# HKU-BAL/MegaGTA

Measured on AMD Instinct MI355X. Metric: HMM-scored node expansions/sec + SdBG-build Gk-mer/s, k=45, 100Mx150bp, higher is better.
Workload: dtype u32

## Files before the change

include/megagta_hip.h:

```cpp
#ifndef MEGAGTA_HIP_H_
#define MEGAGTA_HIP_H_
#include <stdint.h>
#ifdef __cplusplus
extern "C" {
#endif

#define MGTA_OK 0
#define MGTA_EINVAL (-1)
#define MGTA_EHIP (-2)
#define MGTA_ENOMEM (-3)
#define MGTA_EUNSUPPORTED (-4)
#define MGTA_ESINK (-5)
#define MGTA_EOVERFLOW (-6)
#define MGTA_EINTERNAL (-7)

#define MGTA_NUM_BUCKETS 65536

typedef struct mgta_ctx mgta_ctx;
typedef struct mgta_reads mgta_reads;
typedef struct mgta_sdbg mgta_sdbg;
typedef struct mgta_hmm mgta_hmm;

const char *mgta_last_error(void);
const char *mgta_version(void);

mgta_ctx *mgta_ctx_create(int device_id);
void mgta_ctx_destroy(mgta_ctx *);
int mgta_ctx_set_mem_limit(mgta_ctx *, uint64_t bytes);
int mgta_ctx_device_memory(mgta_ctx *, uint64_t *free_bytes, uint64_t *total_bytes);
int mgta_ctx_keep_stream(mgta_ctx *, int on);
typedef struct mgta_stream mgta_stream;
int mgta_sdbg_stream_detach(mgta_ctx *, mgta_stream **out);
int mgta_stream_sizes(const mgta_stream *, uint64_t *n_recs, uint64_t *n_tip_words);
int mgta_stream_download(mgta_stream *, uint16_t *recs, uint32_t *tips);
void mgta_stream_free(mgta_stream *);
int mgta_ctx_release_scratch(mgta_ctx *);
int mgta_ctx_set_full_lsd(mgta_ctx *, int on);
int mgta_sort_plan(uint64_t n_items, int words_per_key, uint32_t bucket_begin, uint32_t bucket_end, int *n_passes, int *skip_bits);
int mgta_ctx_set_search_cost_rate(mgta_ctx *, int expansions_per_seed);
int mgta_ctx_set_search_cost_curve(mgta_ctx *, int expansions_per_seed, uint64_t knee_expansions, int expansions_per_seed_beyond);
int mgta_ctx_set_search_arena(mgta_ctx *, int log2_base_nodes, uint64_t pool_bytes);
int mgta_ctx_set_search_page_limit(mgta_ctx *, int pages);
int mgta_ctx_keep_multiplicity(mgta_ctx *, int on);

int mgta_reads_pack_text(mgta_ctx *, const char *text, uint64_t n_bytes, const uint64_t *offsets , uint64_t n_reads,
                         uint32_t *bin_words, uint64_t capacity_words, uint64_t *n_words_out);


typedef int (*mgta_edge_sink)(void *user, int32_t bucket_begin, int32_t bucket_end,
                              const int64_t *bucket_counts ,
                              const uint16_t *recs, int64_t n_recs, const uint16_t *large, int64_t n_large,
                              const uint32_t *tips, int64_t n_tip_words);

typedef struct mgta_build_stats {
    int32_t k, words_per_key, words_per_tip, n_passes;
    int64_t n_reads, n_kmers;
    int64_t n_items;
    int64_t n_edges, n_tips, n_large;
    int64_t n_sort_launches;
    double ms_total;
    double ms_count, ms_gen, ms_sort, ms_emit, ms_d2h;
    double ms_sort_scatter;
    double ms_local_sort;
    int64_t n_big_segments;
    int64_t n_lsd_tiles;
    uint64_t bytes_peak;
    double ms_stage1;
    int64_t n_fused_passes;
} mgta_build_stats;

int mgta_reads_upload(mgta_ctx *, const uint32_t *packed_seq, uint64_t n_words, const uint64_t *start_idx,
                      uint64_t n_reads, mgta_reads **out);
int mgta_reads_adopt_device(mgta_ctx *, const uint32_t *d_packed_seq, uint64_t n_words,
                            const uint64_t *d_start_idx, uint64_t n_reads, mgta_reads **out);
void mgta_reads_free(mgta_reads *);

int mgta_sdbg_build_resident(mgta_ctx *, const mgta_reads *, uint64_t n_short_reads, int k, int min_count,
                             int need_mercy, int32_t bucket_begin, int32_t bucket_end ,
                             mgta_edge_sink sink, void *user, mgta_build_stats *stats);
int mgta_sdbg_last_counting(mgta_ctx *, int64_t *hist );
int mgta_sdbg_export_records_device(mgta_ctx *, void *d_dst, uint64_t capacity_bytes, uint64_t *n_records);
int mgta_sdbg_build(mgta_ctx *, const uint32_t *packed_seq, uint64_t n_words, const uint64_t *start_idx,
                    uint64_t n_reads, uint64_t n_short_reads, int k, int min_count, int need_mercy,
                    mgta_edge_sink sink, void *user, mgta_build_stats *stats);

int mgta_sdbg_load(mgta_ctx *, int k, const uint16_t *recs, int64_t size, const int64_t *bucket_items,
                   const uint32_t *tips, int64_t n_tip_words, int words_per_tip, mgta_sdbg **out);
int mgta_sdbg_load_resident(mgta_ctx *, mgta_sdbg **out);
int mgta_sdbg_load_large(mgta_ctx *, int k, const uint16_t *recs, int64_t size, const int64_t *bucket_items, const uint32_t *tips,
                         int64_t n_tip_words, int words_per_tip, const uint16_t *large, int64_t n_large, mgta_sdbg **out);
int mgta_sdbg_load_files(mgta_ctx *, const char *prefix, mgta_sdbg **out);
void mgta_sdbg_free(mgta_sdbg *);
int64_t mgta_sdbg_size(const mgta_sdbg *);
int mgta_sdbg_k(const mgta_sdbg *);
int mgta_sdbg_outgoing(mgta_sdbg *, const int64_t *edges, int64_t n, int64_t *out4, int8_t *outdeg);
int mgta_sdbg_invalid_bits(mgta_sdbg *, uint64_t *words);
int mgta_sdbg_index_edges(mgta_sdbg *, const uint8_t *seqs , int64_t n, int64_t *edge_ids);

int mgta_sdbg_edge_multiplicity(mgta_sdbg *, const int64_t *edge_ids, int64_t n, uint16_t *mult);

typedef struct mgta_contig_cov {
    uint64_t sum;
    uint32_t len, n_windows;
    uint32_t n_covered;
    uint32_t min, max, median;
} mgta_contig_cov;
typedef struct mgta_coverage_stats {
    int64_t n_contigs, n_windows;
    int64_t n_walked;
    int64_t n_index_searches;
    int64_t n_batches;
    int64_t groups_per_cu;
    double ms_kernel;
    double ms_walk;
} mgta_coverage_stats;
int mgta_ctx_set_coverage_batch(mgta_ctx *, uint64_t windows);
int mgta_contig_coverage(mgta_sdbg *, const char *seqs, const uint64_t *offsets , int64_t n, mgta_contig_cov *per_contig,
                         uint16_t *per_window , int64_t *abundance , mgta_coverage_stats *stats );

typedef struct mgta_contig_share {
    uint64_t mass;
    uint32_t len, n_windows;
    uint32_t n_covered;
    uint32_t n_unique;
    uint32_t max_share;
    uint32_t reserved_;
} mgta_contig_share;
typedef struct mgta_share_stats {
    int64_t n_contigs, n_windows;
    int64_t n_walked, n_index_searches;
    int64_t n_batches;
    int64_t n_covered;
    int64_t n_distinct_edges;
    uint64_t total_mult;
    uint64_t total_mass;
    uint64_t table_slots;
    uint64_t table_bytes;
    uint64_t window_bytes;
    double ms_walk;
    double ms_count;
    double ms_share;
    double ms_total;
} mgta_share_stats;
int mgta_ctx_set_share_hash_bits(mgta_ctx *, int bits);
int mgta_contig_share_coverage(mgta_sdbg *, const char *seqs, const uint64_t *offsets , int64_t n, mgta_contig_share *per_contig,
                               uint32_t *per_window_share , uint16_t *per_window , mgta_share_stats *stats );

typedef struct mgta_match_stats {
    int64_t n_contigs, n_contig_windows;
    int64_t n_marked_edges;
    int64_t n_reads, n_read_windows;
    int64_t n_walked, n_index_searches;
    int64_t n_matched_reads;
    int64_t groups_per_cu;
    double ms_mark, ms_walk;
} mgta_match_stats;
int mgta_reads_match_contigs(mgta_sdbg *, const mgta_reads *reads, int reads_reversed, uint64_t n_short_reads,
                             const char *seqs, const uint64_t *offsets , int64_t n,
                             uint64_t *match_bits ,
                             uint32_t *hit_windows , mgta_match_stats *stats );

typedef struct mgta_derep_stats {
    int64_t n_seqs, n_letters;
    int64_t n_first;
    int64_t n_duplicates, n_contained, n_kept;
    int64_t n_windows;
    int64_t anchor_len;
    int64_t n_compares;
    double ms_dups, ms_table, ms_verify;
} mgta_derep_stats;
int mgta_seqs_derep(mgta_ctx *, const char *seqs, const uint64_t *offsets , int64_t n,
                    uint8_t *status, int64_t *rep, uint32_t *copies, mgta_derep_stats *stats );
int mgta_ctx_set_derep_hash_bits(mgta_ctx *, int bits);

typedef struct mgta_align_rec {
    double score;
    int32_t status;
    int32_t model_from, model_to;
    int32_t n_match, n_insert, n_delete;
} mgta_align_rec;
typedef struct mgta_align_stats {
    int64_t n_seqs, n_aligned, n_unaligned;
    int64_t n_cells;
    int64_t n_batches;
    int64_t blocks_per_cu;
    int64_t waves_per_block;
    int64_t grid_blocks;
    int64_t lds_bytes;
    int64_t msc_in_lds;
    double ms_fill, ms_trace;
} mgta_align_stats;
int mgta_seqs_align(mgta_ctx *, const mgta_hmm *, const char *seqs, const uint64_t *offsets , int64_t n,
                    mgta_align_rec *recs , uint8_t *cols , char *path ,
                    int32_t *path_len , mgta_align_stats *stats );
int mgta_ctx_set_align_batch(mgta_ctx *, int64_t cells);

typedef struct mgta_row_pair { int32_t i, j; uint16_t n_diff, n_overlap; } mgta_row_pair;
typedef struct mgta_cluster_stats {
    int64_t n_rows, n_unaligned;
    int64_t n_pairs_kept;
    int64_t n_clusters, n_singletons, largest_cluster;
    int64_t n_components;
    int64_t n_tiles;
    int64_t n_link_pops;
    int64_t blocks_per_cu;
    int64_t grid_blocks;
    int64_t lds_bytes;
    int64_t peak_bytes;
    double ms_pairs, ms_link;
} mgta_cluster_stats;
int mgta_rows_pairs(mgta_ctx *, const uint8_t *rows , int64_t n, int64_t M, int64_t min_overlap, double cutoff,
                    mgta_row_pair *pairs , int64_t cap, int64_t *n_pairs, mgta_cluster_stats *stats );
int mgta_rows_cluster(mgta_ctx *, const uint8_t *rows , const int64_t *lens , int64_t n, int64_t M, int64_t min_overlap,
                      double cutoff, int32_t *cluster , int64_t *rep , uint16_t *rep_diff ,
                      uint16_t *rep_overlap , mgta_cluster_stats *stats );
int mgta_pairs_link(const mgta_row_pair *pairs , int64_t n_pairs, const int32_t *n_residues ,
                    const int64_t *lens , int64_t n, int32_t *cluster, int64_t *rep, uint16_t *rep_diff, uint16_t *rep_overlap,
                    mgta_cluster_stats *stats );
int mgta_ctx_set_cluster_tile(mgta_ctx *, int64_t rows_per_tile);

typedef struct mgta_nearest_rec { int32_t status, ref, score, ref_from, ref_to, n_match, n_ident, n_insert, n_delete; } mgta_nearest_rec;
// ... 117 lines not shown
```

megagta_amd/_lib.py:

```python
from __future__ import annotations

import ctypes as C
import os

_HERE = os.path.dirname(os.path.abspath(__file__))
LIB_PATH = os.environ.get("MEGAGTA_HIP_LIB") or os.path.join(_HERE, "libmegagta_hip.so")


class MegaGtaError(RuntimeError):
    pass


class DenovoStats(C.Structure):
    _fields_ = [("n_tips", C.c_int64), ("n_bubbles", C.c_int64), ("n_bubble_candidates", C.c_int64), ("n_bubble_rounds", C.c_int64),
                ("n_paths", C.c_int64), ("n_unitig_sweeps", C.c_int64), ("n_contigs", C.c_int64), ("total_len", C.c_int64),
                ("ms_tips", C.c_float), ("ms_bubbles", C.c_float), ("ms_unitigs", C.c_float)]

    def as_dict(self):
        return {n: getattr(self, n) for n, _ in self._fields_}


class BuildStats(C.Structure):
    _fields_ = [("k", C.c_int32), ("words_per_key", C.c_int32), ("words_per_tip", C.c_int32), ("n_passes", C.c_int32),
                ("n_reads", C.c_int64), ("n_kmers", C.c_int64), ("n_items", C.c_int64), ("n_edges", C.c_int64),
                ("n_tips", C.c_int64), ("n_large", C.c_int64), ("n_sort_launches", C.c_int64), ("ms_total", C.c_double),
                ("ms_count", C.c_double), ("ms_gen", C.c_double), ("ms_sort", C.c_double), ("ms_emit", C.c_double),
                ("ms_d2h", C.c_double), ("ms_sort_scatter", C.c_double), ("ms_local_sort", C.c_double), ("n_big_segments", C.c_int64), ("n_lsd_tiles", C.c_int64),
                ("bytes_peak", C.c_uint64), ("ms_stage1", C.c_double), ("n_fused_passes", C.c_int64)]

    def as_dict(self):
        return {n: getattr(self, n) for n, _ in self._fields_}


class AstarSide(C.Structure):
    _fields_ = [("ok", C.c_int32), ("fval", C.c_int32), ("length", C.c_int32), ("state_no", C.c_int32), ("state", C.c_int32),
                ("partial", C.c_int32), ("node_id", C.c_int64), ("n_closed", C.c_int64), ("n_expanded", C.c_int64),
                ("n_opened", C.c_int64), ("real_score", C.c_double), ("score", C.c_double)]


class AstarStats(C.Structure):
    _fields_ = [("n_seeds", C.c_int64), ("n_expansions", C.c_int64), ("n_opened", C.c_int64), ("n_retries", C.c_int64),
                ("ms_total", C.c_double), ("ms_kernel", C.c_double), ("n_grown", C.c_int64), ("n_rehash", C.c_int64),
                ("n_recycled", C.c_int64), ("pool_bytes", C.c_uint64), ("pool_used", C.c_uint64), ("n_resumes", C.c_int64),
                ("reserve_bytes", C.c_uint64), ("reserve_used", C.c_uint64), ("max_search_nodes", C.c_int64),
                ("max_search_expansions", C.c_int64), ("order_abandoned", C.c_int64), ("n_cache_drops", C.c_int64), ("hmm_in_lds", C.c_int64), ("n_over_limit", C.c_int64), ("ms_queue_drained", C.c_double)]

    def as_dict(self):
        return {n: getattr(self, n) for n, _ in self._fields_}


class LineProbe(C.Structure):
    _fields_ = [("waves_per_cu", C.c_int32), ("groups", C.c_int32), ("unroll", C.c_int32), ("dependent", C.c_int32), ("steps", C.c_uint64),
                ("lines_in_flight_per_cu", C.c_int32), ("pad_", C.c_int32), ("lines", C.c_uint64), ("ms", C.c_double), ("gb_per_s", C.c_double),
                ("ns_per_step", C.c_double)]

    def as_dict(self):
        return {n: getattr(self, n) for n, _ in self._fields_ if n != "pad_"}


class ContigCov(C.Structure):
    _fields_ = [("sum", C.c_uint64), ("len", C.c_uint32), ("n_windows", C.c_uint32), ("n_covered", C.c_uint32), ("min", C.c_uint32),
                ("max", C.c_uint32), ("median", C.c_uint32)]


class CoverageStats(C.Structure):
    _fields_ = [("n_contigs", C.c_int64), ("n_windows", C.c_int64), ("n_walked", C.c_int64), ("n_index_searches", C.c_int64),
                ("n_batches", C.c_int64), ("groups_per_cu", C.c_int64), ("ms_kernel", C.c_double), ("ms_walk", C.c_double)]

    def as_dict(self):
        return {n: getattr(self, n) for n, _ in self._fields_}


class ContigShare(C.Structure):
    _fields_ = [("mass", C.c_uint64), ("len", C.c_uint32), ("n_windows", C.c_uint32), ("n_covered", C.c_uint32), ("n_unique", C.c_uint32),
                ("max_share", C.c_uint32), ("reserved_", C.c_uint32)]


class ShareStats(C.Structure):
    _fields_ = [("n_contigs", C.c_int64), ("n_windows", C.c_int64), ("n_walked", C.c_int64), ("n_index_searches", C.c_int64), ("n_batches", C.c_int64),
                ("n_covered", C.c_int64), ("n_distinct_edges", C.c_int64), ("total_mult", C.c_uint64), ("total_mass", C.c_uint64),
                ("table_slots", C.c_uint64), ("table_bytes", C.c_uint64), ("window_bytes", C.c_uint64), ("ms_walk", C.c_double), ("ms_count", C.c_double),
                ("ms_share", C.c_double), ("ms_total", C.c_double)]

    def as_dict(self):
        return {n: getattr(self, n) for n, _ in self._fields_}


class MatchStats(C.Structure):
    _fields_ = [("n_contigs", C.c_int64), ("n_contig_windows", C.c_int64), ("n_marked_edges", C.c_int64), ("n_reads", C.c_int64),
                ("n_read_windows", C.c_int64), ("n_walked", C.c_int64), ("n_index_searches", C.c_int64), ("n_matched_reads", C.c_int64),
                ("groups_per_cu", C.c_int64), ("ms_mark", C.c_double), ("ms_walk", C.c_double)]

    def as_dict(self):
        return {n: getattr(self, n) for n, _ in self._fields_}


class DerepStats(C.Structure):
    _fields_ = [("n_seqs", C.c_int64), ("n_letters", C.c_int64), ("n_first", C.c_int64), ("n_duplicates", C.c_int64), ("n_contained", C.c_int64),
                ("n_kept", C.c_int64), ("n_windows", C.c_int64), ("anchor_len", C.c_int64), ("n_compares", C.c_int64), ("ms_dups", C.c_double),
                ("ms_table", C.c_double), ("ms_verify", C.c_double)]

    def as_dict(self):
        return {n: getattr(self, n) for n, _ in self._fields_}


class AlignRec(C.Structure):
    _fields_ = [("score", C.c_double), ("status", C.c_int32), ("model_from", C.c_int32), ("model_to", C.c_int32), ("n_match", C.c_int32),
                ("n_insert", C.c_int32), ("n_delete", C.c_int32)]


class AlignStats(C.Structure):
    _fields_ = [("n_seqs", C.c_int64), ("n_aligned", C.c_int64), ("n_unaligned", C.c_int64), ("n_cells", C.c_int64), ("n_batches", C.c_int64),
                ("blocks_per_cu", C.c_int64), ("waves_per_block", C.c_int64), ("grid_blocks", C.c_int64), ("lds_bytes", C.c_int64),
                ("msc_in_lds", C.c_int64), ("ms_fill", C.c_double), ("ms_trace", C.c_double)]

    def as_dict(self):
        return {n: getattr(self, n) for n, _ in self._fields_}


class RowPair(C.Structure):
    _fields_ = [("i", C.c_int32), ("j", C.c_int32), ("n_diff", C.c_uint16), ("n_overlap", C.c_uint16)]


class ClusterStats(C.Structure):
    _fields_ = [("n_rows", C.c_int64), ("n_unaligned", C.c_int64), ("n_pairs_kept", C.c_int64), ("n_clusters", C.c_int64), ("n_singletons", C.c_int64),
                ("largest_cluster", C.c_int64), ("n_components", C.c_int64), ("n_tiles", C.c_int64), ("n_link_pops", C.c_int64),
                ("blocks_per_cu", C.c_int64), ("grid_blocks", C.c_int64), ("lds_bytes", C.c_int64), ("peak_bytes", C.c_int64),
                ("ms_pairs", C.c_double), ("ms_link", C.c_double)]

    def as_dict(self):
        return {n: getattr(self, n) for n, _ in self._fields_}


class NearestRec(C.Structure):
    _fields_ = [("status", C.c_int32), ("ref", C.c_int32), ("score", C.c_int32), ("ref_from", C.c_int32), ("ref_to", C.c_int32), ("n_match", C.c_int32),
                ("n_ident", C.c_int32), ("n_insert", C.c_int32), ("n_delete", C.c_int32)]


class NearestStats(C.Structure):
    _fields_ = [("n_seqs", C.c_int64), ("n_refs", C.c_int64), ("n_pairs", C.c_int64), ("n_unaligned", C.c_int64), ("n_cells", C.c_int64),
                ("n_trace_cells", C.c_int64), ("n_batches", C.c_int64), ("n_segments", C.c_int64), ("blocks_per_cu", C.c_int64),
                ("waves_per_block", C.c_int64), ("grid_blocks", C.c_int64), ("lds_bytes", C.c_int64), ("peak_bytes", C.c_int64),
                ("ms_score", C.c_double), ("ms_trace", C.c_double)]

    def as_dict(self):
        return {n: getattr(self, n) for n, _ in self._fields_}


class ChimeraRec(C.Structure):
    _fields_ = [("status", C.c_int32), ("ref", C.c_int32), ("score", C.c_int32), ("brk", C.c_int32), ("left_ref", C.c_int32), ("left_score", C.c_int32),
                ("right_ref", C.c_int32), ("right_score", C.c_int32), ("two", C.c_int32), ("one", C.c_int32), ("gain", C.c_int32)]


class ChimeraStats(C.Structure):
    _fields_ = [("n_seqs", C.c_int64), ("n_refs", C.c_int64), ("n_clean", C.c_int64), ("n_chimeric", C.c_int64), ("n_unchecked", C.c_int64),
                ("n_cells", C.c_int64), ("n_parent_cells", C.c_int64), ("n_items", C.c_int64), ("n_parent_items", C.c_int64), ("n_segments", C.c_int64),
                ("n_groups", C.c_int64), ("grid_blocks", C.c_int64), ("waves_per_block", C.c_int64), ("blocks_per_cu", C.c_int64), ("lds_bytes", C.c_int64),
                ("bound_bytes", C.c_int64), ("peak_bytes", C.c_int64), ("ms_top", C.c_double), ("ms_parents", C.c_double)]

    def as_dict(self):
        return {n: getattr(self, n) for n, _ in self._fields_}


EDGE_SINK = C.CFUNCTYPE(C.c_int, C.c_void_p, C.c_int32, C.c_int32, C.POINTER(C.c_int64), C.POINTER(C.c_uint16), C.c_int64,
                        C.POINTER(C.c_uint16), C.c_int64, C.POINTER(C.c_uint32), C.c_int64)
CONTIG_SINK = C.CFUNCTYPE(C.c_int, C.c_void_p, C.c_int64, C.c_void_p, C.c_int64, C.c_void_p, C.c_int64,
                          C.POINTER(AstarSide), C.POINTER(AstarSide))

SYMBOLS = {
    "mgta_last_error": (C.c_char_p, []),
    "mgta_version": (C.c_char_p, []),
    "mgta_ctx_create": (C.c_void_p, [C.c_int]),
    "mgta_ctx_destroy": (None, [C.c_void_p]),
    "mgta_ctx_set_mem_limit": (C.c_int, [C.c_void_p, C.c_uint64]),
    "mgta_ctx_set_full_lsd": (C.c_int, [C.c_void_p, C.c_int]),
    "mgta_sort_plan": (C.c_int, [C.c_uint64, C.c_int, C.c_uint32, C.c_uint32, C.POINTER(C.c_int), C.POINTER(C.c_int)]),
    "mgta_reads_upload": (C.c_int, [C.c_void_p, C.c_void_p, C.c_uint64, C.c_void_p, C.c_uint64, C.POINTER(C.c_void_p)]),
    "mgta_reads_adopt_device": (C.c_int, [C.c_void_p, C.c_void_p, C.c_uint64, C.c_void_p, C.c_uint64, C.POINTER(C.c_void_p)]),
    "mgta_reads_free": (None, [C.c_void_p]),
    "mgta_sdbg_build_resident": (C.c_int, [C.c_void_p, C.c_void_p, C.c_uint64, C.c_int, C.c_int, C.c_int, C.c_int32, C.c_int32,
                                          EDGE_SINK, C.c_void_p, C.POINTER(BuildStats)]),
    "mgta_sdbg_last_counting": (C.c_int, [C.c_void_p, C.c_void_p]),
    "mgta_sdbg_export_records_device": (C.c_int, [C.c_void_p, C.c_void_p, C.c_uint64, C.POINTER(C.c_uint64)]),
    "mgta_sdbg_build": (C.c_int, [C.c_void_p, C.c_void_p, C.c_uint64, C.c_void_p, C.c_uint64, C.c_uint64, C.c_int, C.c_int,
                                 C.c_int, EDGE_SINK, C.c_void_p, C.POINTER(BuildStats)]),
    "mgta_findstart": (C.c_int, [C.c_void_p, C.c_void_p, C.c_int, C.c_int, C.c_void_p, C.c_int64, C.c_void_p, C.c_int64, C.c_void_p, C.c_void_p]),
    "mgta_sdbg_load_resident": (C.c_int, [C.c_void_p, C.c_void_p]),
    "mgta_sdbg_load_files": (C.c_int, [C.c_void_p, C.c_char_p, C.c_void_p]),
    "mgta_sdbg_invalid_bits": (C.c_int, [C.c_void_p, C.c_void_p]),
    "mgta_ctx_set_search_cost_rate": (C.c_int, [C.c_void_p, C.c_int]),
    "mgta_ctx_set_search_cost_curve": (C.c_int, [C.c_void_p, C.c_int, C.c_uint64, C.c_int]),
    "mgta_ctx_set_search_arena": (C.c_int, [C.c_void_p, C.c_int, C.c_uint64]),
    "mgta_ctx_set_search_page_limit": (C.c_int, [C.c_void_p, C.c_int]),
    "mgta_ctx_device_memory": (C.c_int, [C.c_void_p, C.POINTER(C.c_uint64), C.POINTER(C.c_uint64)]),
    "mgta_ctx_keep_stream": (C.c_int, [C.c_void_p, C.c_int]),
    "mgta_sdbg_stream_detach": (C.c_int, [C.c_void_p, C.POINTER(C.c_void_p)]),
    "mgta_stream_sizes": (C.c_int, [C.c_void_p, C.POINTER(C.c_uint64), C.POINTER(C.c_uint64)]),
    "mgta_stream_download": (C.c_int, [C.c_void_p, C.c_void_p, C.c_void_p]),
    "mgta_stream_free": (None, [C.c_void_p]),
    "mgta_sdbg_k": (C.c_int, [C.c_void_p]),
    "mgta_ctx_set_search_share": (C.c_int, [C.c_void_p, C.c_int, C.c_int]),
    "mgta_astar_batch_on": (C.c_int, [C.c_void_p, C.c_void_p, C.c_void_p, C.c_void_p, C.c_char_p, C.c_void_p, C.c_int64, C.c_int, C.c_double,
                                     C.c_int, CONTIG_SINK, C.c_void_p, C.POINTER(AstarStats)]),
    "mgta_astar_batch_packed": (C.c_int, [C.c_void_p, C.c_void_p, C.c_void_p, C.c_char_p, C.c_void_p, C.c_int64, C.c_int, C.c_double, C.c_int,
                                         C.POINTER(C.c_void_p), C.c_void_p, C.c_void_p, C.POINTER(AstarStats)]),
    "mgta_reads_pack_text": (C.c_int, [C.c_void_p, C.c_char_p, C.c_uint64, C.c_void_p, C.c_uint64, C.c_void_p, C.c_uint64, C.POINTER(C.c_uint64)]),
    "mgta_ctx_release_scratch": (C.c_int, [C.c_void_p]),
    "mgta_denovo": (C.c_int, [C.c_void_p, C.c_int, C.c_int, C.c_int, C.c_void_p, C.c_void_p, C.c_void_p]),
    "mgta_host_free": (None, [C.c_void_p]),
    "mgta_sdbg_load": (C.c_int, [C.c_void_p, C.c_int, C.c_void_p, C.c_int64, C.c_void_p, C.c_void_p, C.c_int64, C.c_int,
                                C.POINTER(C.c_void_p)]),
    "mgta_ctx_keep_multiplicity": (C.c_int, [C.c_void_p, C.c_int]),
    "mgta_ctx_set_coverage_batch": (C.c_int, [C.c_void_p, C.c_uint64]),
    "mgta_sdbg_load_large": (C.c_int, [C.c_void_p, C.c_int, C.c_void_p, C.c_int64, C.c_void_p, C.c_void_p, C.c_int64, C.c_int, C.c_void_p, C.c_int64,
                                      C.POINTER(C.c_void_p)]),
    "mgta_sdbg_edge_multiplicity": (C.c_int, [C.c_void_p, C.c_void_p, C.c_int64, C.c_void_p]),
    "mgta_contig_coverage": (C.c_int, [C.c_void_p, C.c_char_p, C.c_void_p, C.c_int64, C.c_void_p, C.c_void_p, C.c_void_p, C.c_void_p]),
    "mgta_contig_share_coverage": (C.c_int, [C.c_void_p, C.c_char_p, C.c_void_p, C.c_int64, C.c_void_p, C.c_void_p, C.c_void_p, C.c_void_p]),
    "mgta_ctx_set_share_hash_bits": (C.c_int, [C.c_void_p, C.c_int]),
    "mgta_reads_match_contigs": (C.c_int, [C.c_void_p, C.c_void_p, C.c_int, C.c_uint64, C.c_char_p, C.c_void_p, C.c_int64, C.c_void_p, C.c_void_p,
                                          C.c_void_p]),
    "mgta_seqs_derep": (C.c_int, [C.c_void_p, C.c_char_p, C.c_void_p, C.c_int64, C.c_void_p, C.c_void_p, C.c_void_p, C.c_void_p]),
    "mgta_ctx_set_derep_hash_bits": (C.c_int, [C.c_void_p, C.c_int]),
    "mgta_seqs_align": (C.c_int, [C.c_void_p, C.c_void_p, C.c_char_p, C.c_void_p, C.c_int64, C.c_void_p, C.c_void_p, C.c_void_p, C.c_void_p, C.c_void_p]),
    "mgta_ctx_set_align_batch": (C.c_int, [C.c_void_p, C.c_int64]),
    "mgta_rows_pairs": (C.c_int, [C.c_void_p, C.c_void_p, C.c_int64, C.c_int64, C.c_int64, C.c_double, C.c_void_p, C.c_int64, C.c_void_p, C.c_void_p]),
    "mgta_rows_cluster": (C.c_int, [C.c_void_p, C.c_void_p, C.c_void_p, C.c_int64, C.c_int64, C.c_int64, C.c_double, C.c_void_p, C.c_void_p, C.c_void_p,
                                    C.c_void_p, C.c_void_p]),
    "mgta_pairs_link": (C.c_int, [C.c_void_p, C.c_int64, C.c_void_p, C.c_void_p, C.c_int64, C.c_void_p, C.c_void_p, C.c_void_p, C.c_void_p, C.c_void_p]),
    "mgta_ctx_set_cluster_tile": (C.c_int, [C.c_void_p, C.c_int64]),
    "mgta_seqs_nearest": (C.c_int, [C.c_void_p, C.c_char_p, C.c_void_p, C.c_int64, C.c_char_p, C.c_void_p, C.c_int64, C.c_void_p, C.c_int32, C.c_int32,
                                    C.c_void_p, C.c_void_p, C.c_void_p, C.c_void_p, C.c_void_p]),
    "mgta_ctx_set_nearest_batch": (C.c_int, [C.c_void_p, C.c_int64]),
    "mgta_seqs_chimera": (C.c_int, [C.c_void_p, C.c_char_p, C.c_void_p, C.c_int64, C.c_char_p, C.c_void_p, C.c_int64, C.c_void_p, C.c_int32, C.c_int32,
                                    C.c_int32, C.c_int32, C.c_void_p, C.c_void_p, C.c_void_p]),
    "mgta_ctx_set_chimera_segment": (C.c_int, [C.c_void_p, C.c_int64]),
    "mgta_ctx_set_chimera_groups": (C.c_int, [C.c_void_p, C.c_int64]),
    "mgta_sdbg_free": (None, [C.c_void_p]),
    "mgta_sdbg_size": (C.c_int64, [C.c_void_p]),
    "mgta_sdbg_outgoing": (C.c_int, [C.c_void_p, C.c_void_p, C.c_int64, C.c_void_p, C.c_void_p]),
    "mgta_sdbg_index_edges": (C.c_int, [C.c_void_p, C.c_void_p, C.c_int64, C.c_void_p]),
    "mgta_hmm_load": (C.c_int, [C.c_void_p, C.c_int, C.c_int, C.c_void_p, C.c_void_p, C.c_void_p, C.c_void_p, C.c_void_p,
                               C.POINTER(C.c_void_p)]),
    "mgta_hmm_free": (None, [C.c_void_p]),
    "mgta_probe_random_lines": (C.c_int, [C.c_void_p, C.c_uint64, C.POINTER(LineProbe), C.c_int]),
    "mgta_astar_batch": (C.c_int, [C.c_void_p, C.c_void_p, C.c_void_p, C.c_char_p, C.c_void_p, C.c_int64, C.c_int, C.c_double,
                                  C.c_int, CONTIG_SINK, C.c_void_p, C.POINTER(AstarStats)]),
}

_LIB = None


def load():
    global _LIB
    if _LIB is not None:
        return _LIB
    if not os.path.exists(LIB_PATH):
        raise MegaGtaError(f"{LIB_PATH} is missing: build it with `python -c 'import __graft_entry__ as g; g.build()'` "
                           "(make -C megagta_amd/csrc). There is no CPU fallback.")
    L = C.CDLL(LIB_PATH)
    for name, (res, args) in SYMBOLS.items():
        fn = getattr(L, name)
        fn.restype, fn.argtypes = res, args
    _LIB = L
    return L


def check(rc: int, what: str):
    if rc != 0:
        raise MegaGtaError(f"{what} failed ({rc}): {load().mgta_last_error().decode()}")
```

megagta_amd/csrc/common.hpp:

```cpp
#pragma once
#include <hip/hip_runtime.h>

#include <cstdarg>
#include <cstdint>
#include <cstdio>
#include <cstring>
#include <exception>
#include <new>
#include <string>
#include <vector>

#include "../../include/megagta_hip.h"

namespace mgta {

void set_error(const char *fmt, ...);

struct HipError {
    int code;
};

#define MGTA_HIP_CHECK(expr)                                                                        \
    do {                                                                                            \
        hipError_t e_ = (expr);                                                                     \
        if (e_ != hipSuccess) {                                                                     \
            ::mgta::set_error("%s failed: %s (%s:%d)", #expr, hipGetErrorString(e_), __FILE__, __LINE__); \
            throw ::mgta::HipError{e_ == hipErrorOutOfMemory ? MGTA_ENOMEM : MGTA_EHIP};           \
        }                                                                                           \
    } while (0)

struct DevBuf {
    void *p = nullptr;
    size_t bytes = 0;
    uint64_t *live = nullptr, *peak = nullptr;
    DevBuf() = default;
    DevBuf(const DevBuf &) = delete;
    DevBuf &operator=(const DevBuf &) = delete;
    DevBuf(DevBuf &&o) noexcept { *this = std::move(o); }
    DevBuf &operator=(DevBuf &&o) noexcept {
        if (this != &o) { release(); p = o.p; bytes = o.bytes; live = o.live; peak = o.peak; o.p = nullptr; o.bytes = 0; }
        return *this;
    }
    ~DevBuf() { release(); }
    void alloc(size_t n, uint64_t *live_ = nullptr, uint64_t *peak_ = nullptr) {
        release();
        if (n == 0) n = 16;
        MGTA_HIP_CHECK(hipMalloc(&p, n));
        bytes = n; live = live_; peak = peak_;
        if (live) { *live += n; if (peak && *live > *peak) *peak = *live; }
    }
    void release() {
        if (p) { (void)hipFree(p); if (live) *live -= bytes; }
        p = nullptr; bytes = 0;
    }
    template <class T> T *as() const { return reinterpret_cast<T *>(p); }
};

template <class F> int guarded(const char *who, F &&f) {
    try { return f(); }
    catch (const HipError &e) { return e.code; }
    catch (const std::bad_alloc &) { set_error("%s: out of host memory", who); return MGTA_ENOMEM; }
    catch (const std::exception &e) { set_error("%s: %s", who, e.what()); return MGTA_EHIP; }
}

struct Timer {
    hipEvent_t a = nullptr, b = nullptr;
    hipStream_t st;
    explicit Timer(hipStream_t s) : st(s) { MGTA_HIP_CHECK(hipEventCreate(&a)); MGTA_HIP_CHECK(hipEventCreate(&b)); }
    Timer(Timer &&o) noexcept : a(o.a), b(o.b), st(o.st) { o.a = o.b = nullptr; }
    ~Timer() { if (a) (void)hipEventDestroy(a); if (b) (void)hipEventDestroy(b); }
    void start() { MGTA_HIP_CHECK(hipEventRecord(a, st)); }
    void end() { MGTA_HIP_CHECK(hipEventRecord(b, st)); }
    float ms() const { float t = 0; MGTA_HIP_CHECK(hipEventElapsedTime(&t, a, b)); return t; }
    double stop() {
        MGTA_HIP_CHECK(hipGetLastError());
        end();
        MGTA_HIP_CHECK(hipEventSynchronize(b));
        MGTA_HIP_CHECK(hipGetLastError());
        return ms();
    }
};

enum Slot { S_BLOCK_COUNT, S_BLOCK_BASE, S_SCAN_TMP, S_SMALL, S_KEYS_A, S_KEYS_B, S_HIST, S_TILE_HEADS, S_TILE_BASE, S_CNT, S_BASE,
            S_FIRST, S_OUT_REC, S_OUT_LARGE, S_OUT_TIPS, S_PLAN, S_BIG, S_LSD, S_MULTI_COUNT, S_POS2ID, S_SOLID, S_MERCY, S_EDGE_COUNT, S_SIDE, S_FUSED_HIST, S_NUM };

}

namespace mgta {
struct AstarArenas {
    DevBuf pool, meta;
};
}

struct mgta_ctx {
    int refs = 1;
    int device = 0;
    hipStream_t stream = nullptr;
    uint64_t mem_limit = 0;
    int force_full_lsd = 0;
    int lsd_skip_left = 0;
    int astar_log_b0 = 0;
    uint64_t astar_pool_bytes = 0;
    int search_page_limit = 0;
    int search_share_num = 1, search_share_den = 1;
    int search_cost_rate = 0;
    uint64_t search_cost_knee = 0;
    int search_cost_rate2 = 0;
    int force_lsd_tiles = 0;
    uint64_t live_bytes = 0, peak_bytes = 0;
    int num_cus = 256;
    hipDeviceProp_t prop;
    std::vector<mgta::DevBuf> pool;
    mgta::AstarArenas astar;
    std::vector<int64_t> edge_counting;
    const void *last_rec = nullptr;
    uint64_t last_n_rec = 0;
    uint32_t last_bucket_lo = 0, last_bucket_hi = 0;
    const void *last_tips = nullptr;
    const void *last_first = nullptr;
    uint64_t last_n_tips = 0;
    int last_k = 0, last_words_per_tip = 0;
    int keep_stream = 0;
    bool acc_valid = false;
    mgta::DevBuf acc_rec, acc_tips;
    uint64_t acc_n_rec = 0, acc_n_tips = 0;
    std::vector<int64_t> acc_items;
    int keep_multiplicity = 0;
    uint64_t coverage_batch_windows = 0;
    uint64_t align_batch_cells = 0;
    uint64_t nearest_batch_cells = 0;
    uint64_t chimera_segment_cols = 0;
    uint64_t chimera_groups = 0;
    uint64_t cluster_tile_rows = 0;
    int derep_hash_bits = 64;
    int share_hash_bits = 64;
    const void *last_large = nullptr;
    uint64_t last_n_large = 0;
    mgta::DevBuf acc_large;
    uint64_t acc_n_large = 0;
    bool acc_has_large = false;
};

namespace mgta {
inline void ctx_retain(mgta_ctx *c) { __atomic_add_fetch(&c->refs, 1, __ATOMIC_RELAXED); }
void ctx_release(mgta_ctx *c);
inline void forget_last_build(mgta_ctx *c) {
    c->last_rec = nullptr; c->last_tips = nullptr; c->last_first = nullptr; c->last_n_rec = 0; c->last_n_tips = 0; c->last_k = 0;
    c->last_large = nullptr; c->last_n_large = 0;
}
}

struct mgta_hmm {
    mgta_ctx *ctx = nullptr;
    int M = 0, A = 0;
    mgta::DevBuf tab;
    int8_t col[2][64];
    mgta::DevBuf d_col;
    int8_t alpha[128];
    mgta::DevBuf d_alpha;
    size_t n_doubles = 0;
};

struct mgta_reads {
    mgta_ctx *ctx = nullptr;
    const uint32_t *d_packed = nullptr;
    const uint64_t *d_start = nullptr;
    uint64_t n_words = 0, n_reads = 0;
    mgta::DevBuf own_packed, own_start;
};
```

megagta_amd/csrc/sdbg_build.hip:

```cpp
#include <algorithm>
#include <cmath>
#include <cstdlib>
#include <memory>
#include <type_traits>

#include "common.hpp"
#include "device_utils.hpp"
#include "scan.hpp"

namespace mgta {

constexpr int kDollar = 4;

template <int W>
struct Key {
    uint32_t w[W];
};

template <int W>
__device__ __forceinline__ void shl_bits(uint32_t (&x)[W], int s) {
    if (s == 0) return;
    if (s == 32) {
#pragma unroll
        for (int j = 0; j < W - 1; ++j) x[j] = x[j + 1];
        x[W - 1] = 0;
        return;
    }
#pragma unroll
    for (int j = 0; j < W; ++j) x[j] = (x[j] << s) | (j + 1 < W ? (x[j + 1] >> (32 - s)) : 0u);
}

template <int W>
__device__ __forceinline__ void keep_chars(uint32_t (&x)[W], int n) {
#pragma unroll
    for (int j = 0; j < W; ++j) {
        int lo = j * 16;
        if (n <= lo) x[j] = 0;
        else if (n < lo + 16) x[j] &= ~0u << (32 - 2 * (n - lo));
    }
}

template <int W>
__device__ __forceinline__ Key<W> make_key(const uint32_t (&e)[W], int from, int n, int k, int prev) {
    uint32_t t[W];
#pragma unroll
    for (int j = 0; j < W; ++j) t[j] = e[j];
    shl_bits<W>(t, 2 * from);
    keep_chars<W>(t, n);
    t[W - 1] |= (uint32_t)(n == k) << 3;
    t[W - 1] |= (uint32_t)prev;
    Key<W> key;
#pragma unroll
    for (int j = 0; j < W; ++j) key.w[j] = t[j];
    return key;
}

__device__ __forceinline__ uint32_t rev_chars(uint32_t x) {
    x = __brev(x);
    return ((x >> 1) & 0x55555555u) | ((x & 0x55555555u) << 1);
}

constexpr int kScanBlock = 256;
constexpr int kReadsPerBlock = 64;

struct ScanArgs {
    const uint32_t *packed;
    uint64_t n_words;
    const uint64_t *start;
    uint64_t n_reads;
    int k;
    uint32_t b_lo, b_hi;
    uint32_t *block_count;
    const uint64_t *block_base;
    void *out;
    unsigned long long *n_kmers;
    const unsigned long long *is_solid;
    int num_k1_per_read;
    uint64_t n_short;
    unsigned long long *n_sentinel;
    uint32_t multi_width, multi_n;
    uint64_t multi_magic;
    uint8_t *side;
    int side_shift;
    uint32_t side_bias;
    uint64_t *fz_hist;
    const uint64_t *fz_totals;
    uint64_t fz_n;
    uint32_t fz_bias[8];
    uint32_t fz_shift[8];
};
constexpr int kMaxCountRanges = 64;
constexpr int kMaxFusedRanges = 8;

__device__ __forceinline__ uint32_t xcd_tile(uint32_t b, uint32_t n) {
    if (n < 64) return b;
    const uint32_t x = b & 7u, idx = b >> 3, q = n >> 3, r = n & 7u;
    return x * q + (x < r ? x : r) + idx;
}

constexpr int kFusedLdsKB = 26;
template <int W> struct FusedCfg {
    static constexpr int kWaveRound = 6 * 64;
    static constexpr int kFit = (kFusedLdsKB * 1024 - 5 * 1024) / (4 * W + 2) / 128 * 128;
    static constexpr int kCap = kFit < kWaveRound ? kWaveRound : (kFit > 8192 ? 8192 : kFit);
};
template <int W> struct FusedShared {
    Key<W> stage[FusedCfg<W>::kCap];
    uint16_t perm[FusedCfg<W>::kCap];
    uint32_t cnt[256];
    uint32_t pos[256];
    uint64_t next[256];
    uint32_t wave_tot[2][kScanBlock / 64];
    uint32_t scr[kScanBlock / 64];
    uint64_t s64[kScanBlock / 64 + 1];
};

template <int W>
__device__ __forceinline__ void keep_masks(int n, uint32_t (&m)[W]) {
#pragma unroll
    for (int j = 0; j < W; ++j) {
        const int lo = j * 16;
        m[j] = n <= lo ? 0u : (n < lo + 16 ? ~0u << (32 - 2 * (n - lo)) : ~0u);
    }
}

template <int W, bool WRITE, bool CENSUS, bool FUSED>
__device__ __forceinline__ void item_scan_body(const ScanArgs &a) {
    static_assert(!(CENSUS && WRITE) && !(FUSED && !WRITE), "the census belongs to the count scan, the placing to the writer");
    static_assert(kScanBlock == 256, "fused writer: one thread per digit value");
    __shared__ uint32_t s_cursor;
    __shared__ uint32_t s_wave_cnt[kScanBlock / 64];
    __shared__ uint32_t s_range_cnt[kMaxCountRanges];
    __shared__ uint32_t s_fz_hist[CENSUS ? kMaxFusedRanges * 256 : 1];
    __shared__ uint32_t s_fz_bias[kMaxFusedRanges], s_fz_shift[kMaxFusedRanges];
    __shared__ std::conditional_t<FUSED, FusedShared<W>, uint32_t> fs;
    const int k = a.k;
    const int lane = lane_id(), wv = wave_id();
    __shared__ uint64_t s_start[kReadsPerBlock + 1];
    const bool multi = !WRITE && a.multi_n > 0;
    const uint64_t multi_magic = a.multi_magic;
    const bool magic24 = multi_magic < (1u << 24);
    const uint32_t blk = (CENSUS || FUSED) ? xcd_tile(blockIdx.x, gridDim.x) : blockIdx.x;
    uint64_t r0 = (uint64_t)blk * kReadsPerBlock;
    uint64_t r1 = r0 + kReadsPerBlock < a.n_reads ? r0 + kReadsPerBlock : a.n_reads;
    if (threadIdx.x == 0) s_cursor = 0;
    if (!WRITE && threadIdx.x < kMaxCountRanges) s_range_cnt[threadIdx.x] = 0;
    if (threadIdx.x <= r1 - r0) s_start[threadIdx.x] = a.start[r0 + threadIdx.x];
    if constexpr (CENSUS) {
        for (int i = threadIdx.x; i < kMaxFusedRanges * 256; i += kScanBlock) s_fz_hist[i] = 0;
        if (threadIdx.x < kMaxFusedRanges) { s_fz_bias[threadIdx.x] = a.fz_bias[threadIdx.x]; s_fz_shift[threadIdx.x] = a.fz_shift[threadIdx.x]; }
    }
    const uint32_t fz_bias = a.fz_bias[0], fz_shift = a.fz_shift[0];
    uint32_t fz_fill = 0, fz_round = 0;
    if constexpr (FUSED) {
        const uint64_t t = a.fz_totals[threadIdx.x];
        const uint64_t ex = block_excl_scan64<kScanBlock>(t, fs.s64, nullptr);
        fs.next[threadIdx.x] = ex + a.fz_hist[(uint64_t)threadIdx.x * gridDim.x + blk];
        fs.cnt[threadIdx.x] = 0;
    }
    __syncthreads();
    Key<W> *out = reinterpret_cast<Key<W> *>(a.out);
    uint64_t base = WRITE && !FUSED ? a.block_base[blockIdx.x] : 0;
    uint32_t my_count = 0;
    unsigned long long kmers = 0;
    const int pad_bits = 2 * (16 * W - (k + 1));
    const bool even = !((k + 1) & 1);
    const bool few = multi && a.multi_n <= 8;
    uint32_t acc[8] = {0, 0, 0, 0, 0, 0, 0, 0};
    uint32_t m_edge[W], m_k[W], m_k1[W];
    keep_masks<W>(k + 1, m_edge);
    keep_masks<W>(k, m_k);
    keep_masks<W>(k - 1, m_k1);
    const bool in_bounds = wave_uniform((s_start[r1 - r0] >> 4) + (uint64_t)(W + 1)) < a.n_words;

    auto fz_digit = [&](uint32_t w0) { return ((w0 - fz_bias) >> fz_shift) & 255u; };
    auto flush = [&](uint32_t n) {
        if constexpr (FUSED) {
            const uint32_t tid = threadIdx.x;
            __syncthreads();
            const uint32_t c = fs.cnt[tid], inc = wave_incl_scan(c);
            if (lane == 63) fs.scr[wv] = inc;
            __syncthreads();
            uint32_t ex = inc - c;
            for (int w = 0; w < wv; ++w) ex += fs.scr[w];
            fs.pos[tid] = ex;
            fs.cnt[tid] = 0;
            __syncthreads();
            for (uint32_t j = tid; j < n; j += kScanBlock) {
                const uint32_t d = fz_digit(fs.stage[j].w[0]);
                fs.perm[fs.pos[d] + atomicAdd(&fs.cnt[d], 1u)] = (uint16_t)j;
            }
            __syncthreads();
            for (uint32_t i = tid; i < n; i += kScanBlock) {
                const Key<W> key = fs.stage[fs.perm[i]];
                const uint32_t d = fz_digit(key.w[0]);
                const uint64_t to = fs.next[d] + (i - fs.pos[d]);
                if (to < a.fz_n) {
                    out[to] = key;
                    if (a.side) a.side[to] = (uint8_t)((key.w[0] - a.side_bias) >> a.side_shift);
                }
            }
            __syncthreads();
            fs.next[tid] += c;
            fs.cnt[tid] = 0;
            __syncthreads();
        }
    };
    auto positions = [&](bool active, uint64_t r, uint64_t s0, int p, int npos, bool more = false) {
        bool run_first = p == 0, run_last = p == npos - 1;
        if (active && a.is_solid && r < a.n_short) {
            auto sol = [&](int pp) {
                uint64_t bit = (uint64_t)a.num_k1_per_read * r + (uint64_t)pp;
                return (bool)((a.is_solid[bit >> 6] >> (bit & 63)) & 1);
            };
            active = sol(p);
            if (active) {
                run_first = p == 0 || !sol(p - 1);
                run_last = p == npos - 1 || !sol(p + 1);
            }
        }
        int cnt = 0;
        uint32_t fields = 0;
        uint32_t mask = 0;
        uint32_t e[W], rc[W];
        if (active) {
            uint64_t q = s0 + (uint64_t)p;
            uint64_t wi = q >> 4;
            int sh = (int)(q & 15) * 2;
            uint32_t raw[W + 1];
            if (in_bounds) {
#pragma unroll
                for (int j = 0; j <= W; ++j) raw[j] = a.packed[wi + j];
            } else {
#pragma unroll
                for (int j = 0; j <= W; ++j) raw[j] = (wi + j < a.n_words) ? a.packed[wi + j] : 0u;
            }
#pragma unroll
            for (int j = 0; j < W; ++j) e[j] = (uint32_t)(((((uint64_t)raw[j]) << 32) | (uint64_t)raw[j + 1]) >> (32 - sh)) & m_edge[j];
#pragma unroll
            for (int j = 0; j < W; ++j) rc[j] = rev_chars(~e[W - 1 - j]);
            shl_bits<W>(rc, pad_bits);
            bool pal = even;
            if (even) {
#pragma unroll
                for (int j = 0; j < W; ++j) pal = pal && (e[j] == rc[j]);
            }
            auto push = [&](int t, const uint32_t (&src)[W], int from, uint32_t keep0) {
                const uint32_t b = ((src[0] << (2 * from)) >> 16);
                if (b < a.b_lo || b >= a.b_hi) return;
                if (WRITE) mask |= 1u << t;
                else if (multi) {
                    const uint32_t x = b - a.b_lo;
                    uint32_t range;
                    if (magic24) asm("v_mul_hi_u32_u24 %0, %1, %2" : "=v"(range) : "v"(x), "v"((uint32_t)multi_magic));
                    else range = (uint32_t)(((uint64_t)x * multi_magic) >> 32);
                    if (few) fields += 1u << (4 * range);
                    else atomicAdd(&s_range_cnt[range], 1u);
                    if constexpr (CENSUS) {
                        const uint32_t w0 = (from ? ((src[0] << (2 * from)) | (src[W > 1 ? 1 : 0] >> (32 - 2 * from))) : src[0]) & keep0;
                        if (range < (uint32_t)kMaxFusedRanges)
                            atomicAdd(&s_fz_hist[range * 256u + (((w0 - s_fz_bias[range]) >> s_fz_shift[range]) & 255u)], 1u);
                    }
                }
                ++cnt;
            };
            if (run_first) {
                push(0, e, 0, m_k[0]);
                if (!pal) push(1, rc, 2, m_k1[0]);
            }
            push(2, e, 1, m_k[0]);
            if (!pal) push(3, rc, 1, m_k[0]);
            if (run_last) {
                push(4, e, 2, m_k1[0]);
                if (!pal) push(5, rc, 0, m_k[0]);
            }
        }
        if (!WRITE) {
            my_count += (uint32_t)cnt;
            if (few) {
#pragma unroll
                for (int g = 0; g < 8; ++g)
                    if (g < (int)a.multi_n) acc[g] += (fields >> (4 * g)) & 15u;
            }
        } else {
            const uint32_t inc = wave_incl_scan((uint32_t)cnt);
            const uint32_t tot = __shfl(inc, 63, 64);
            uint32_t fz_before = 0, fz_tot[kScanBlock / 64] = {};
            bool any_more = false;
            if constexpr (FUSED) {
                const uint32_t par = fz_round & 1u;
                ++fz_round;
                if (lane == 0) fs.wave_tot[par][wv] = tot | (more ? 0x80000000u : 0u);
                __syncthreads();
                for (int w = 0; w < kScanBlock / 64; ++w) fz_tot[w] = wave_uniform(fs.wave_tot[par][w]);
            }
            auto take_turns = [&](int from, int to) {
                if constexpr (FUSED) {
#pragma unroll
                    for (int turn = 0; turn < kScanBlock / 64; ++turn) {
                        if (turn < from || turn >= to) continue;
                        const uint32_t tw = fz_tot[turn] & 0x7FFFFFFFu;
                        any_more = any_more || (fz_tot[turn] >> 31);
                        if (fz_fill + tw > (uint32_t)FusedCfg<W>::kCap) { flush(fz_fill); fz_fill = 0; }
                        fz_before = fz_fill;
                        fz_fill += tw;
                    }
                }
            };
            take_turns(0, wv + 1);
            if (tot) {
                uint32_t wbase = 0;
                if (!FUSED && lane == 0) wbase = atomicAdd(&s_cursor, tot);
                const uint64_t first = base + (uint64_t)wave_uniform(wbase);
                char *const wave_out = reinterpret_cast<char *>(out + first);
                uint8_t *const wave_side = !FUSED && a.side ? a.side + first : nullptr;
                uint32_t slot = inc - (uint32_t)cnt + fz_before;
                auto put = [&](int t, const uint32_t (&src)[W], int from, const uint32_t (&keep)[W], uint32_t flags) {
                    if (!((mask >> t) & 1u)) return;
                    Key<W> key;
#pragma unroll
                    for (int j = 0; j < W; ++j) {
                        const uint32_t nx = j + 1 < W ? src[j + 1 < W ? j + 1 : j] : 0u;
                        key.w[j] = (from ? ((src[j] << (2 * from)) | (nx >> (32 - 2 * from))) : src[j]) & keep[j];
                    }
                    key.w[W - 1] |= flags;
                    if constexpr (FUSED) {
                        if (slot < (uint32_t)FusedCfg<W>::kCap) {
                            fs.stage[slot] = key;
                            atomicAdd(&fs.cnt[fz_digit(key.w[0])], 1u);
                        }
                    } else {
                        *reinterpret_cast<Key<W> *>(wave_out + slot * (uint32_t)sizeof(Key<W>)) = key;
                        if (wave_side) wave_side[slot] = (uint8_t)((key.w[0] - a.side_bias) >> a.side_shift);
                    }
                    ++slot;
                };
                const uint32_t e0 = e[0] >> 30, e1 = (e[0] >> 28) & 3u, r0c = rc[0] >> 30, r1c = (rc[0] >> 28) & 3u;
                put(0, e, 0, m_k, 8u | (uint32_t)kDollar);
                put(1, rc, 2, m_k1, r1c);
                put(2, e, 1, m_k, 8u | e0);
                put(3, rc, 1, m_k, 8u | r0c);
                put(4, e, 2, m_k1, e1);
                put(5, rc, 0, m_k, 8u | (uint32_t)kDollar);
            }
            take_turns(wv + 1, kScanBlock / 64);
            if constexpr (FUSED) {
                if (!any_more) flush(fz_fill);
                return any_more;
            }
        }
        return false;
    };
// ... 116 lines not shown
    if (threadIdx.x == kScanBlock - 1) s_first[256] = ex + t;
    __syncthreads();
    if (blockIdx.x == 0 && threadIdx.x == 0 && s_first[256] != n) atomicAdd(&bad[1], 1u);
    for (uint64_t i = (uint64_t)blockIdx.x * kScanBlock + threadIdx.x; i < n; i += (uint64_t)gridDim.x * kScanBlock) {
        const uint32_t d = ((keys[i].w[0] - bias) >> shift) & 255u;
        if (i < s_first[d] || i >= s_first[d + 1]) atomicAdd(&bad[0], 1u);
    }
}

template <int W>
__global__ __launch_bounds__(kScanBlock) void item_write_closed_kernel(ScanArgs a) {
    __shared__ uint32_t s_read_base[kReadsPerBlock];
    __shared__ uint64_t s_start[kReadsPerBlock + 1];
    const int k = a.k;
    const int lane = lane_id(), wv = wave_id();
    const uint64_t r0 = (uint64_t)blockIdx.x * kReadsPerBlock;
    const uint64_t r1 = r0 + kReadsPerBlock < a.n_reads ? r0 + kReadsPerBlock : a.n_reads;
    if (wv == 0) {
        const uint64_t st = r0 + lane <= r1 ? a.start[r0 + lane] : 0, st_next = r0 + lane < r1 ? a.start[r0 + lane + 1] : st;
        s_start[lane] = st;
        if (r0 + lane + 1 == r1) s_start[lane + 1] = st_next;
        uint32_t items = 0;
        if (r0 + lane < r1) {
            const int len = (int)(st_next - st);
            if (len >= k + 1) items = 2u * (uint32_t)(len - k) + 4u;
        }
        s_read_base[lane] = wave_incl_scan(items) - items;
    }
    __syncthreads();
    Key<W> *out = reinterpret_cast<Key<W> *>(a.out) + a.block_base[blockIdx.x];
    const int pad_bits = 2 * (16 * W - (k + 1));
    for (uint64_t r = r0 + wv; r < r1; r += kScanBlock / 64) {
        const uint64_t s0 = s_start[r - r0];
        const int len = (int)(s_start[r - r0 + 1] - s0);
        if (len < k + 1) continue;
        const int npos = len - k;
        Key<W> *ro = out + s_read_base[r - r0];
        for (int c0 = 0; c0 < npos; c0 += 64) {
            const int p = c0 + lane;
            if (p >= npos) continue;
            const uint64_t q = s0 + (uint64_t)p, wi = q >> 4;
            const int sh = (int)(q & 15) * 2;
            uint32_t raw[W + 1], e[W], rc[W];
#pragma unroll
            for (int j = 0; j <= W; ++j) raw[j] = (wi + j < a.n_words) ? a.packed[wi + j] : 0u;
#pragma unroll
            for (int j = 0; j < W; ++j) e[j] = sh ? ((raw[j] << sh) | (raw[j + 1] >> (32 - sh))) : raw[j];
            keep_chars<W>(e, k + 1);
#pragma unroll
            for (int j = 0; j < W; ++j) rc[j] = rev_chars(~e[W - 1 - j]);
            shl_bits<W>(rc, pad_bits);
            const int e0 = e[0] >> 30, e1 = (e[0] >> 28) & 3, r0c = rc[0] >> 30, r1c = (rc[0] >> 28) & 3;
            bool pal = false;
            if (!((k + 1) & 1)) {
                pal = true;
#pragma unroll
                for (int j = 0; j < W; ++j) pal = pal && e[j] == rc[j];
            }
            Key<W> sentinel;
#pragma unroll
            for (int j = 0; j < W; ++j) sentinel.w[j] = ~0u;
            ro[2 + 2 * p] = make_key<W>(e, 1, k, k, e0);
            ro[3 + 2 * p] = pal ? sentinel : make_key<W>(rc, 1, k, k, r0c);
            if (p == 0) {
                ro[0] = make_key<W>(e, 0, k, k, kDollar);
                ro[1] = pal ? sentinel : make_key<W>(rc, 2, k - 1, k, r1c);
            }
            if (p == npos - 1) {
                ro[2 + 2 * npos] = make_key<W>(e, 2, k - 1, k, e1);
                ro[3 + 2 * npos] = pal ? sentinel : make_key<W>(rc, 0, k, k, kDollar);
            }
            const unsigned long long pm = __ballot(pal);
            if (pm && lane == __ffsll((long long)pm) - 1) {
                unsigned long long c = 0;
                for (unsigned long long m = pm; m; m &= m - 1) {
                    const int l = __ffsll((long long)m) - 1, pp = c0 + l;
                    c += 1ull + (pp == 0) + (pp == npos - 1);
                }
                atomicAdd(a.n_sentinel, c);
            }
        }
    }
}

__global__ __launch_bounds__(256) void item_count_closed_kernel(const uint64_t *start, uint64_t n_reads, uint64_t n_blocks, int k,
                                                                uint32_t *block_count, unsigned long long *n_kmers) {
    unsigned long long kmers = 0;
    for (int q = 0; q < 16; ++q) {
        const uint64_t blk = ((uint64_t)blockIdx.x * 4 + wave_id()) * 16 + q;
        if (blk >= n_blocks) break;
        const uint64_t r = blk * kReadsPerBlock + lane_id();
        uint32_t items = 0, npos = 0;
        if (r < n_reads) {
            const int len = (int)(start[r + 1] - start[r]);
            if (len >= k + 1) { npos = (uint32_t)(len - k); items = 2 * npos + 4; }
        }
        items = wave_sum(items);
        kmers += wave_sum(npos);
        if (lane_id() == 0 && block_count) block_count[blk] = items;
    }
    if (lane_id() == 0 && n_kmers && kmers) atomicAdd(n_kmers, kmers);
}

constexpr int kSortThreads = 1024;
constexpr int kSortWaves = kSortThreads / 64;
constexpr int kItemsPerThread = 4;
constexpr int kSubTile = kSortThreads * kItemsPerThread;
constexpr int kSubTilesPerBlock = 8;
constexpr int kBlockTile = kSubTile * kSubTilesPerBlock;

struct Digit {
    int pos;
    int bits;
    uint32_t bias;
};

template <int W, bool BIASED = false>
__device__ __forceinline__ uint32_t get_digit(const Key<W> &key, Digit d) {
    const int wi = W - 1 - (d.pos >> 5), off = d.pos & 31;
    uint32_t lo = 0, hi = 0;
#pragma unroll
    for (int j = 0; j < W; ++j) {
        if (j == wi) {
            lo = key.w[j] - (BIASED && j == 0 ? d.bias : 0u);
            hi = j > 0 ? key.w[j - 1] - (BIASED && j == 1 ? d.bias : 0u) : 0u;
            asm volatile("" : "+v"(lo), "+v"(hi));
        }
    }
    return __builtin_amdgcn_alignbit(hi, lo, (uint32_t)off) & ((1u << d.bits) - 1u);
}

template <int W, int N, bool BIASED = false>
__device__ __forceinline__ void get_digits(const Key<W> (&key)[N], Digit d, uint32_t (&dg)[N]) {
    const int wi = W - 1 - (d.pos >> 5), off = d.pos & 31;
    uint32_t lo[N], hi[N];
#pragma unroll
    for (int i = 0; i < N; ++i) { lo[i] = 0; hi[i] = 0; }
#pragma unroll
    for (int j = 0; j < W; ++j) {
        if (j == wi) {
#pragma unroll
            for (int i = 0; i < N; ++i) {
                lo[i] = key[i].w[j] - (BIASED && j == 0 ? d.bias : 0u);
                hi[i] = j > 0 ? key[i].w[j - 1] - (BIASED && j == 1 ? d.bias : 0u) : 0u;
                asm volatile("" : "+v"(lo[i]), "+v"(hi[i]));
            }
        }
    }
    const uint32_t mask = (1u << d.bits) - 1u;
#pragma unroll
    for (int i = 0; i < N; ++i) dg[i] = __builtin_amdgcn_alignbit(hi[i], lo[i], (uint32_t)off) & mask;
}

template <int W>
__global__ __launch_bounds__(kSortThreads) void radix_census_kernel(const Key<W> *keys, uint64_t n, Digit d, uint64_t n_tiles,
                                                                     uint64_t *hist) {
    __shared__ uint32_t h[256];
    for (int i = threadIdx.x; i < 256; i += kSortThreads) h[i] = 0;
    __syncthreads();
    const uint32_t tile = xcd_tile(blockIdx.x, (uint32_t)n_tiles);
    uint64_t base = (uint64_t)tile * kBlockTile;
    int wi = W - 1 - (d.pos >> 5), off = d.pos & 31;
    bool straddle = off + d.bits > 32 && wi > 0;
    uint32_t mask = (1u << d.bits) - 1u;
    for (int i = 0; i < kBlockTile / kSortThreads; ++i) {
        uint64_t idx = base + (uint64_t)i * kSortThreads + threadIdx.x;
        if (idx < n) {
            uint32_t v = (keys[idx].w[wi] - (wi == 0 ? d.bias : 0u)) >> off;
            if (straddle) v |= (keys[idx].w[wi - 1] - (wi == 1 ? d.bias : 0u)) << (32 - off);
            atomicAdd(&h[v & mask], 1u);
        }
    }
    __syncthreads();
    for (int i = threadIdx.x; i < 256; i += kSortThreads) hist[(uint64_t)i * n_tiles + tile] = h[i];
}

__global__ __launch_bounds__(kSortThreads) void radix_census_side_kernel(const uint8_t *side, uint64_t n, uint64_t n_tiles, uint64_t *hist) {
    __shared__ uint32_t h[256];
    for (int i = threadIdx.x; i < 256; i += kSortThreads) h[i] = 0;
    __syncthreads();
    const uint32_t tile = xcd_tile(blockIdx.x, (uint32_t)n_tiles);
    const uint64_t base = (uint64_t)tile * kBlockTile;
    constexpr int kPerThread = kBlockTile / kSortThreads;
#pragma unroll
    for (int half = 0; half < kPerThread / 16; ++half) {
        const uint64_t idx = base + (uint64_t)half * (kSortThreads * 16) + (uint64_t)threadIdx.x * 16;
        if (idx + 16 <= n) {
            const uint4 v = *reinterpret_cast<const uint4 *>(side + idx);
            const uint32_t w[4] = {v.x, v.y, v.z, v.w};
#pragma unroll
            for (int j = 0; j < 4; ++j) {
                atomicAdd(&h[w[j] & 255u], 1u);
                atomicAdd(&h[(w[j] >> 8) & 255u], 1u);
                atomicAdd(&h[(w[j] >> 16) & 255u], 1u);
                atomicAdd(&h[w[j] >> 24], 1u);
            }
        } else {
            for (uint64_t i = idx; i < n && i < idx + 16; ++i) atomicAdd(&h[side[i]], 1u);
        }
    }
    __syncthreads();
    for (int i = threadIdx.x; i < 256; i += kSortThreads) hist[(uint64_t)i * n_tiles + tile] = h[i];
}

template <int W>
__global__ __launch_bounds__(kScanBlock) void item_write_tiled_kernel(ScanArgs a, uint64_t n_blocks, uint64_t n_items, int digit_shift,
                                                                      uint64_t n_tiles, uint64_t *hist) {
    __shared__ uint32_t s_hist[256];
    __shared__ uint32_t s_read_base[kReadsPerBlock];
    __shared__ uint64_t s_start[kReadsPerBlock + 1];
    const int k = a.k;
    const int lane = lane_id(), wv = wave_id();
    for (int i = threadIdx.x; i < 256; i += kScanBlock) s_hist[i] = 0;
    const uint64_t lo = (uint64_t)blockIdx.x * kBlockTile;
    const uint64_t hi = lo + kBlockTile < n_items ? lo + kBlockTile : n_items;
    uint64_t left = 0, right = n_blocks;
    while (right - left > 1) {
        const uint64_t step = (right - left + 63) / 64, idx = left + (uint64_t)lane * step;
        const bool ok = idx < right && a.block_base[idx] <= lo;
        const unsigned long long m = __ballot(ok);
        const uint64_t nl = left + (uint64_t)(__popcll(m) - 1) * step;
        right = nl + step < right ? nl + step : right;
        left = nl;
    }
    Key<W> *out = reinterpret_cast<Key<W> *>(a.out);
    const int pad_bits = 2 * (16 * W - (k + 1));
    for (uint64_t b = left; b < n_blocks; ++b) {
        const uint64_t bb = a.block_base[b];
        if (bb >= hi) break;
        const uint64_t r0 = b * kReadsPerBlock;
        const uint64_t r1 = r0 + kReadsPerBlock < a.n_reads ? r0 + kReadsPerBlock : a.n_reads;
        __syncthreads();
        if (wv == 0) {
            const uint64_t st = r0 + lane <= r1 ? a.start[r0 + lane] : 0, st_next = r0 + lane < r1 ? a.start[r0 + lane + 1] : st;
            s_start[lane] = st;
            if (r0 + lane + 1 == r1) s_start[lane + 1] = st_next;
            uint32_t items = 0;
            if (r0 + lane < r1) {
                const int len = (int)(st_next - st);
                if (len >= k + 1) items = 2u * (uint32_t)(len - k) + 4u;
            }
            s_read_base[lane] = wave_incl_scan(items) - items;
        }
        __syncthreads();
        for (uint64_t r = r0 + wv; r < r1; r += kScanBlock / 64) {
            const uint64_t s0 = s_start[r - r0];
            const int len = (int)(s_start[r - r0 + 1] - s0);
            if (len < k + 1) continue;
            const int npos = len - k;
            const uint64_t rb = bb + s_read_base[r - r0], re = rb + 2ull * (uint64_t)npos + 4ull;
            if (re <= lo || rb >= hi) continue;
            const int j_lo = rb >= lo ? 0 : (int)((lo - rb) >> 1), j_hi = re <= hi ? npos + 2 : (int)((hi - rb) >> 1);
            Key<W> *ro = out + rb;
            for (int c0 = j_lo; c0 < j_hi; c0 += 64) {
                const int j = c0 + lane;
                if (j >= j_hi) continue;
                const int p = j == 0 ? 0 : (j == npos + 1 ? npos - 1 : j - 1);
                const uint64_t q = s0 + (uint64_t)p, wi = q >> 4;
                const int sh = (int)(q & 15) * 2;
                uint32_t raw[W + 1], e[W], rc[W];
#pragma unroll
                for (int i = 0; i <= W; ++i) raw[i] = (wi + i < a.n_words) ? a.packed[wi + i] : 0u;
#pragma unroll
                for (int i = 0; i < W; ++i) e[i] = sh ? ((raw[i] << sh) | (raw[i + 1] >> (32 - sh))) : raw[i];
                keep_chars<W>(e, k + 1);
#pragma unroll
                for (int i = 0; i < W; ++i) rc[i] = rev_chars(~e[W - 1 - i]);
                shl_bits<W>(rc, pad_bits);
                const int e0 = e[0] >> 30, e1 = (e[0] >> 28) & 3, r0c = rc[0] >> 30, r1c = (rc[0] >> 28) & 3;
                bool pal = false;
                if (!((k + 1) & 1)) {
                    pal = true;
#pragma unroll
                    for (int i = 0; i < W; ++i) pal = pal && e[i] == rc[i];
                }
                Key<W> ka, kb;
                if (j == 0) {
                    ka = make_key<W>(e, 0, k, k, kDollar);
                    kb = make_key<W>(rc, 2, k - 1, k, r1c);
                } else if (j == npos + 1) {
                    ka = make_key<W>(e, 2, k - 1, k, e1);
                    kb = make_key<W>(rc, 0, k, k, kDollar);
                } else {
                    ka = make_key<W>(e, 1, k, k, e0);
                    kb = make_key<W>(rc, 1, k, k, r0c);
                }
                if (pal) {
#pragma unroll
                    for (int i = 0; i < W; ++i) kb.w[i] = ~0u;
                }
                const unsigned long long pm = __ballot(pal);
                if (pm && lane == __ffsll((long long)pm) - 1) atomicAdd(a.n_sentinel, (unsigned long long)__popcll(pm));
                ro[2 * j] = ka;
                ro[2 * j + 1] = kb;
                atomicAdd(&s_hist[(ka.w[0] >> digit_shift) & 255u], 1u);
                atomicAdd(&s_hist[(kb.w[0] >> digit_shift) & 255u], 1u);
            }
        }
    }
    __syncthreads();
    for (int i = threadIdx.x; i < 256; i += kScanBlock) hist[(uint64_t)i * n_tiles + blockIdx.x] = s_hist[i];
}

__global__ __launch_bounds__(1024) void radix_rowscan_kernel(uint64_t *hist, uint64_t n_tiles, uint64_t *totals) {
    __shared__ uint64_t scratch[1024 / 64 + 1];
    __shared__ uint64_t carry_s;
    uint64_t *row = hist + (uint64_t)blockIdx.x * n_tiles;
    if (threadIdx.x == 0) carry_s = 0;
    __syncthreads();
    for (uint64_t b = 0; b < n_tiles; b += 1024) {
        uint64_t idx = b + threadIdx.x;
        uint64_t x = idx < n_tiles ? row[idx] : 0, tot;
        uint64_t ex = block_excl_scan64<1024>(x, scratch, &tot);
        uint64_t carry = carry_s;
        if (idx < n_tiles) row[idx] = carry + ex;
        __syncthreads();
        if (threadIdx.x == 0) carry_s = carry + tot;
        __syncthreads();
    }
    if (threadIdx.x == 0) totals[blockIdx.x] = carry_s;
}

template <int W> struct ScatterCfg {
    static constexpr int kIpt = W >= 10 ? 2 : kItemsPerThread;
    static constexpr int kSub = kSortThreads * kIpt;
    static constexpr int kChunk = kSub / kSortWaves;
};

template <int W>
struct ScatterShared {
    Key<W> keys[ScatterCfg<W>::kSub];
    uint16_t whist[kSortWaves][256];
    uint64_t gbase[256];
    uint64_t gdelta[256];
    uint32_t scratch[kSortThreads / 64 + 1];
};

struct SideShared {
    uint8_t bytes[kBlockTile];
    uint64_t gtile[256];
    uint32_t toff[257];
};

template <int W, bool BIASED = false, bool SIDE = false, bool STABLE = true>
__device__ __forceinline__ void scatter_subtiles(ScatterShared<W> &sh, const Key<W> *in, Key<W> *out, uint64_t n, Digit d, SideShared *ss = nullptr,
                                                 Digit d_next = Digit{0, 0, 0}) {
    constexpr int kItemsPerThread = ScatterCfg<W>::kIpt, kSubTile = ScatterCfg<W>::kSub, kWaveChunk = ScatterCfg<W>::kChunk;
    const int tid = threadIdx.x, lane = lane_id(), wv = wave_id();
    uint16_t *whist = sh.whist[wv];
    for (int i = lane; i < 256; i += 64) whist[i] = 0;
    constexpr bool kPrefetch = W * kItemsPerThread <= 16;
    Key<W> key[kItemsPerThread], nxt[kItemsPerThread];
    auto load = [&](Key<W> (&dst)[kItemsPerThread], uint64_t sub_base) {
#pragma unroll
        for (int it = 0; it < kItemsPerThread; ++it) {
            uint64_t idx = sub_base + (uint32_t)wv * kWaveChunk + (uint32_t)it * 64 + (uint32_t)lane;
            if (idx < n) dst[it] = in[idx];
        }
    };
    load(key, 0);
    for (uint64_t sub_base = 0; sub_base < n; sub_base += kSubTile) {
        uint32_t n_valid = (uint32_t)((n - sub_base) < (uint64_t)kSubTile ? (n - sub_base) : (uint64_t)kSubTile);
        uint32_t dr[kItemsPerThread], cnt[kItemsPerThread];
        get_digits<W, kItemsPerThread, BIASED>(key, d, dr);
        if constexpr (STABLE) {
#pragma unroll
            for (int it = 0; it < kItemsPerThread; ++it) {
                uint32_t j = (uint32_t)wv * kWaveChunk + (uint32_t)it * 64 + (uint32_t)lane;
                bool valid = j < n_valid;
                uint32_t dg = valid ? dr[it] : 0u, rank;
                wave_match(dg, d.bits, valid, rank, cnt[it]);
                dr[it] = dg | (rank << 8) | ((uint32_t)valid << 31);
            }
#pragma unroll
            for (int it = 0; it < kItemsPerThread; ++it) {
                if (dr[it] >> 31) {
                    const uint32_t dg = dr[it] & 255u, rank = (dr[it] >> 8) & 0xFFu, prev = whist[dg];
                    if (rank == cnt[it] - 1) whist[dg] = (uint16_t)(prev + cnt[it]);
                    dr[it] += prev << 8;
                }
                wave_lds_fence();
            }
        } else {
            uint32_t *const wh32 = reinterpret_cast<uint32_t *>(whist);
#pragma unroll
            for (int it = 0; it < kItemsPerThread; ++it) {
                const uint32_t j = (uint32_t)wv * kWaveChunk + (uint32_t)it * 64 + (uint32_t)lane;
                const bool valid = j < n_valid;
                const uint32_t dg = valid ? dr[it] : 0u;
                uint32_t taken = 0;
                if (valid) taken = (atomicAdd(&wh32[dg >> 1], 1u << (16u * (dg & 1u))) >> (16u * (dg & 1u))) & 0xFFFFu;
                dr[it] = dg | (taken << 8) | ((uint32_t)valid << 31);
            }
            wave_lds_fence();
        }
        if (kPrefetch && sub_base + kSubTile < n) load(nxt, sub_base + kSubTile);
        __syncthreads();
        uint32_t tot = 0, inc = 0;
        if (wv < 4) {
#pragma unroll
            for (int w = 0; w < kSortWaves; ++w) tot += sh.whist[w][tid];
            inc = wave_incl_scan(tot);
            if (lane == 63) sh.scratch[wv] = inc;
        }
        __syncthreads();
        if (wv < 4) {
            uint32_t running = inc - tot;
            for (int w = 0; w < wv; ++w) running += sh.scratch[w];
            const uint64_t g = sh.gbase[tid];
            sh.gdelta[tid] = g - running;
            sh.gbase[tid] = g + tot;
#pragma unroll
            for (int w = 0; w < kSortWaves; ++w) { uint32_t c = sh.whist[w][tid]; sh.whist[w][tid] = (uint16_t)running; running += c; }
        }
        __syncthreads();
#pragma unroll
        for (int it = 0; it < kItemsPerThread; ++it) {
            if (dr[it] >> 31) {
                const uint32_t pos = whist[dr[it] & 255u] + ((dr[it] >> 8) & 0x7FFFFFu);
#pragma unroll
                for (int w = 0; w < W; ++w) sh.keys[pos].w[w] = key[it].w[w];
            }
        }
        __syncthreads();
        for (int i = lane; i < 256; i += 64) whist[i] = 0;
        if (kPrefetch) {
            Key<W> kk[kItemsPerThread];
            uint32_t dg[kItemsPerThread];
#pragma unroll
            for (int it = 0; it < kItemsPerThread; ++it) {
                uint32_t j = (uint32_t)it * kSortThreads + (uint32_t)tid;
                if (j < n_valid) kk[it] = sh.keys[j];
            }
            get_digits<W, kItemsPerThread, BIASED>(kk, d, dg);
            if constexpr (SIDE) {
                uint32_t dn[kItemsPerThread];
                get_digits<W, kItemsPerThread, BIASED>(kk, d_next, dn);
#pragma unroll
                for (int it = 0; it < kItemsPerThread; ++it) {
                    uint32_t j = (uint32_t)it * kSortThreads + (uint32_t)tid;
                    if (j < n_valid) {
                        const uint64_t to = sh.gdelta[dg[it]] + j;
                        out[to] = kk[it];
                        ss->bytes[(uint32_t)(to - ss->gtile[dg[it]])] = (uint8_t)dn[it];
                    }
                }
            } else {
#pragma unroll
                for (int it = 0; it < kItemsPerThread; ++it) {
                    uint32_t j = (uint32_t)it * kSortThreads + (uint32_t)tid;
                    if (j < n_valid) out[sh.gdelta[dg[it]] + j] = kk[it];
                }
            }
#pragma unroll
            for (int it = 0; it < kItemsPerThread; ++it) key[it] = nxt[it];
        } else {
#pragma unroll
            for (int it = 0; it < kItemsPerThread; ++it) {
                uint32_t j = (uint32_t)it * kSortThreads + (uint32_t)tid;
                if (j < n_valid) {
                    Key<W> kk = sh.keys[j];
                    const uint32_t dg = get_digit<W, BIASED>(kk, d);
                    const uint64_t to = sh.gdelta[dg] + j;
                    out[to] = kk;
                    if constexpr (SIDE) ss->bytes[(uint32_t)(to - ss->gtile[dg])] = (uint8_t)get_digit<W, BIASED>(kk, d_next);
                }
            }
            if (sub_base + kSubTile < n) load(key, sub_base + kSubTile);
        }
    }
}

template <int W> constexpr bool kSideFits = sizeof(ScatterShared<W>) + sizeof(SideShared) + 1024 <= 160 * 1024;

template <int W, bool BIASED, bool SIDE = false, bool STABLE = true>
__global__ __launch_bounds__(kSortThreads, 4) void radix_scatter_kernel(const Key<W> *in, Key<W> *out, uint64_t n, Digit d,
                                                                      uint64_t n_tiles, const uint64_t *rowoff,
                                                                      const uint64_t *totals, uint8_t *side = nullptr,
                                                                      Digit d_next = Digit{0, 0, 0}) {
    __shared__ ScatterShared<W> sh;
    __shared__ uint64_t s64[kSortThreads / 64 + 1];
    const int tid = threadIdx.x;
    const uint32_t tile = xcd_tile(blockIdx.x, (uint32_t)n_tiles);
    uint64_t t = tid < 256 ? totals[tid] : 0;
    uint64_t ex = block_excl_scan64<kSortThreads>(t, s64, nullptr);
    const uint64_t my_off = tid < 256 ? rowoff[(uint64_t)tid * n_tiles + tile] : 0;
    if (tid < 256) sh.gbase[tid] = ex + my_off;
    const uint64_t tile_base = (uint64_t)tile * kBlockTile;
    if constexpr (SIDE) {
        __shared__ SideShared ss;
        uint64_t c = 0;
        if (tid < 256) c = (tile + 1 < n_tiles ? rowoff[(uint64_t)tid * n_tiles + tile + 1] : t) - my_off;
        __syncthreads();
        const uint64_t place = block_excl_scan64<kSortThreads>(c, s64, nullptr);
        if (tid < 256) {
            ss.toff[tid] = (uint32_t)place;
            ss.gtile[tid] = ex + my_off - place;
            if (tid == 255) ss.toff[256] = (uint32_t)(place + c);
        }
        __syncthreads();
        if (tile_base >= n) return;
        const uint64_t cnt = (n - tile_base) < (uint64_t)kBlockTile ? (n - tile_base) : (uint64_t)kBlockTile;
        scatter_subtiles<W, BIASED, true, STABLE>(sh, in + tile_base, out, cnt, d, &ss, d_next);
        __syncthreads();
        const int lane = lane_id(), wv = wave_id();
        for (int v = wv * (256 / kSortWaves); v < (wv + 1) * (256 / kSortWaves); ++v) {
            const uint32_t from = ss.toff[v], len = ss.toff[v + 1] - from;
            uint8_t *to = side + ss.gtile[v] + from;
            for (uint32_t i = lane; i < len; i += 64) to[i] = ss.bytes[from + i];
        }
    } else {
        __syncthreads();
        if (tile_base >= n) return;
        const uint64_t cnt = (n - tile_base) < (uint64_t)kBlockTile ? (n - tile_base) : (uint64_t)kBlockTile;
        scatter_subtiles<W, BIASED, false, STABLE>(sh, in + tile_base, out, cnt, d);
    }
}

template <int W>
__global__ __launch_bounds__(kSortThreads) void segment_sort_kernel(Key<W> *buf_a, Key<W> *buf_b, const uint64_t *big, const uint64_t *big_end,
                                                                     const Digit *low_plan, int n_low, uint32_t lds_cap) {
    __shared__ ScatterShared<W> sh;
    __shared__ uint64_t s64[kSortThreads / 64 + 1];
    __shared__ uint32_t s_cnt[256];
    const int tid = threadIdx.x;
    const uint64_t s0 = big[blockIdx.x], cnt = big_end[blockIdx.x] - s0;
    if (cnt <= (uint64_t)lds_cap) return;
    Key<W> *x = buf_a + s0, *y = buf_b + s0;
    for (int pass = 0; pass < n_low; ++pass) {
        const Digit d = low_plan[pass];
        if (tid < 256) s_cnt[tid] = 0;
        __syncthreads();
        for (uint64_t i = tid; i < cnt; i += kSortThreads) atomicAdd(&s_cnt[get_digit<W>(x[i], d)], 1u);
        __syncthreads();
        uint64_t c = tid < 256 ? s_cnt[tid] : 0;
        uint64_t ex = block_excl_scan64<kSortThreads>(c, s64, nullptr);
        if (tid < 256) sh.gbase[tid] = ex;
        __syncthreads();
        scatter_subtiles<W>(sh, x, y, cnt, d);
        __threadfence();
        __syncthreads();
        Key<W> *t = x; x = y; y = t;
    }
    if (x != buf_a + s0)
        for (uint64_t i = tid; i < cnt; i += kSortThreads) y[i] = x[i];
}

template <int W> struct LocalCfg {
    static constexpr int kTile = W <= 4 ? 4096 : 2048;
    static constexpr int kIpt = kTile / kSortThreads;
    static constexpr int kChunk = kTile / kSortWaves;
};

template <int W> struct BigCfg {
    static constexpr int kTile = W <= 4 ? 8192 : (W <= 8 ? 4096 : 0);
};

template <int W, int TILE = LocalCfg<W>::kTile>
struct LocalShared {
    Key<W> keys[TILE];
    uint16_t seg[TILE];
    uint16_t whist[kSortWaves][256];
    uint32_t start[256];
    uint32_t scratch[kSortThreads / 64 + 1];
    uint32_t wheads[kSortWaves + 1];
};

template <int W>
struct CompareShared {
    static constexpr int kRoom = (80 * 1024 - 1024 - LocalCfg<W>::kTile * 4 * W) / 2;
    static constexpr int kBins = kRoom >= 2048 ? (kRoom / 2048 * 2048 < 16384 ? kRoom / 2048 * 2048 : 16384) : 16384;
    static_assert(kBins >= LocalCfg<W>::kTile || kBins == 16384, "a bin per segment at least");
    Key<W> keys[LocalCfg<W>::kTile];
    uint32_t hist[kBins / 2];
    uint32_t scratch[kSortThreads / 64 + 1];
    uint32_t flags[2];
    uint64_t masks[LocalCfg<W>::kTile / 64];
};

template <int W>
__device__ __forceinline__ uint32_t key_prefix(const Key<W> &key, int T) { return T == 0 ? 0u : (key.w[0] >> (32 - T)); }

struct LocalPlan {
    const Digit *low_plan;
    int n_low;
    int T;
    Digit upper;
    uint32_t mask_last2;
    uint32_t mask_last;
    uint32_t stride;
    uint64_t *lsd_list;
    uint32_t *lsd_count;
    uint32_t lsd_cap;
    int debug;
};

constexpr uint32_t kMaxAvgRun = 40;
constexpr uint32_t kMaxRun = 256;

template <int W, int FIRST, bool MASKED>
__device__ __forceinline__ bool key_less(const Key<W> &a, const Key<W> &b, uint32_t m2, uint32_t m1) {
    bool lt = false;
    auto word = [&](const Key<W> &k, int j) {
        uint32_t x = k.w[j];
        if (MASKED && j == W - 1) x &= m1;
        if (MASKED && j == W - 2) x &= m2;
        return x;
    };
#pragma unroll
    for (int j = W - 1; j >= FIRST; j -= 2) {
        if (j - 1 >= FIRST) {
            const uint64_t x = ((uint64_t)word(a, j - 1) << 32) | word(a, j), y = ((uint64_t)word(b, j - 1) << 32) | word(b, j);
            lt = x < y || (x == y && lt);
        } else {
            const uint32_t x = word(a, j), y = word(b, j);
            lt = x < y || (x == y && lt);
        }
    }
    return lt;
}

template <int W>
__device__ __forceinline__ int tile_load(LocalShared<W> &sh, const Key<W> *keys, uint64_t first, uint32_t nt, int T, Key<W> (&key)[LocalCfg<W>::kIpt],
                                         uint32_t (&seg)[LocalCfg<W>::kIpt]) {
    constexpr int kIpt = LocalCfg<W>::kIpt, kChunk = LocalCfg<W>::kChunk;
    const int lane = lane_id(), wv = wave_id();
    const uint64_t le_mask = lanemask_lt() | (1ull << lane);
    uint32_t running = 0;
#pragma unroll
    for (int it = 0; it < kIpt; ++it) {
        uint32_t j = (uint32_t)wv * kChunk + (uint32_t)it * 64 + (uint32_t)lane;
        bool valid = j < nt, head = false;
        if (valid) {
            key[it] = keys[first + j];
            head = j == 0 || key_prefix<W>(key[it], T) != key_prefix<W>(keys[first + j - 1], T);
        }
        uint64_t bal = __ballot(head);
        seg[it] = running + (uint32_t)__popcll(bal & le_mask);
        running += (uint32_t)__popcll(bal);
    }
    if (lane == 0) sh.wheads[wv] = running;
    __syncthreads();
    uint32_t before = 0, nseg = 0;
    for (int w = 0; w < kSortWaves; ++w) { uint32_t c = sh.wheads[w]; if (w < wv) before += c; nseg += c; }
    before = wave_uniform(before);
    nseg = wave_uniform(nseg);
#pragma unroll
    for (int it = 0; it < kIpt; ++it) seg[it] = seg[it] + before - 1;
    return nseg <= 1 ? 0 : (nseg <= 256 ? 1 : 2);
}

template <int W, int TILE = LocalCfg<W>::kTile>
__device__ __forceinline__ void tile_zero_counts(LocalShared<W, TILE> &sh) {
    uint16_t *whist = sh.whist[wave_id()];
    for (int i = lane_id(); i < 256; i += 64) whist[i] = 0;
}

template <int W, int TILE = LocalCfg<W>::kTile>
__device__ __forceinline__ void lds_pass(LocalShared<W, TILE> &sh, Key<W> (&key)[TILE / kSortThreads], uint32_t (&seg)[TILE / kSortThreads], uint32_t nt,
                                         Digit d, bool by_seg, int seg_shift, bool reload, uint32_t off = 0) {
    constexpr int kIpt = TILE / kSortThreads, kChunk = TILE / kSortWaves;
    const int tid = threadIdx.x, lane = lane_id(), wv = wave_id();
    uint16_t *whist = sh.whist[wv];
    uint32_t dr[kIpt], cnt[kIpt];
    if (by_seg) {
#pragma unroll
        for (int it = 0; it < kIpt; ++it) dr[it] = (seg[it] >> seg_shift) & 255u;
    } else {
// ... 457 lines not shown
constexpr int kDecideTile = kDecideThreads * kDecidePerThread;
constexpr int kDecideHalo = 32;

__device__ __forceinline__ bool run_suppressed(int a, int b, int has_a, int has_b) {
    return (a == kDollar && ((has_b >> b) & 1)) || (b == kDollar && ((has_a >> a) & 1));
}

__global__ __launch_bounds__(kDecideThreads) void emit_decide_kernel(RunStarts sub_start, const uint8_t *sub_info, uint64_t m,
                                                                      uint64_t n_items, uint16_t *rec, uint32_t *cnt_e,
                                                                      uint32_t *cnt_l, uint32_t *cnt_t) {
    __shared__ uint32_t s_e[kDecideThreads / 64], s_l[kDecideThreads / 64], s_t[kDecideThreads / 64];
    __shared__ uint8_t s_info[kDecideTile + 2 * kDecideHalo];
    const uint64_t t0 = (uint64_t)blockIdx.x * kDecideTile;
    const uint64_t w_lo = t0 >= (uint64_t)kDecideHalo ? t0 - kDecideHalo : 0;
    const uint64_t w_hi = t0 + kDecideTile + kDecideHalo < m ? t0 + kDecideTile + kDecideHalo : m;
    for (uint64_t x = w_lo + threadIdx.x; x < w_hi; x += kDecideThreads) s_info[x - w_lo] = sub_info[x];
    __syncthreads();
    auto info_at = [&](uint64_t x) -> int { return (x >= w_lo && x < w_hi) ? (int)s_info[x - w_lo] : (int)sub_info[x]; };
    uint32_t ne = 0, nl = 0, nt = 0;
    for (int q = 0; q < kDecidePerThread; ++q) {
        uint64_t s = t0 + (uint64_t)q * kDecideThreads + threadIdx.x;
        if (s >= m) break;
        int inf = info_at(s);
        int a = inf & 7, b = (inf >> 3) & 7;
        int has_a = 0, has_b = 0;
        auto collect = [&](int xi) {
            const int xa = xi & 7, xb = (xi >> 3) & 7;
            if (xa != kDollar && xb != kDollar) { has_a |= 1 << xa; has_b |= 1 << xb; }
        };
        collect(inf);
        bool front_b_solid = false, front_b_dollar = false;
        uint64_t gs = s;
        for (int gi = inf; !(gi & 64);) {
            --gs; gi = info_at(gs); collect(gi);
            if (((gi >> 3) & 7) == b) { if ((gi & 7) != kDollar) front_b_solid = true; else front_b_dollar = true; }
        }
        uint64_t ge = s + 1;
        while (ge < m) {
            const int xi = info_at(ge);
            if (xi & 64) break;
            collect(xi);
            ++ge;
        }
        uint16_t r = 0xFFFF;
        if (!run_suppressed(a, b, has_a, has_b)) {
            const bool seen_b = front_b_solid || (front_b_dollar && !((has_b >> b) & 1));
            int w = (b == kDollar) ? 0 : (seen_b ? b + 5 : b + 1);
            int last = 0;
            if (a != kDollar) {
                bool later = false;
                for (uint64_t x = s + 1; x < ge; ++x) {
                    int xi = info_at(x), xa = xi & 7, xb = (xi >> 3) & 7;
                    if (xa == a && (xb != kDollar || !((has_a >> a) & 1))) later = true;
                }
                last = later ? 0 : 1;
            }
            uint64_t run = run_length(sub_start, s, m, n_items);
            uint32_t count = run > 65535 ? 65535u : (uint32_t)run;
            int tip = a == kDollar;
            r = (uint16_t)(w | (last << 4) | (tip << 5) | ((count > 255 ? 255u : count) << 8));
            ne++;
            nl += count > 254;
            nt += tip;
        }
        rec[s] = r;
    }
    ne = wave_sum(ne); nl = wave_sum(nl); nt = wave_sum(nt);
    if (lane_id() == 0) { s_e[wave_id()] = ne; s_l[wave_id()] = nl; s_t[wave_id()] = nt; }
    __syncthreads();
    if (threadIdx.x == 0) {
        uint32_t e = 0, l = 0, t = 0;
        for (int w = 0; w < kDecideThreads / 64; ++w) { e += s_e[w]; l += s_l[w]; t += s_t[w]; }
        cnt_e[blockIdx.x] = e; cnt_l[blockIdx.x] = l; cnt_t[blockIdx.x] = t;
    }
}

template <int W>
__global__ __launch_bounds__(kDecideThreads) void emit_write_kernel(const Key<W> *keys, RunStarts sub_start, const uint8_t *sub_info, const uint16_t *rec,
                                                                     uint64_t m, uint64_t n_items, const uint64_t *base_e,
                                                                     const uint64_t *base_l, const uint64_t *base_t, int words_per_tip,
                                                                     uint32_t b_lo, uint16_t *out_rec, uint16_t *out_large,
                                                                     uint32_t *out_tips, int64_t *bucket_first ) {
    __shared__ uint64_t s_scr[kDecideThreads / 64 + 1];
    uint64_t s0 = (uint64_t)blockIdx.x * kDecideTile + (uint64_t)threadIdx.x * kDecidePerThread;
    uint16_t r[kDecidePerThread];
    uint64_t packed = 0;
    uint32_t cnts[kDecidePerThread];
    for (int q = 0; q < kDecidePerThread; ++q) {
        uint64_t s = s0 + q;
        r[q] = 0xFFFF; cnts[q] = 0;
        if (s < m) {
            r[q] = rec[s];
            if (r[q] != 0xFFFF) {
                uint64_t run = run_length(sub_start, s, m, n_items);
                cnts[q] = run > 65535 ? 65535u : (uint32_t)run;
                packed += 1ull + ((uint64_t)(cnts[q] > 254) << 20) + ((uint64_t)((r[q] >> 5) & 1) << 40);
            }
        }
    }
    uint64_t ex = block_excl_scan64<kDecideThreads>(packed, s_scr, nullptr);
    uint64_t ie = base_e[blockIdx.x] + (ex & 0xFFFFF), il = base_l[blockIdx.x] + ((ex >> 20) & 0xFFFFF),
             it = base_t[blockIdx.x] + (ex >> 40);
    for (int q = 0; q < kDecidePerThread; ++q) {
        uint64_t s = s0 + q;
        if (s >= m) break;
        const bool is_tip = r[q] != 0xFFFF && ((r[q] >> 5) & 1);
        const bool bucket_head = (sub_info[s] & 128) != 0;
        const uint64_t first_item = (is_tip || bucket_head) ? run_full_start(sub_start, s) : 0;
        if (bucket_head) {
            uint32_t bucket = keys[first_item].w[0] >> 16;
            int64_t *bf = bucket_first + (uint64_t)(bucket - b_lo) * 3;
            bf[0] = (int64_t)ie; bf[1] = (int64_t)il; bf[2] = (int64_t)it;
        }
        if (r[q] != 0xFFFF) {
            out_rec[ie++] = r[q];
            if (cnts[q] > 254) out_large[il++] = (uint16_t)cnts[q];
            if ((r[q] >> 5) & 1) {
                for (int j = 0; j < words_per_tip; ++j) out_tips[it * words_per_tip + j] = keys[first_item].w[j];
                it++;
            }
        }
    }
}

}
#include "sdbg_solid.hpp"
namespace mgta {

static std::vector<Digit> low_digit_plan(int k, int W, int T) {
    std::vector<Digit> plan;
    int pad = 32 * W - 2 * k - 4, top = 32 * W - T;
    if (top > 0) plan.push_back(Digit{0, std::min(4, top)});
    for (int pos = 4 + pad; pos < top; pos += 8) plan.push_back(Digit{pos, std::min(8, top - pos)});
    return plan;
}

template <class T>
static T *pool_get(mgta_ctx *ctx, int slot, uint64_t bytes) {
    if ((int)ctx->pool.size() < S_NUM) ctx->pool.resize(S_NUM);
    DevBuf &b = ctx->pool[slot];
    if (b.bytes < bytes || !b.p) {
        b.release();
        b.alloc(bytes + bytes / 8, &ctx->live_bytes, &ctx->peak_bytes);
    }
    return b.as<T>();
}
static uint64_t pool_bytes(const mgta_ctx *ctx) {
    uint64_t t = 0;
    for (const DevBuf &b : ctx->pool) t += b.bytes;
    return t;
}

struct SortModes {
    int bias = 1, side = 1, fused = 1;
    static SortModes from_env() {
        const char *bias = getenv("MGTA_SORT_BIAS"), *side = getenv("MGTA_SORT_SIDE"), *fused = getenv("MGTA_SORT_FUSED");
        return SortModes{bias ? atoi(bias) : 1, side ? atoi(side) : 1, fused ? atoi(fused) : 1};
    }
};

static double avg_segment_len(uint64_t n_items, int p, double prefix_frac) { return (double)n_items / std::max(1.0, std::pow(256.0, p) * prefix_frac); }
struct TopPlan {
    int P = 0, skip = 0;
    uint32_t bias = 0;
    double frac = 1.0;
    int T() const { return 8 * P + skip; }
    Digit pass_digit(int W, int i) const { return Digit{32 * W - 8 * (i + 1) - skip, 8, bias}; }
};
static TopPlan choose_top_plan(const mgta_ctx *ctx, uint64_t n_items, int max_top, double prefix_frac, uint32_t b_lo = 0, uint32_t b_hi = 0,
                               int mode = 0) {
    TopPlan plain;
    plain.frac = prefix_frac;
    if (ctx && ctx->force_full_lsd) return plain;
    while (plain.P < max_top && avg_segment_len(n_items, plain.P, prefix_frac) > (plain.P >= 3 ? 700.0 : 256.0)) ++plain.P;
    if (mode == 0 || b_hi <= b_lo || (b_lo == 0 && b_hi >= (uint32_t)MGTA_NUM_BUCKETS)) return plain;
    const uint32_t span = ((b_hi - b_lo) << 16) - 1u;
    const int skip_full = __builtin_clz(span | 1u);
    for (int P = 1; P <= max_top; ++P) {
        const int skip = std::min(skip_full, 32 - 8 * P);
        if (skip <= 0 || 8 * P + skip < 16) continue;
        const double frac = std::min(1.0, prefix_frac * std::pow(2.0, skip));
        const double limit = mode >= 2 ? (P >= 3 ? 700.0 : 256.0) : (P >= 3 ? 400.0 : 256.0);
        if (P < max_top && avg_segment_len(n_items, P, frac) > limit) continue;
        if (P < plain.P || (mode >= 2 && P <= plain.P)) return TopPlan{P, skip, b_lo << 16, frac};
        break;
    }
    return plain;
}

template <int WT>
struct SortJob {
    Key<WT> *a = nullptr, *b = nullptr;
    uint64_t n = 0;
    TopPlan top;
    std::vector<Digit> low;
    uint32_t mask_last2 = ~0u, mask_last = ~0u;
    int side_mode = 1;
    bool census_done = false;
    bool side_done = false;
    bool first_pass_done = false;
    bool uses_side() const { return side_mode > 0 && top.P >= 2 && kSideFits<WT>; }
};
struct SortLog {
    mgta_build_stats *S = nullptr;
    std::vector<Timer> scatter;
};

template <int WT>
static Key<WT> *global_passes(mgta_ctx *ctx, const SortJob<WT> &job, SortLog *log) {
    hipStream_t stream = ctx->stream;
    const uint64_t n = job.n, tiles = (n + kBlockTile - 1) / kBlockTile;
    uint64_t *d_hist = pool_get<uint64_t>(ctx, S_HIST, std::max<uint64_t>(1, tiles) * 256 * 8);
    uint64_t *d_totals = pool_get<uint64_t>(ctx, S_SMALL, 4096) + 8;
    uint8_t *d_side = job.uses_side() ? pool_get<uint8_t>(ctx, S_SIDE, n + 64) : nullptr;
    bool side_valid = job.side_done && d_side;
    const dim3 grid((unsigned)tiles), block(kSortThreads);
    Key<WT> *src = job.a, *dst = job.b;
    for (int i = job.top.P - 1 - (job.first_pass_done ? 1 : 0); i >= 0; --i) {
        const bool first = i == job.top.P - 1;
        const Digit dg = job.top.pass_digit(WT, i), dn = i > 0 ? job.top.pass_digit(WT, i - 1) : Digit{0, 0, 0};
        if (!(first && job.census_done)) {
            if (side_valid) {
                hipLaunchKernelGGL(radix_census_side_kernel, grid, block, 0, stream, d_side, n, tiles, d_hist);
                if (job.side_mode >= 2) {
                    std::vector<uint64_t> h_side(tiles * 256), h_keys(tiles * 256);
                    MGTA_HIP_CHECK(hipStreamSynchronize(stream));
                    MGTA_HIP_CHECK(hipMemcpy(h_side.data(), d_hist, tiles * 256 * 8, hipMemcpyDeviceToHost));
                    hipLaunchKernelGGL((radix_census_kernel<WT>), grid, block, 0, stream, src, n, dg, tiles, d_hist);
                    MGTA_HIP_CHECK(hipStreamSynchronize(stream));
                    MGTA_HIP_CHECK(hipMemcpy(h_keys.data(), d_hist, tiles * 256 * 8, hipMemcpyDeviceToHost));
                    if (h_side != h_keys) { set_error("internal: side-digit census differs from the census of the keys"); return nullptr; }
                }
            } else
                hipLaunchKernelGGL((radix_census_kernel<WT>), grid, block, 0, stream, src, n, dg, tiles, d_hist);
        }
        hipLaunchKernelGGL(radix_rowscan_kernel, dim3(256), dim3(1024), 0, stream, d_hist, tiles, d_totals);
        if (log) log->scatter.emplace_back(stream).start();
        const bool write_side = d_side && i > 0;
        auto launch = [&](auto biased, auto side, auto stable) {
            hipLaunchKernelGGL((radix_scatter_kernel<WT, decltype(biased)::value, decltype(side)::value, decltype(stable)::value>), grid, block, 0, stream, src, dst, n,
                               dg, tiles, d_hist, d_totals, decltype(side)::value ? d_side : nullptr, dn);
        };
        auto pick_stable = [&](auto biased, auto side) { first ? launch(biased, side, std::false_type{}) : launch(biased, side, std::true_type{}); };
        auto pick_side = [&](auto biased) {
            if constexpr (kSideFits<WT>) {
                if (write_side) { pick_stable(biased, std::true_type{}); return; }
            }
            pick_stable(biased, std::false_type{});
        };
        dg.bias ? pick_side(std::true_type{}) : pick_side(std::false_type{});
        side_valid = write_side;
        if (log) { log->scatter.back().end(); log->S->n_sort_launches++; }
        std::swap(src, dst);
    }
    return src;
}

template <int WT>
static Key<WT> *lds_finish(mgta_ctx *ctx, const SortJob<WT> &job, Key<WT> *src, Key<WT> *dst, SortLog *log) {
    hipStream_t stream = ctx->stream;
    const uint64_t n_items = job.n;
    const int T = job.top.T();
    const std::vector<Digit> &low = job.low;
    if (low.size() > 64) { set_error("too many sort digits"); return nullptr; }
    Digit *d_plan = pool_get<Digit>(ctx, S_PLAN, 64 * sizeof(Digit));
    MGTA_HIP_CHECK(hipMemcpyAsync(d_plan, low.data(), low.size() * sizeof(Digit), hipMemcpyHostToDevice, stream));
    const double avg_seg = avg_segment_len(n_items, job.top.P, job.top.frac);
    uint32_t margin = (uint32_t)std::min<double>(LocalCfg<WT>::kTile / 2, std::max<double>(LocalCfg<WT>::kTile / 8, 2.5 * avg_seg));
    margin = (margin + 63u) & ~63u;
    const uint32_t stride = (uint32_t)LocalCfg<WT>::kTile - margin;
    const uint64_t l_blocks = (n_items + stride - 1) / stride;
    if (l_blocks > 0x7FFFFFFFull) { set_error("too many sort tiles"); return nullptr; }
    const uint32_t big_cap = (uint32_t)l_blocks + 1;
    uint64_t *d_big = pool_get<uint64_t>(ctx, S_BIG, (2 * (uint64_t)big_cap + 2) * 8);
    uint32_t *d_big_count = reinterpret_cast<uint32_t *>(d_big + 2 * (uint64_t)big_cap);
    MGTA_HIP_CHECK(hipMemsetAsync(d_big_count, 0, 8, stream));
    uint64_t *d_lsd = pool_get<uint64_t>(ctx, S_LSD, 2 * l_blocks * 8);
    Timer t(stream);
    t.start();
    const bool skip_a = ctx->lsd_skip_left > 0;
    if (skip_a) --ctx->lsd_skip_left;
    const int ub = ((ctx->force_lsd_tiles & 1) || skip_a) ? 0 : std::max(0, std::min(8, (WT > 1 ? 40 : 32) - T));
    LocalPlan lp;
    lp.low_plan = d_plan; lp.n_low = (int)low.size(); lp.T = T;
    lp.upper = Digit{32 * WT - T - ub, ub};
    lp.mask_last2 = job.mask_last2; lp.mask_last = job.mask_last; lp.stride = stride;
    lp.lsd_list = d_lsd; lp.lsd_count = d_big_count + 1; lp.lsd_cap = (uint32_t)l_blocks;
    lp.debug = ctx->force_lsd_tiles >> 1;
    if (ub > 0)
        hipLaunchKernelGGL((local_sort_kernel<WT, true>), dim3((unsigned)l_blocks), dim3(kSortThreads), 0, stream, src, n_items, lp, d_big, d_big_count,
                           big_cap);
    else
        hipLaunchKernelGGL((local_sort_kernel<WT, false>), dim3((unsigned)l_blocks), dim3(kSortThreads), 0, stream, src, n_items, lp, d_big, d_big_count,
                           big_cap);
    t.end();
    uint32_t n_big = 0, n_lsd_tiles = 0;
    MGTA_HIP_CHECK(hipMemcpyAsync(&n_lsd_tiles, d_big_count + 1, 4, hipMemcpyDeviceToHost, stream));
    MGTA_HIP_CHECK(hipMemcpyAsync(&n_big, d_big_count, 4, hipMemcpyDeviceToHost, stream));
    MGTA_HIP_CHECK(hipStreamSynchronize(stream));
    const float ms_local = t.ms();
    if (n_big > big_cap) { set_error("more than %u oversized key segments in one pass", big_cap); return nullptr; }
    if (n_lsd_tiles > lp.lsd_cap) { set_error("internal: tile list overflow"); return nullptr; }
    if (ub > 0 && l_blocks >= 64 && 2 * (uint64_t)n_lsd_tiles > l_blocks) ctx->lsd_skip_left = 7;
    t.start();
    if (n_lsd_tiles > 0 && !(lp.debug & 2))
        hipLaunchKernelGGL((local_lsd_kernel<WT>), dim3(n_lsd_tiles), dim3(kSortThreads), 0, stream, src, d_lsd, d_lsd + 1, 2, lp);
    if (n_big > 0) {
        hipLaunchKernelGGL((segment_end_kernel<WT>), dim3(n_big), dim3(256), 0, stream, src, n_items, T, d_big, d_big + big_cap);
        hipLaunchKernelGGL((local_lsd_kernel<WT>), dim3(n_big), dim3(kSortThreads), 0, stream, src, d_big, d_big + big_cap, 1, lp);
        const bool use_big = BigCfg<WT>::kTile > 0 && !low.empty();
        if (use_big) hipLaunchKernelGGL((segment_lds_kernel<WT>), dim3(n_big), dim3(kSortThreads), 0, stream, src, d_big, d_big + big_cap, lp);
        hipLaunchKernelGGL((segment_sort_kernel<WT>), dim3(n_big), dim3(kSortThreads), 0, stream, src, dst, d_big, d_big + big_cap, d_plan,
                           (int)low.size(), (uint32_t)(use_big ? BigCfg<WT>::kTile : LocalCfg<WT>::kTile));
    }
    t.end();
    MGTA_HIP_CHECK(hipEventSynchronize(t.b));
    const float ms = t.ms();
    if (log) { log->S->ms_local_sort += ms_local + ms; log->S->n_lsd_tiles += n_lsd_tiles; log->S->n_big_segments += n_big; }
    return src;
}

template <int WT>
static Key<WT> *device_sort(mgta_ctx *ctx, const SortJob<WT> &job, SortLog *log = nullptr) {
    Key<WT> *src = global_passes(ctx, job, log);
    return src ? lds_finish(ctx, job, src, src == job.a ? job.b : job.a, log) : nullptr;
}

template <int W>
static int run_stage1(mgta_ctx *ctx, const mgta_reads *rd, uint64_t n_short, int k, int min_count, int need_mercy, uint64_t budget,
                      int side_mode, unsigned long long **is_solid_out, int *num_k1_out) {
    constexpr int WT = W + 2;
    hipStream_t stream = ctx->stream;
    const uint64_t n_reads = rd->n_reads;
    const uint64_t n_blocks = (n_reads + kReadsPerBlock - 1) / kReadsPerBlock;
    uint64_t *d_small = pool_get<uint64_t>(ctx, S_SMALL, 4096);
    uint64_t *d_total = d_small;
    unsigned int *d_maxlen = reinterpret_cast<unsigned int *>(d_small + 300);
    unsigned long long *d_mercy_count = reinterpret_cast<unsigned long long *>(d_small + 302), *d_num_mercy = d_mercy_count + 1;
    MGTA_HIP_CHECK(hipMemsetAsync(d_small + 300, 0, 64, stream));
    if (n_short > n_reads) n_short = n_reads;
    if (n_short) hipLaunchKernelGGL(max_len_kernel, dim3((unsigned)((n_short + 255) / 256)), dim3(256), 0, stream, rd->d_start, n_short, d_maxlen);
    unsigned int max_len = 0;
    MGTA_HIP_CHECK(hipMemcpyAsync(&max_len, d_maxlen, 4, hipMemcpyDeviceToHost, stream));
    MGTA_HIP_CHECK(hipStreamSynchronize(stream));
    if (n_reads >= 0xFFFFFFFFull) { set_error("stage 1: more than 2^32 reads"); return MGTA_EUNSUPPORTED; }
    const uint64_t bases_bound = rd->n_words * 16 + 16;
    const uint64_t n_pos_entries = (bases_bound >> kPosStepLog) + 2;
    uint32_t *d_pos2id = pool_get<uint32_t>(ctx, S_POS2ID, n_pos_entries * 4);
    hipLaunchKernelGGL(pos_to_id_kernel, dim3((unsigned)((n_pos_entries + 255) / 256)), dim3(256), 0, stream, rd->d_start, n_reads, n_pos_entries, d_pos2id);
    int cand_shift = 0;
    while (cand_shift < 40 && (((bases_bound << 2) | 3ull) << (cand_shift + 1)) >> (cand_shift + 1) == ((bases_bound << 2) | 3ull)) ++cand_shift;
    const int num_k1 = std::max<int>(0, (int)max_len - k);
    const uint64_t n_bits = (uint64_t)num_k1 * n_short;
    unsigned long long *d_solid = pool_get<unsigned long long>(ctx, S_SOLID, (n_bits / 64 + 2) * 8);
    MGTA_HIP_CHECK(hipMemsetAsync(d_solid, 0, (n_bits / 64 + 2) * 8, stream));
    unsigned long long *d_edge_count = pool_get<unsigned long long>(ctx, S_EDGE_COUNT, 65536 * 8);
    MGTA_HIP_CHECK(hipMemsetAsync(d_edge_count, 0, 65536 * 8, stream));
    uint32_t *d_block_count = pool_get<uint32_t>(ctx, S_BLOCK_COUNT, std::max<uint64_t>(1, n_blocks) * 4);
    uint64_t *d_block_base = pool_get<uint64_t>(ctx, S_BLOCK_BASE, std::max<uint64_t>(1, n_blocks) * 8);

    S1Args sa;
    sa.packed = rd->d_packed; sa.n_words = rd->n_words; sa.start = rd->d_start; sa.n_reads = n_reads; sa.k = k;
    sa.block_count = d_block_count; sa.block_base = d_block_base; sa.out = nullptr;
    Key<2> *d_mercy = nullptr;
    uint64_t mercy_cap = 0;
    int n_pass = 1;
    uint32_t b_lo = 0;
    while (b_lo < MGTA_NUM_BUCKETS) {
        uint32_t width = (MGTA_NUM_BUCKETS + n_pass - 1) / n_pass;
        uint32_t b_hi = std::min<uint32_t>(MGTA_NUM_BUCKETS, b_lo + width);
        sa.b_lo = b_lo; sa.b_hi = b_hi;
        uint64_t *d_scan_tmp = pool_get<uint64_t>(ctx, S_SCAN_TMP, scan_tmp_elems(std::max<uint64_t>(n_blocks, 1024)) * 8);
        if (n_blocks) hipLaunchKernelGGL((s1_scan_kernel<W, false>), dim3((unsigned)n_blocks), dim3(kScanBlock), 0, stream, sa);
        exclusive_scan_u32(stream, d_block_count, n_blocks, d_block_base, d_scan_tmp, d_total);
        uint64_t n_items = 0;
        MGTA_HIP_CHECK(hipMemcpyAsync(&n_items, d_total, 8, hipMemcpyDeviceToHost, stream));
        MGTA_HIP_CHECK(hipStreamSynchronize(stream));
        uint64_t n_tiles = (n_items + kBlockTile - 1) / kBlockTile;
        uint64_t need = 2 * n_items * sizeof(Key<WT>) + n_tiles * 256 * 8 + (need_mercy ? n_items * 8 : 0) + (8u << 20);
        uint64_t other = ctx->live_bytes - pool_bytes(ctx);
        if (need + need / 8 > budget - std::min<uint64_t>(budget, other) && width > 1) { n_pass *= 2; continue; }
        if (n_items > 0) {
            Key<WT> *d_a = pool_get<Key<WT>>(ctx, S_KEYS_A, n_items * sizeof(Key<WT>));
            Key<WT> *d_b = pool_get<Key<WT>>(ctx, S_KEYS_B, n_items * sizeof(Key<WT>));
            if (need_mercy && (!d_mercy || mercy_cap < 2 * n_items)) {
                uint64_t have = 0;
                MGTA_HIP_CHECK(hipMemcpy(&have, d_mercy_count, 8, hipMemcpyDeviceToHost));
                uint64_t new_cap = have + 2 * n_items;
                DevBuf keep;
                if (have) { keep.alloc(have * 8); MGTA_HIP_CHECK(hipMemcpy(keep.p, d_mercy, have * 8, hipMemcpyDeviceToDevice)); }
                d_mercy = pool_get<Key<2>>(ctx, S_MERCY, new_cap * 8);
                if (have) MGTA_HIP_CHECK(hipMemcpy(d_mercy, keep.p, have * 8, hipMemcpyDeviceToDevice));
                mercy_cap = new_cap;
            }
            sa.out = d_a;
            hipLaunchKernelGGL((s1_scan_kernel<W, true>), dim3((unsigned)n_blocks), dim3(kScanBlock), 0, stream, sa);
            const int pad1 = 32 * W - 2 * (k - 1) - 6;
            auto low_plan = [&](int T) {
                std::vector<Digit> plan;
                int top = 32 * WT - T;
                plan.push_back(Digit{0, 6});
                if (top > 64) plan.push_back(Digit{64, std::min(6, top - 64)});
                for (int pos = 64 + 6 + pad1; pos < top; pos += 8) plan.push_back(Digit{pos, std::min(8, top - pos)});
                return plan;
            };
            const int max_top = std::min(4, std::max(0, (2 * (k - 1)) / 8));
            SortJob<WT> job{d_a, d_b, n_items, choose_top_plan(ctx, n_items, max_top, (double)(b_hi - b_lo) / MGTA_NUM_BUCKETS)};
            job.low = low_plan(job.top.T()); job.mask_last2 = 0u; job.mask_last = 0x3Fu; job.side_mode = side_mode;
            Key<WT> *sorted = device_sort(ctx, job);
            if (!sorted) return MGTA_EUNSUPPORTED;
            char *scratch = reinterpret_cast<char *>(sorted == d_a ? d_b : d_a);
            uint64_t e_tiles = (n_items + kEmitTile - 1) / kEmitTile;
            uint32_t *d_tile_heads = pool_get<uint32_t>(ctx, S_TILE_HEADS, e_tiles * 4);
            uint64_t *d_tile_base = pool_get<uint64_t>(ctx, S_TILE_BASE, e_tiles * 8);
            d_scan_tmp = pool_get<uint64_t>(ctx, S_SCAN_TMP, scan_tmp_elems(std::max<uint64_t>(n_blocks, e_tiles)) * 8);
            hipLaunchKernelGGL((s1_mark_kernel<W>), dim3((unsigned)e_tiles), dim3(kEmitThreads), 0, stream, sorted, n_items, d_tile_heads);
            exclusive_scan_u32(stream, d_tile_heads, e_tiles, d_tile_base, d_scan_tmp, d_total);
            uint64_t m = 0;
            MGTA_HIP_CHECK(hipMemcpyAsync(&m, d_total, 8, hipMemcpyDeviceToHost, stream));
            MGTA_HIP_CHECK(hipStreamSynchronize(stream));
            uint64_t *run_start = reinterpret_cast<uint64_t *>(scratch);
            uint16_t *run_info = reinterpret_cast<uint16_t *>(scratch + m * 8);
            uint16_t *group_mask = reinterpret_cast<uint16_t *>(scratch + m * 10);
            hipLaunchKernelGGL((s1_compact_kernel<W>), dim3((unsigned)e_tiles), dim3(kEmitThreads), 0, stream, sorted, n_items, k, d_tile_base,
                               run_start, run_info);
            unsigned rb = (unsigned)((m + 255) / 256);
            hipLaunchKernelGGL(s1_group_kernel, dim3(rb), dim3(256), 0, stream, run_start, run_info, m, n_items, min_count, group_mask);
            hipLaunchKernelGGL((s1_apply_kernel<W>), dim3(std::min(rb, 8192u)), dim3(256), 0, stream, sorted, run_start, run_info, group_mask, m, n_items, min_count,
                               k, rd->d_start, n_reads, n_short, num_k1, d_solid, d_edge_count, d_mercy, d_mercy_count, mercy_cap, need_mercy,
                               d_pos2id, cand_shift);
        }
        b_lo = b_hi;
    }
    ctx->edge_counting.assign(65536, 0);
    MGTA_HIP_CHECK(hipMemcpyAsync(ctx->edge_counting.data(), d_edge_count, 65536 * 8, hipMemcpyDeviceToHost, stream));
    MGTA_HIP_CHECK(hipStreamSynchronize(stream));
    if (need_mercy) {
        uint64_t n_cand = 0;
        MGTA_HIP_CHECK(hipMemcpy(&n_cand, d_mercy_count, 8, hipMemcpyDeviceToHost));
        if (n_cand > mercy_cap) { set_error("mercy candidate list overflow"); return MGTA_ENOMEM; }
        if (n_cand > 0) {
            Key<2> *d_tmp = pool_get<Key<2>>(ctx, S_KEYS_A, n_cand * 8);
            auto low64 = [&](int T) {
                std::vector<Digit> plan;
                for (int pos = 0; pos < 64 - T; pos += 8) plan.push_back(Digit{pos, std::min(8, 64 - T - pos)});
                return plan;
            };
            SortJob<2> job{d_mercy, d_tmp, n_cand, choose_top_plan(ctx, n_cand, 4, 1.0)};
            job.low = low64(job.top.T()); job.side_mode = side_mode;
            Key<2> *cs = device_sort(ctx, job);
            if (!cs) return MGTA_EUNSUPPORTED;
            if ((int)max_len <= kMercyMaxLen) {
                hipLaunchKernelGGL(mercy_kernel<false>, dim3((unsigned)((n_cand + 255) / 256)), dim3(256), 0, stream, cs, n_cand, rd->d_start, n_reads, k,
                                   num_k1, d_solid, d_num_mercy, d_pos2id, cand_shift, (uint8_t *)nullptr, (uint64_t)0);
                MGTA_HIP_CHECK(hipGetLastError());
                MGTA_HIP_CHECK(hipStreamSynchronize(stream));
            } else {
                const uint64_t stride = ((uint64_t)max_len + 64 + 63) & ~63ull;
                const unsigned grid = (unsigned)std::min<uint64_t>((n_cand + 255) / 256, (uint64_t)ctx->num_cus * 8);
                DevBuf d_flags;
                d_flags.alloc((uint64_t)grid * 4 * 3 * stride, &ctx->live_bytes, &ctx->peak_bytes);
                hipLaunchKernelGGL(mercy_kernel<true>, dim3(grid), dim3(256), 0, stream, cs, n_cand, rd->d_start, n_reads, k, num_k1, d_solid,
                                   d_num_mercy, d_pos2id, cand_shift, d_flags.as<uint8_t>(), stride);
                MGTA_HIP_CHECK(hipGetLastError());
                MGTA_HIP_CHECK(hipStreamSynchronize(stream));
            }
        }
    }
    *is_solid_out = d_solid;
    *num_k1_out = num_k1;
    return MGTA_OK;
}

struct Pass {
    uint32_t b_lo = 0, b_hi = 0, width = 0;
    bool closed_form = false;
    uint64_t n_items = 0, n_tiles = 0, key_b = 0;
    uint64_t n_edges = 0, n_large = 0, n_tips = 0;
    uint16_t *rec = nullptr, *large = nullptr;
    uint32_t *tips = nullptr;
    int64_t *first = nullptr;
    uint32_t nb() const { return b_hi - b_lo; }
};

template <int W>
struct Build {
    mgta_ctx *ctx;
    hipStream_t stream = ctx->stream;
    const mgta_reads *rd = nullptr;
    uint64_t n_short = 0, n_blocks = 0;
    int k = 0, words_per_tip = 0, min_count = 1, need_mercy = 0;
    uint32_t bucket_begin = 0, bucket_end = 0;
    mgta_edge_sink sink = nullptr; void *user = nullptr;
    SortModes modes;
    uint64_t budget = 0;
    bool acc = false;
    ScanArgs sa{};
    uint64_t *d_block_base = nullptr, *d_total = nullptr, *d_kmers = nullptr, *d_tot3 = nullptr, *d_sentinel = nullptr;
    uint32_t multi_n = 0, multi_width = 0, multi_lo = 0;
    uint32_t *d_multi_count = nullptr;
    struct FusedAhead { bool on = false; int P = 0, skip = 0; uint32_t bias = 0; };
    FusedAhead fz_plan[kMaxFusedRanges];
    uint64_t *fz_table = nullptr;
    uint64_t wide_items = 0;
    uint32_t wide_nb = 0;
    bool fz_check_failed = false;
    mgta_build_stats S{};
    Timer t_all{stream}, t_ph{stream};
    SortLog log{&S, {}};
    std::vector<int64_t> h_first, h_items;
    std::vector<uint16_t> h_rec, h_large;
    std::vector<uint32_t> h_tips;
    explicit Build(mgta_ctx *c) : ctx(c) {}

    int run() {
        int rc = start();
        if (rc == MGTA_OK) rc = solid_from_stage1();
        if (rc != MGTA_OK) return rc;
        t_all.start();
        int n_pass = 1;
        for (uint32_t b_lo = bucket_begin; b_lo < bucket_end;) {
            Pass p;
            p.width = (bucket_end - bucket_begin + n_pass - 1) / n_pass;
            p.b_lo = b_lo; p.b_hi = std::min<uint32_t>(bucket_end, b_lo + p.width);
            count_pass(p);
            if (const int more = admit_pass(p, n_pass)) { n_pass = more; wide_items = p.n_items; wide_nb = p.nb(); continue; }
            S.n_items += (int64_t)p.n_items;
            S.n_passes++;
            if (p.n_items > 0) {
                Key<W> *a = pool_get<Key<W>>(ctx, S_KEYS_A, p.key_b), *b = pool_get<Key<W>>(ctx, S_KEYS_B, p.key_b);
                const SortJob<W> job = plan_sort(p, a, b);
                write_keys(p, job);
                if (fz_check_failed) { set_error("internal: the fused key writer left keys outside the slice of their first sort digit"); return MGTA_EINTERNAL; }
                Key<W> *sorted = sort_keys(job);
                if (!sorted) return MGTA_EUNSUPPORTED;
                if ((rc = drop_sentinels(p)) != MGTA_OK || (rc = emit(p, sorted, sorted == a ? b : a)) != MGTA_OK) return rc;
            }
            publish_last(p.b_lo, p.b_hi, p.rec, p.n_edges, p.tips, p.n_tips, p.first, p.large, p.n_large);
            if (acc && p.n_items > 0) append_to_stream(p);
            S.n_edges += (int64_t)p.n_edges; S.n_large += (int64_t)p.n_large; S.n_tips += (int64_t)p.n_tips;
            if ((rc = deliver_pass(p)) != MGTA_OK) return rc;
            b_lo = p.b_hi;
        }
        if (acc) publish_last(bucket_begin, bucket_end, ctx->acc_rec.p, ctx->acc_n_rec, ctx->acc_tips.p, ctx->acc_n_tips, nullptr,
                              ctx->acc_has_large ? ctx->acc_large.p : nullptr, ctx->acc_n_large);
        ctx->acc_valid = acc;
        S.ms_total = t_all.stop();
        for (const Timer &t : log.scatter) S.ms_sort_scatter += t.ms();
        S.bytes_peak = ctx->peak_bytes;
        return MGTA_OK;
    }

    int start() {
        words_per_tip = (2 * k + 31) / 32;
        n_blocks = (rd->n_reads + kReadsPerBlock - 1) / kReadsPerBlock;
        if (n_blocks * (uint64_t)kScanBlock >= (1ull << 32)) { set_error("too many reads for one launch (%llu)", (unsigned long long)rd->n_reads); return MGTA_EUNSUPPORTED; }
        S.k = k; S.words_per_key = W; S.words_per_tip = words_per_tip; S.n_reads = (int64_t)rd->n_reads;
        ctx->peak_bytes = ctx->live_bytes;
        size_t free_b = 0, total_b = 0;
        MGTA_HIP_CHECK(hipMemGetInfo(&free_b, &total_b));
        const uint64_t avail = (uint64_t)free_b + pool_bytes(ctx);
        budget = ctx->mem_limit ? std::min<uint64_t>(ctx->mem_limit, avail) : (uint64_t)(avail * 0.9);
        acc = ctx->keep_stream != 0;
        ctx->acc_valid = false; ctx->acc_n_rec = 0; ctx->acc_n_tips = 0;
        ctx->acc_n_large = 0; ctx->acc_has_large = acc && ctx->keep_multiplicity;
        if (acc) ctx->acc_items.assign(MGTA_NUM_BUCKETS, 0);
        point_scans_at_pool();
        uint64_t *d_small = pool_get<uint64_t>(ctx, S_SMALL, 4096);
        d_total = d_small; d_kmers = d_small + 1; d_tot3 = d_small + 2; d_sentinel = d_small + 5;
        sa.packed = rd->d_packed; sa.n_words = rd->n_words; sa.start = rd->d_start; sa.n_reads = rd->n_reads; sa.k = k; sa.n_short = n_short;
        sa.n_kmers = (unsigned long long *)d_kmers; sa.n_sentinel = (unsigned long long *)d_sentinel;
        return MGTA_OK;
    }
    void point_scans_at_pool() {
        sa.block_count = pool_get<uint32_t>(ctx, S_BLOCK_COUNT, std::max<uint64_t>(1, n_blocks) * 4);
        sa.block_base = d_block_base = pool_get<uint64_t>(ctx, S_BLOCK_BASE, std::max<uint64_t>(1, n_blocks) * 8);
    }

    int solid_from_stage1() {
        if (min_count <= 1) return MGTA_OK;
        unsigned long long *sol = nullptr;
        int nk1 = 0;
        t_ph.start();
        const int rc = run_stage1<W>(ctx, rd, n_short, k, min_count, need_mercy, budget, modes.side, &sol, &nk1);
        if (rc != MGTA_OK) return rc;
        S.ms_stage1 = t_ph.stop();
        sa.is_solid = sol; sa.num_k1_per_read = nk1;
        point_scans_at_pool();
        return MGTA_OK;
    }

    void count_pass(Pass &p) {
        const bool first_pass = S.n_passes == 0;
        t_ph.start();
        sa.b_lo = p.b_lo; sa.b_hi = p.b_hi;
        sa.n_kmers = first_pass ? (unsigned long long *)d_kmers : nullptr;
        if (first_pass) MGTA_HIP_CHECK(hipMemsetAsync(d_kmers, 0, 8, stream));
        uint64_t *d_scan_tmp = pool_get<uint64_t>(ctx, S_SCAN_TMP, scan_tmp_elems(std::max<uint64_t>(n_blocks, 1024)) * 8);
        static_assert(kReadsPerBlock == 64, "item_count_closed_kernel: one lane per read of a workgroup");
        p.closed_form = !sa.is_solid && p.b_lo == 0 && p.b_hi == (uint32_t)MGTA_NUM_BUCKETS && !ctx->force_full_lsd;
        const uint32_t *counts = sa.block_count;
        sa.multi_n = 0; sa.multi_width = 0; sa.multi_magic = 0;
        if (n_blocks && (p.closed_form || sa.n_kmers))
            hipLaunchKernelGGL(item_count_closed_kernel, dim3((unsigned)((n_blocks + 63) / 64)), dim3(256), 0, stream, sa.start, sa.n_reads, n_blocks, k,
                               p.closed_form ? sa.block_count : nullptr, sa.n_kmers);
        if (n_blocks && !p.closed_form) {
            sa.n_kmers = nullptr;
            const uint32_t width = p.width, b_lo = p.b_lo, ranges_left = (bucket_end - b_lo + width - 1) / width;
            if (multi_n && (width != multi_width || b_lo < multi_lo || (b_lo - multi_lo) % width != 0 || (b_lo - multi_lo) / width >= multi_n)) multi_n = 0;
            if (!multi_n && ranges_left > 1 && ranges_left <= (uint32_t)kMaxCountRanges) {
                d_multi_count = pool_get<uint32_t>(ctx, S_MULTI_COUNT, (uint64_t)ranges_left * n_blocks * 4);
                ScanArgs sm = sa;
                sm.block_count = d_multi_count; sm.b_hi = bucket_end; sm.multi_width = width; sm.multi_n = ranges_left; sm.multi_magic = ((1ull << 32) + width - 1) / width;
                fz_table = nullptr;
                if (plan_ahead(sm, b_lo, width, ranges_left)) {
                    fz_table = sm.fz_hist = pool_get<uint64_t>(ctx, S_FUSED_HIST, fused_table_bytes(ranges_left));
                    if constexpr (W >= 2)
                        hipLaunchKernelGGL((item_scan_kernel<W, false, true>), dim3((unsigned)n_blocks), dim3(kScanBlock), 0, stream, sm);
                } else
                    hipLaunchKernelGGL((item_scan_kernel<W, false>), dim3((unsigned)n_blocks), dim3(kScanBlock), 0, stream, sm);
                multi_n = ranges_left; multi_width = width; multi_lo = b_lo;
            }
            if (multi_n) counts = d_multi_count + (uint64_t)((b_lo - multi_lo) / width) * n_blocks;
            else hipLaunchKernelGGL((item_scan_kernel<W, false>), dim3((unsigned)n_blocks), dim3(kScanBlock), 0, stream, sa);
        }
        exclusive_scan_u32(stream, counts, n_blocks, d_block_base, d_scan_tmp, d_total);
        MGTA_HIP_CHECK(hipMemcpyAsync(&p.n_items, d_total, 8, hipMemcpyDeviceToHost, stream));
        S.ms_count += t_ph.stop();
        if (first_pass) {
            unsigned long long km = 0;
            MGTA_HIP_CHECK(hipMemcpy(&km, d_kmers, 8, hipMemcpyDeviceToHost));
            S.n_kmers = (int64_t)km;
        }
    }

    int max_top() const { return (2 * k + 4 + 7) / 8 > 1 ? std::min(4, (32 * W - 8) / 8) : 0; }
    uint64_t fused_table_bytes(uint32_t ranges) const { return (uint64_t)ranges * 256 * std::max<uint64_t>(1, n_blocks) * 8; }

    bool plan_ahead(ScanArgs &sm, uint32_t b_lo, uint32_t width, uint32_t ranges) {
        for (FusedAhead &f : fz_plan) f = FusedAhead{};
        if (modes.fused <= 0 || W < 2 || !wide_nb || ranges > (uint32_t)kMaxFusedRanges) return false;
        bool any = false;
        uint64_t est_max = 0;
        for (uint32_t g = 0; g < ranges; ++g) {
            const uint32_t lo = b_lo + g * width, hi = std::min<uint32_t>(bucket_end, lo + width);
            const uint64_t est = (uint64_t)((double)wide_items * (double)(hi - lo) / (double)wide_nb);
            const TopPlan tp = choose_top_plan(ctx, est, max_top(), (double)(hi - lo) / MGTA_NUM_BUCKETS, lo, hi, modes.bias);
            est_max = std::max(est_max, est);
            sm.fz_bias[g] = 0; sm.fz_shift[g] = 0;
            if (tp.P < 1 || tp.T() > 32) continue;
            fz_plan[g] = FusedAhead{true, tp.P, tp.skip, tp.bias};
            sm.fz_bias[g] = tp.bias; sm.fz_shift[g] = (uint32_t)(32 - tp.T());
            any = true;
        }
        if (!any) return false;
        uint64_t key_b = 0;
        const uint64_t need = pass_need(est_max, &key_b) + fused_table_bytes(ranges);
        return need + need / 8 <= avail_bytes();
    }

    uint64_t pass_need(uint64_t n_items, uint64_t *key_b) const {
        const uint64_t n_tiles = (n_items + kBlockTile - 1) / kBlockTile;
        *key_b = std::max<uint64_t>(n_items * sizeof(Key<W>), n_items * 12) + 4096;
        return 2 * *key_b + n_tiles * 256 * 8 + n_items * 2 + n_items  + (8u << 20);
    }
    uint64_t avail_bytes() const {
        uint64_t other = ctx->live_bytes - pool_bytes(ctx);
        if (acc) {
            const double range_frac = (double)(bucket_end - bucket_begin) / (double)MGTA_NUM_BUCKETS;
            const uint64_t est = (uint64_t)((double)S.n_kmers * 1.5 * range_frac) + (64ull << 20);
            const uint64_t have = ctx->acc_rec.bytes + ctx->acc_tips.bytes;
            other += est > have ? est - have : 0;
        }
        return budget - std::min<uint64_t>(budget, other);
    }

    int admit_pass(Pass &p, int n_pass) {
        p.n_tiles = (p.n_items + kBlockTile - 1) / kBlockTile;
        uint64_t need = pass_need(p.n_items, &p.key_b);
        const uint64_t avail = avail_bytes();
        if ((int)ctx->pool.size() > S_FUSED_HIST && ctx->pool[S_FUSED_HIST].bytes) {
            const uint64_t with = need + ctx->pool[S_FUSED_HIST].bytes;
            if (with + with / 8 <= avail) need = with;
            else if (need + need / 8 <= avail) { ctx->pool[S_FUSED_HIST].release(); fz_table = nullptr; }
        }
        if (need + need / 8 <= avail || p.width <= 1) return 0;
        const double ratio = (double)(need + need / 8) / (double)std::max<uint64_t>(avail, 1) * 1.03;
        return std::max(n_pass + 1, (int)std::ceil((double)n_pass * ratio));
    }

    SortJob<W> plan_sort(const Pass &p, Key<W> *a, Key<W> *b) const {
        SortJob<W> job{a, b, p.n_items, choose_top_plan(ctx, p.n_items, max_top(), (double)p.nb() / MGTA_NUM_BUCKETS, p.b_lo, p.b_hi, modes.bias)};
        job.low = low_digit_plan(k, W, job.top.T());
        job.side_mode = modes.side;
        job.census_done = p.closed_form && job.top.P >= 1 && p.n_tiles <= 0x7FFFFFFFull;
        job.side_done = !p.closed_form && job.uses_side();
        if (!p.closed_form && fz_table && multi_n && p.width == multi_width && p.b_lo >= multi_lo && (p.b_lo - multi_lo) % p.width == 0) {
            const uint32_t g = (p.b_lo - multi_lo) / p.width;
            if (g < multi_n && g < (uint32_t)kMaxFusedRanges) {
                const FusedAhead &f = fz_plan[g];
                job.first_pass_done = f.on && job.top.P >= 1 && f.P == job.top.P && f.skip == job.top.skip && f.bias == job.top.bias;
            }
        }
        return job;
    }

    void write_keys(const Pass &p, const SortJob<W> &job) {
        t_ph.start();
        sa.out = job.a;
        if (p.closed_form) MGTA_HIP_CHECK(hipMemsetAsync(d_sentinel, 0, 8, stream));
        const int shift = 32 - job.top.T();
        if (job.census_done) {
            uint64_t *d_hist = pool_get<uint64_t>(ctx, S_HIST, std::max<uint64_t>(1, p.n_tiles) * 256 * 8);
            hipLaunchKernelGGL((item_write_tiled_kernel<W>), dim3((unsigned)p.n_tiles), dim3(kScanBlock), 0, stream, sa, n_blocks, p.n_items,
                               shift, p.n_tiles, d_hist);
        } else if (p.closed_form)
            hipLaunchKernelGGL((item_write_closed_kernel<W>), dim3((unsigned)n_blocks), dim3(kScanBlock), 0, stream, sa);
        else if (job.first_pass_done) {
            uint64_t *tab = fz_table + (uint64_t)((p.b_lo - multi_lo) / p.width) * 256 * n_blocks;
            uint64_t *d_totals = pool_get<uint64_t>(ctx, S_SMALL, 4096) + 8;
            hipLaunchKernelGGL(radix_rowscan_kernel, dim3(256), dim3(1024), 0, stream, tab, n_blocks, d_totals);
            sa.fz_hist = tab; sa.fz_totals = d_totals; sa.fz_n = p.n_items;
            sa.fz_bias[0] = job.top.bias; sa.fz_shift[0] = (uint32_t)shift;
            if (job.side_done) {
                sa.side = pool_get<uint8_t>(ctx, S_SIDE, p.n_items + 64);
                sa.side_shift = shift + 8;
                sa.side_bias = job.top.bias;
            }
            if constexpr (W >= 2)
                hipLaunchKernelGGL((item_write_fused_kernel<W>), dim3((unsigned)n_blocks), dim3(kScanBlock), 0, stream, sa);
            sa.side = nullptr; sa.fz_hist = nullptr; sa.fz_totals = nullptr;
            S.n_fused_passes++;
            if (modes.fused >= 2) {
                uint32_t *d_bad = reinterpret_cast<uint32_t *>(pool_get<uint64_t>(ctx, S_SMALL, 4096) + 320);
                uint32_t bad[2] = {0, 0};
                MGTA_HIP_CHECK(hipMemsetAsync(d_bad, 0, 8, stream));
                const unsigned grid = (unsigned)std::min<uint64_t>((p.n_items + kScanBlock - 1) / kScanBlock, (uint64_t)ctx->num_cus * 16);
                hipLaunchKernelGGL((fused_check_kernel<W>), dim3(grid), dim3(kScanBlock), 0, stream, job.a, p.n_items, d_totals, job.top.bias, (uint32_t)shift, d_bad);
                MGTA_HIP_CHECK(hipMemcpyAsync(bad, d_bad, 8, hipMemcpyDeviceToHost, stream));
                MGTA_HIP_CHECK(hipStreamSynchronize(stream));
                if (bad[0] || bad[1]) fz_check_failed = true;
            }
        } else {
            if (job.side_done) {
                sa.side = pool_get<uint8_t>(ctx, S_SIDE, p.n_items + 64);
                sa.side_shift = shift;
                sa.side_bias = job.top.bias;
            }
            hipLaunchKernelGGL((item_scan_kernel<W, true>), dim3((unsigned)n_blocks), dim3(kScanBlock), 0, stream, sa);
            sa.side = nullptr;
        }
        S.ms_gen += t_ph.stop();
    }

    Key<W> *sort_keys(const SortJob<W> &job) {
        t_ph.start();
        Key<W> *sorted = device_sort(ctx, job, &log);
        if (sorted) S.ms_sort += t_ph.stop();
        return sorted;
    }

    int drop_sentinels(Pass &p) {
        if (!p.closed_form || ((k + 1) & 1)) return MGTA_OK;
        unsigned long long n_sent = 0;
        MGTA_HIP_CHECK(hipMemcpy(&n_sent, d_sentinel, 8, hipMemcpyDeviceToHost));
        if (n_sent >= p.n_items) { set_error("internal: %llu sentinel keys among %llu items", n_sent, (unsigned long long)p.n_items); return MGTA_EINTERNAL; }
        p.n_items -= n_sent;
        S.n_items -= (int64_t)n_sent;
        return MGTA_OK;
    }

    int emit(Pass &p, const Key<W> *sorted, Key<W> *scratch_keys) {
        const uint64_t n_items = p.n_items;
        t_ph.start();
        char *scratch = reinterpret_cast<char *>(scratch_keys);
        uint64_t e_tiles = (n_items + kEmitTile - 1) / kEmitTile;
        uint64_t *d_scan_tmp = pool_get<uint64_t>(ctx, S_SCAN_TMP, scan_tmp_elems(std::max<uint64_t>(std::max(n_blocks, e_tiles), n_items / kDecideTile + 1)) * 8);
        if (e_tiles > 0xFFFFFFFFull) { set_error("too many emit tiles"); return MGTA_EUNSUPPORTED; }
        unsigned long long *d_chain = pool_get<unsigned long long>(ctx, S_TILE_BASE, (e_tiles + 4) * 8);
        EmitChain chain;
        chain.state = d_chain; chain.total = d_chain + e_tiles;
        chain.ticket = reinterpret_cast<uint32_t *>(d_chain + e_tiles + 1); chain.error = reinterpret_cast<uint32_t *>(d_chain + e_tiles + 2);
        RunStarts sub_start;
        sub_start.lo = reinterpret_cast<uint32_t *>(scratch);
        uint16_t *rec = reinterpret_cast<uint16_t *>(scratch + n_items * 4);
        uint8_t *info = reinterpret_cast<uint8_t *>(scratch + n_items * 6);
        sub_start.base = reinterpret_cast<uint64_t *>(scratch + ((n_items * 7 + 7) & ~7ull));
        unsigned long long chain_out[3] = {0, 0, 0};
        for (int attempt = 0; attempt < 2; ++attempt) {
            MGTA_HIP_CHECK(hipMemsetAsync(d_chain, 0, (e_tiles + 4) * 8, stream));
            if (attempt == 0 && !ctx->force_full_lsd)
                hipLaunchKernelGGL((emit_compact_kernel<W, false>), dim3((unsigned)e_tiles), dim3(kEmitThreads), 0, stream, sorted, n_items, k, chain,
                                   (uint32_t)e_tiles, sub_start, info);
            else
                hipLaunchKernelGGL((emit_compact_kernel<W, true>), dim3((unsigned)e_tiles), dim3(kEmitThreads), 0, stream, sorted, n_items, k, chain,
                                   (uint32_t)e_tiles, sub_start, info);
            MGTA_HIP_CHECK(hipMemcpyAsync(chain_out, d_chain + e_tiles, 24, hipMemcpyDeviceToHost, stream));
            MGTA_HIP_CHECK(hipStreamSynchronize(stream));
            if ((uint32_t)chain_out[2] == 0) break;
        }
        if ((uint32_t)chain_out[2] != 0) { set_error("internal: chained scan of the emitter timed out"); return MGTA_EINTERNAL; }
        const uint64_t m = chain_out[0];
        uint64_t d_tiles = (m + kDecideTile - 1) / kDecideTile;
        uint32_t *ce = pool_get<uint32_t>(ctx, S_CNT, d_tiles * 4 * 3), *cl = ce + d_tiles, *ct = cl + d_tiles;
        uint64_t *be = pool_get<uint64_t>(ctx, S_BASE, d_tiles * 8 * 3), *bl = be + d_tiles, *bt = bl + d_tiles;
        p.first = pool_get<int64_t>(ctx, S_FIRST, (uint64_t)MGTA_NUM_BUCKETS * 3 * 8);
        MGTA_HIP_CHECK(hipMemsetAsync(p.first, 0xFF, (uint64_t)p.nb() * 3 * 8, stream));
        hipLaunchKernelGGL(emit_decide_kernel, dim3((unsigned)d_tiles), dim3(kDecideThreads), 0, stream, sub_start, info, m, n_items,
                           rec, ce, cl, ct);
        exclusive_scan_u32(stream, ce, d_tiles, be, d_scan_tmp, d_tot3);
        exclusive_scan_u32(stream, cl, d_tiles, bl, d_scan_tmp, d_tot3 + 1);
        exclusive_scan_u32(stream, ct, d_tiles, bt, d_scan_tmp, d_tot3 + 2);
        uint64_t tot3[3];
        MGTA_HIP_CHECK(hipMemcpyAsync(tot3, d_tot3, 24, hipMemcpyDeviceToHost, stream));
        MGTA_HIP_CHECK(hipStreamSynchronize(stream));
        p.n_edges = tot3[0]; p.n_large = tot3[1]; p.n_tips = tot3[2];
        p.rec = pool_get<uint16_t>(ctx, S_OUT_REC, p.n_edges * 2);
        p.large = pool_get<uint16_t>(ctx, S_OUT_LARGE, p.n_large * 2);
        p.tips = pool_get<uint32_t>(ctx, S_OUT_TIPS, p.n_tips * words_per_tip * 4);
        hipLaunchKernelGGL((emit_write_kernel<W>), dim3((unsigned)d_tiles), dim3(kDecideThreads), 0, stream, sorted, sub_start, info, rec, m,
                           n_items, be, bl, bt, words_per_tip, p.b_lo, p.rec, p.large, p.tips, p.first);
        S.ms_emit += t_ph.stop();
        return MGTA_OK;
    }

    void publish_last(uint32_t lo, uint32_t hi, const void *rec, uint64_t n_rec, const void *tips, uint64_t n_tips, const void *first,
                      const void *large, uint64_t n_large) {
        ctx->last_large = large; ctx->last_n_large = n_large;
        ctx->last_rec = rec; ctx->last_n_rec = n_rec; ctx->last_bucket_lo = lo; ctx->last_bucket_hi = hi;
        ctx->last_tips = tips; ctx->last_n_tips = n_tips; ctx->last_first = first; ctx->last_k = k; ctx->last_words_per_tip = words_per_tip;
    }

    void append_to_stream(const Pass &p) {
        const uint64_t tip_b = words_per_tip * 4;
        auto ensure = [&](DevBuf &buf, uint64_t used, uint64_t add) {
            if (used + add <= buf.bytes) return;
            const double done = (double)(p.b_hi - bucket_begin) / (double)(bucket_end - bucket_begin);
            uint64_t want = (uint64_t)((double)(used + add) / std::max(done, 1e-3) * 1.1) + (1u << 20);
            want = std::max<uint64_t>(want, used + add);
            DevBuf bigger;
            bigger.alloc(want, &ctx->live_bytes, &ctx->peak_bytes);
            if (used) MGTA_HIP_CHECK(hipMemcpyAsync(bigger.p, buf.p, used, hipMemcpyDeviceToDevice, stream));
            MGTA_HIP_CHECK(hipStreamSynchronize(stream));
            buf = std::move(bigger);
        };
        ensure(ctx->acc_rec, ctx->acc_n_rec * 2, p.n_edges * 2);
        ensure(ctx->acc_tips, ctx->acc_n_tips * tip_b, p.n_tips * tip_b);
        if (ctx->acc_has_large) {
            ensure(ctx->acc_large, ctx->acc_n_large * 2, p.n_large * 2);
            if (p.n_large) MGTA_HIP_CHECK(hipMemcpyAsync(ctx->acc_large.as<char>() + ctx->acc_n_large * 2, p.large, p.n_large * 2, hipMemcpyDeviceToDevice, stream));
        }
        if (p.n_edges) MGTA_HIP_CHECK(hipMemcpyAsync(ctx->acc_rec.as<char>() + ctx->acc_n_rec * 2, p.rec, p.n_edges * 2, hipMemcpyDeviceToDevice, stream));
        if (p.n_tips) MGTA_HIP_CHECK(hipMemcpyAsync(ctx->acc_tips.as<char>() + ctx->acc_n_tips * tip_b, p.tips, p.n_tips * tip_b, hipMemcpyDeviceToDevice, stream));
        h_first.resize((size_t)p.nb() * 3);
        MGTA_HIP_CHECK(hipMemcpyAsync(h_first.data(), p.first, (size_t)p.nb() * 3 * 8, hipMemcpyDeviceToHost, stream));
        MGTA_HIP_CHECK(hipStreamSynchronize(stream));
        int64_t nxt = (int64_t)p.n_edges;
        for (int64_t b = (int64_t)p.nb() - 1; b >= 0; --b) {
            int64_t f = h_first[(size_t)b * 3];
            if (f < 0) f = nxt;
            ctx->acc_items[(size_t)p.b_lo + (size_t)b] = nxt - f;
            nxt = f;
        }
        ctx->acc_n_rec += p.n_edges; ctx->acc_n_tips += p.n_tips; ctx->acc_n_large += p.n_large;
    }

    int deliver_pass(const Pass &p) {
        if (!sink) return MGTA_OK;
        const bool to_host = ctx->keep_stream != 2;
        const uint64_t n_tip_words = p.n_tips * words_per_tip;
        h_items.assign((size_t)p.nb() * 3, 0);
        if (p.n_items > 0) {
            t_ph.start();
            h_rec.resize(to_host ? p.n_edges : 0); h_large.resize(p.n_large); h_tips.resize(to_host ? n_tip_words : 0);
            h_first.resize((size_t)p.nb() * 3);
            if (p.n_edges && to_host) MGTA_HIP_CHECK(hipMemcpyAsync(h_rec.data(), p.rec, p.n_edges * 2, hipMemcpyDeviceToHost, stream));
            if (p.n_large) MGTA_HIP_CHECK(hipMemcpyAsync(h_large.data(), p.large, p.n_large * 2, hipMemcpyDeviceToHost, stream));
            if (p.n_tips && to_host) MGTA_HIP_CHECK(hipMemcpyAsync(h_tips.data(), p.tips, n_tip_words * 4, hipMemcpyDeviceToHost, stream));
            MGTA_HIP_CHECK(hipMemcpyAsync(h_first.data(), p.first, (size_t)p.nb() * 3 * 8, hipMemcpyDeviceToHost, stream));
            S.ms_d2h += t_ph.stop();
            int64_t nxt[3] = {(int64_t)p.n_edges, (int64_t)p.n_large, (int64_t)p.n_tips};
            for (int64_t b = (int64_t)p.nb() - 1; b >= 0; --b)
                for (int c = 0; c < 3; ++c) {
                    int64_t f = h_first[(size_t)b * 3 + c];
                    if (f < 0) f = nxt[c];
                    h_items[(size_t)b * 3 + c] = nxt[c] - f;
                    nxt[c] = f;
                }
        } else { h_rec.clear(); h_large.clear(); h_tips.clear(); }
        const int rc = sink(user, (int32_t)p.b_lo, (int32_t)p.b_hi, h_items.data(), to_host ? h_rec.data() : nullptr, (int64_t)p.n_edges,
                            h_large.data(), (int64_t)p.n_large, to_host ? h_tips.data() : nullptr, (int64_t)n_tip_words);
        if (rc != 0) { set_error("edge sink returned %d", rc); return MGTA_ESINK; }
        return MGTA_OK;
    }
};

template <int W = 1, class F>
static int with_key_words(int words, F &&f) {
    if constexpr (W < 9) {
        if (words == W) return f(std::integral_constant<int, W>{});
        return with_key_words<W + 1>(words, f);
    } else
        return f(std::integral_constant<int, W>{});
}

}

using namespace mgta;

extern "C" {

int mgta_reads_upload(mgta_ctx *ctx, const uint32_t *packed, uint64_t n_words, const uint64_t *start_idx, uint64_t n_reads,
                      mgta_reads **out) {
    if (!ctx || !packed || !start_idx || !out) { set_error("mgta_reads_upload: null argument"); return MGTA_EINVAL; }
    return guarded("mgta_reads_upload", [&] {
        MGTA_HIP_CHECK(hipSetDevice(ctx->device));
        auto r = std::make_unique<mgta_reads>();
        r->ctx = ctx; r->n_words = n_words; r->n_reads = n_reads;
        r->own_packed.alloc((n_words + 16) * 4, &ctx->live_bytes, &ctx->peak_bytes);
        r->own_start.alloc((n_reads + 1) * 8, &ctx->live_bytes, &ctx->peak_bytes);
        MGTA_HIP_CHECK(hipMemsetAsync((char *)r->own_packed.p + n_words * 4, 0, 64, ctx->stream));
        MGTA_HIP_CHECK(hipMemcpyAsync(r->own_packed.p, packed, n_words * 4, hipMemcpyHostToDevice, ctx->stream));
        MGTA_HIP_CHECK(hipMemcpyAsync(r->own_start.p, start_idx, (n_reads + 1) * 8, hipMemcpyHostToDevice, ctx->stream));
        MGTA_HIP_CHECK(hipStreamSynchronize(ctx->stream));
        r->d_packed = r->own_packed.as<uint32_t>();
        r->d_start = r->own_start.as<uint64_t>();
        ctx_retain(ctx);
        *out = r.release();
        return MGTA_OK;
    });
}

int mgta_reads_adopt_device(mgta_ctx *ctx, const uint32_t *d_packed, uint64_t n_words, const uint64_t *d_start, uint64_t n_reads,
                            mgta_reads **out) {
    if (!ctx || !d_packed || !d_start || !out) { set_error("mgta_reads_adopt_device: null argument"); return MGTA_EINVAL; }
    return guarded("mgta_reads_adopt_device", [&] {
        auto *r = new mgta_reads;
        r->ctx = ctx; r->d_packed = d_packed; r->d_start = d_start; r->n_words = n_words; r->n_reads = n_reads;
        ctx_retain(ctx);
        *out = r;
        return MGTA_OK;
    });
}

void mgta_reads_free(mgta_reads *r) {
    if (!r) return;
    mgta_ctx *c = r->ctx;
    delete r;
    ctx_release(c);
}

int mgta_sdbg_build_resident(mgta_ctx *ctx, const mgta_reads *rd, uint64_t n_short_reads, int k, int min_count, int need_mercy,
                             int32_t bucket_begin, int32_t bucket_end, mgta_edge_sink sink, void *user, mgta_build_stats *stats) {
    if (!ctx || !rd) { set_error("mgta_sdbg_build: null argument"); return MGTA_EINVAL; }
    if (k < 9 || k > 127) { set_error("k=%d out of range [9,127] (kMaxK, definitions.h:56)", k); return MGTA_EINVAL; }
    if (bucket_begin < 0 || bucket_end > MGTA_NUM_BUCKETS || bucket_begin >= bucket_end) {
        set_error("bucket range [%d,%d) invalid", bucket_begin, bucket_end);
        return MGTA_EINVAL;
    }
    if (min_count < 1) { set_error("min_count must be >= 1"); return MGTA_EINVAL; }
    return guarded("mgta_sdbg_build", [&] {
        MGTA_HIP_CHECK(hipSetDevice(ctx->device));
        return with_key_words((2 * k + 4 + 31) / 32, [&](auto w) {
            Build<decltype(w)::value> B(ctx);
            B.rd = rd; B.n_short = n_short_reads; B.k = k; B.min_count = min_count; B.need_mercy = need_mercy;
            B.bucket_begin = (uint32_t)bucket_begin; B.bucket_end = (uint32_t)bucket_end; B.sink = sink; B.user = user;
            B.modes = SortModes::from_env();
            const int rc = B.run();
            if (rc == MGTA_OK && stats) *stats = B.S;
            return rc;
        });
    });
}

int mgta_sdbg_last_counting(mgta_ctx *ctx, int64_t *hist) {
    if (!ctx || !hist) { set_error("mgta_sdbg_last_counting: null argument"); return MGTA_EINVAL; }
    if (ctx->edge_counting.size() != 65536) { set_error("no stage-1 run (min_count > 1) on this context yet"); return MGTA_EINVAL; }
    std::copy(ctx->edge_counting.begin(), ctx->edge_counting.end(), hist);
    return MGTA_OK;
}

int mgta_sort_plan(uint64_t n_items, int words_per_key, uint32_t bucket_begin, uint32_t bucket_end, int *n_passes, int *skip_bits) {
    if (!n_passes || !skip_bits || words_per_key < 2 || bucket_end > (uint32_t)MGTA_NUM_BUCKETS || bucket_begin >= bucket_end) {
        set_error("mgta_sort_plan: bad argument");
        return MGTA_EINVAL;
    }
    const TopPlan tp = choose_top_plan(nullptr, n_items, std::min(4, (32 * words_per_key - 8) / 8), (double)(bucket_end - bucket_begin) / MGTA_NUM_BUCKETS,
                                       bucket_begin, bucket_end, SortModes::from_env().bias);
    *n_passes = tp.P;
    *skip_bits = tp.skip;
    return MGTA_OK;
}

int mgta_sdbg_export_records_device(mgta_ctx *ctx, void *d_dst, uint64_t capacity_bytes, uint64_t *n_records) {
    if (!ctx || !n_records) { set_error("mgta_sdbg_export_records_device: null argument"); return MGTA_EINVAL; }
    *n_records = ctx->last_n_rec;
    if (ctx->last_k == 0 || (!ctx->last_rec && ctx->last_n_rec)) { set_error("no device-resident build output"); return MGTA_EINVAL; }
    if (!d_dst) return MGTA_OK;
    if (capacity_bytes < ctx->last_n_rec * 2) { set_error("destination too small"); return MGTA_EINVAL; }
    return guarded("mgta_sdbg_export_records_device", [&] {
        MGTA_HIP_CHECK(hipSetDevice(ctx->device));
        if (ctx->last_n_rec) MGTA_HIP_CHECK(hipMemcpyAsync(d_dst, ctx->last_rec, ctx->last_n_rec * 2, hipMemcpyDeviceToDevice, ctx->stream));
        MGTA_HIP_CHECK(hipStreamSynchronize(ctx->stream));
        return MGTA_OK;
    });
}

int mgta_sdbg_build(mgta_ctx *ctx, const uint32_t *packed, uint64_t n_words, const uint64_t *start_idx, uint64_t n_reads,
                    uint64_t n_short_reads, int k, int min_count, int need_mercy, mgta_edge_sink sink, void *user,
                    mgta_build_stats *stats) {
    mgta_reads *rd = nullptr;
    int rc = mgta_reads_upload(ctx, packed, n_words, start_idx, n_reads, &rd);
    if (rc != MGTA_OK) return rc;
    rc = mgta_sdbg_build_resident(ctx, rd, n_short_reads, k, min_count, need_mercy, 0, MGTA_NUM_BUCKETS, sink, user, stats);
    mgta_reads_free(rd);
    return rc;
}

}
```

Baseline: 8.743.

## Allow wider 9-bit radix digits in top sort passes to cut pass count

Adds support for radix digits wider than 8 bits (up to 9 for key widths 2-3 words) in the census, scatter and side-digit paths, with a wide wave-match ballot routine and 16-bit side entries. A widened top plan can then cover the same key bits in fewer scatter passes, lowering global memory traffic for the SdBG sort. In exchange, per-block LDS use and histogram size grow, which may lower occupancy. Each ballot loop also runs more iterations, and the side buffer doubles in size when a wide pass follows.

```diff
diff --git a/include/megagta_hip.h b/include/megagta_hip.h
--- a/include/megagta_hip.h
+++ b/include/megagta_hip.h
@@ -37,6 +37,8 @@
 int mgta_ctx_release_scratch(mgta_ctx *);
 int mgta_ctx_set_full_lsd(mgta_ctx *, int on);
 int mgta_sort_plan(uint64_t n_items, int words_per_key, uint32_t bucket_begin, uint32_t bucket_end, int *n_passes, int *skip_bits);
+int mgta_sort_plan_wide(uint64_t n_items, int words_per_key, uint32_t bucket_begin, uint32_t bucket_end, int *n_passes, int *skip_bits,
+                        int *widths );
 int mgta_ctx_set_search_cost_rate(mgta_ctx *, int expansions_per_seed);
 int mgta_ctx_set_search_cost_curve(mgta_ctx *, int expansions_per_seed, uint64_t knee_expansions, int expansions_per_seed_beyond);
 int mgta_ctx_set_search_arena(mgta_ctx *, int log2_base_nodes, uint64_t pool_bytes);
@@ -67,6 +69,7 @@
     uint64_t bytes_peak;
     double ms_stage1;
     int64_t n_fused_passes;
+    int64_t n_wide_passes;
 } mgta_build_stats;
 
 int mgta_reads_upload(mgta_ctx *, const uint32_t *packed_seq, uint64_t n_words, const uint64_t *start_idx,
diff --git a/megagta_amd/_lib.py b/megagta_amd/_lib.py
--- a/megagta_amd/_lib.py
+++ b/megagta_amd/_lib.py
@@ -26,7 +26,8 @@
                 ("n_tips", C.c_int64), ("n_large", C.c_int64), ("n_sort_launches", C.c_int64), ("ms_total", C.c_double),
                 ("ms_count", C.c_double), ("ms_gen", C.c_double), ("ms_sort", C.c_double), ("ms_emit", C.c_double),
                 ("ms_d2h", C.c_double), ("ms_sort_scatter", C.c_double), ("ms_local_sort", C.c_double), ("n_big_segments", C.c_int64), ("n_lsd_tiles", C.c_int64),
-                ("bytes_peak", C.c_uint64), ("ms_stage1", C.c_double), ("n_fused_passes", C.c_int64)]
+                ("bytes_peak", C.c_uint64), ("ms_stage1", C.c_double), ("n_fused_passes", C.c_int64),
+                ("n_wide_passes", C.c_int64)]
 
     def as_dict(self):
         return {n: getattr(self, n) for n, _ in self._fields_}
@@ -175,6 +176,7 @@
     "mgta_ctx_set_mem_limit": (C.c_int, [C.c_void_p, C.c_uint64]),
     "mgta_ctx_set_full_lsd": (C.c_int, [C.c_void_p, C.c_int]),
     "mgta_sort_plan": (C.c_int, [C.c_uint64, C.c_int, C.c_uint32, C.c_uint32, C.POINTER(C.c_int), C.POINTER(C.c_int)]),
+    "mgta_sort_plan_wide": (C.c_int, [C.c_uint64, C.c_int, C.c_uint32, C.c_uint32, C.POINTER(C.c_int), C.POINTER(C.c_int), C.POINTER(C.c_int)]),
     "mgta_reads_upload": (C.c_int, [C.c_void_p, C.c_void_p, C.c_uint64, C.c_void_p, C.c_uint64, C.POINTER(C.c_void_p)]),
     "mgta_reads_adopt_device": (C.c_int, [C.c_void_p, C.c_void_p, C.c_uint64, C.c_void_p, C.c_uint64, C.POINTER(C.c_void_p)]),
     "mgta_reads_free": (None, [C.c_void_p]),
diff --git a/megagta_amd/csrc/common.hpp b/megagta_amd/csrc/common.hpp
--- a/megagta_amd/csrc/common.hpp
+++ b/megagta_amd/csrc/common.hpp
@@ -82,7 +82,8 @@
 };
 
 enum Slot { S_BLOCK_COUNT, S_BLOCK_BASE, S_SCAN_TMP, S_SMALL, S_KEYS_A, S_KEYS_B, S_HIST, S_TILE_HEADS, S_TILE_BASE, S_CNT, S_BASE,
-            S_FIRST, S_OUT_REC, S_OUT_LARGE, S_OUT_TIPS, S_PLAN, S_BIG, S_LSD, S_MULTI_COUNT, S_POS2ID, S_SOLID, S_MERCY, S_EDGE_COUNT, S_SIDE, S_FUSED_HIST, S_NUM };
+            S_FIRST, S_OUT_REC, S_OUT_LARGE, S_OUT_TIPS, S_PLAN, S_BIG, S_LSD, S_MULTI_COUNT, S_POS2ID, S_SOLID, S_MERCY, S_EDGE_COUNT, S_SIDE, S_FUSED_HIST,
+            S_DIGIT_TOTALS , S_NUM };
 
 }
 
diff --git a/megagta_amd/csrc/sdbg_build.hip b/megagta_amd/csrc/sdbg_build.hip
--- a/megagta_amd/csrc/sdbg_build.hip
+++ b/megagta_amd/csrc/sdbg_build.hip
@@ -83,6 +83,7 @@
     uint8_t *side;
     int side_shift;
     uint32_t side_bias;
+    int side_bits;
     uint64_t *fz_hist;
     const uint64_t *fz_totals;
     uint64_t fz_n;
@@ -197,7 +198,11 @@
                 const uint64_t to = fs.next[d] + (i - fs.pos[d]);
                 if (to < a.fz_n) {
                     out[to] = key;
-                    if (a.side) a.side[to] = (uint8_t)((key.w[0] - a.side_bias) >> a.side_shift);
+                    if (a.side) {
+                        const uint32_t sd = (key.w[0] - a.side_bias) >> a.side_shift;
+                        if (a.side_bits > 8) reinterpret_cast<uint16_t *>(a.side)[to] = (uint16_t)(sd & ((1u << a.side_bits) - 1u));
+                        else a.side[to] = (uint8_t)sd;
+                    }
                 }
             }
             __syncthreads();
@@ -620,11 +625,28 @@
     for (int i = 0; i < N; ++i) dg[i] = __builtin_amdgcn_alignbit(hi[i], lo[i], (uint32_t)off) & mask;
 }
 
-template <int W>
+template <int BITS>
+__device__ __forceinline__ void wave_match_wide(uint32_t dg, bool valid, uint32_t &rank, uint32_t &cnt) {
+    static_assert(BITS > 8 && BITS <= 16, "wave_match covers digits of up to 8 bits");
+    const uint64_t v = __ballot(valid);
+    uint32_t lo = (uint32_t)v, hi = (uint32_t)(v >> 32);
+#pragma unroll
+    for (int b = 0; b < BITS; ++b) {
+        const int sx = (int)(dg << (31 - b)) >> 31;
+        const uint64_t bal = __ballot(sx < 0);
+        lo &= ~((uint32_t)bal ^ (uint32_t)sx);
+        hi &= ~((uint32_t)(bal >> 32) ^ (uint32_t)sx);
+    }
+    rank = __builtin_amdgcn_mbcnt_hi(hi, __builtin_amdgcn_mbcnt_lo(lo, 0u));
+    cnt = (uint32_t)__popc(lo) + (uint32_t)__popc(hi);
+}
+
+template <int W, int BITS = 8>
 __global__ __launch_bounds__(kSortThreads) void radix_census_kernel(const Key<W> *keys, uint64_t n, Digit d, uint64_t n_tiles,
                                                                      uint64_t *hist) {
-    __shared__ uint32_t h[256];
-    for (int i = threadIdx.x; i < 256; i += kSortThreads) h[i] = 0;
+    constexpr int kVals = 1 << BITS;
+    __shared__ uint32_t h[kVals];
+    for (int i = threadIdx.x; i < kVals; i += kSortThreads) h[i] = 0;
     __syncthreads();
     const uint32_t tile = xcd_tile(blockIdx.x, (uint32_t)n_tiles);
     uint64_t base = (uint64_t)tile * kBlockTile;
@@ -640,35 +662,46 @@
         }
     }
     __syncthreads();
-    for (int i = threadIdx.x; i < 256; i += kSortThreads) hist[(uint64_t)i * n_tiles + tile] = h[i];
-}
-
-__global__ __launch_bounds__(kSortThreads) void radix_census_side_kernel(const uint8_t *side, uint64_t n, uint64_t n_tiles, uint64_t *hist) {
-    __shared__ uint32_t h[256];
-    for (int i = threadIdx.x; i < 256; i += kSortThreads) h[i] = 0;
+    for (int i = threadIdx.x; i < kVals; i += kSortThreads) hist[(uint64_t)i * n_tiles + tile] = h[i];
+}
+
+template <int BITS> using SideEntry = std::conditional_t<(BITS > 8), uint16_t, uint8_t>;
+
+template <int BITS = 8>
+__global__ __launch_bounds__(kSortThreads) void radix_census_side_kernel(const SideEntry<BITS> *side, uint64_t n, uint64_t n_tiles, uint64_t *hist) {
+    constexpr int kVals = 1 << BITS;
+    constexpr uint32_t kMask = kVals - 1;
+    __shared__ uint32_t h[kVals];
+    for (int i = threadIdx.x; i < kVals; i += kSortThreads) h[i] = 0;
     __syncthreads();
     const uint32_t tile = xcd_tile(blockIdx.x, (uint32_t)n_tiles);
     const uint64_t base = (uint64_t)tile * kBlockTile;
     constexpr int kPerThread = kBlockTile / kSortThreads;
-#pragma unroll
-    for (int half = 0; half < kPerThread / 16; ++half) {
-        const uint64_t idx = base + (uint64_t)half * (kSortThreads * 16) + (uint64_t)threadIdx.x * 16;
-        if (idx + 16 <= n) {
+    constexpr int kPerLoad = 16 / (int)sizeof(SideEntry<BITS>);
+#pragma unroll
+    for (int half = 0; half < kPerThread / kPerLoad; ++half) {
+        const uint64_t idx = base + (uint64_t)half * (kSortThreads * kPerLoad) + (uint64_t)threadIdx.x * kPerLoad;
+        if (idx + kPerLoad <= n) {
             const uint4 v = *reinterpret_cast<const uint4 *>(side + idx);
             const uint32_t w[4] = {v.x, v.y, v.z, v.w};
 #pragma unroll
             for (int j = 0; j < 4; ++j) {
-                atomicAdd(&h[w[j] & 255u], 1u);
-                atomicAdd(&h[(w[j] >> 8) & 255u], 1u);
-                atomicAdd(&h[(w[j] >> 16) & 255u], 1u);
-                atomicAdd(&h[w[j] >> 24], 1u);
+                if constexpr (BITS > 8) {
+                    atomicAdd(&h[w[j] & kMask], 1u);
+                    atomicAdd(&h[(w[j] >> 16) & kMask], 1u);
+                } else {
+                    atomicAdd(&h[w[j] & 255u], 1u);
+                    atomicAdd(&h[(w[j] >> 8) & 255u], 1u);
+                    atomicAdd(&h[(w[j] >> 16) & 255u], 1u);
+                    atomicAdd(&h[w[j] >> 24], 1u);
+                }
             }
         } else {
-            for (uint64_t i = idx; i < n && i < idx + 16; ++i) atomicAdd(&h[side[i]], 1u);
+            for (uint64_t i = idx; i < n && i < idx + kPerLoad; ++i) atomicAdd(&h[side[i] & kMask], 1u);
         }
     }
     __syncthreads();
-    for (int i = threadIdx.x; i < 256; i += kSortThreads) hist[(uint64_t)i * n_tiles + tile] = h[i];
+    for (int i = threadIdx.x; i < kVals; i += kSortThreads) hist[(uint64_t)i * n_tiles + tile] = h[i];
 }
 
 template <int W>
@@ -795,28 +828,35 @@
     static constexpr int kChunk = kSub / kSortWaves;
 };
 
-template <int W>
+template <int W, int BITS = 8>
 struct ScatterShared {
+    static constexpr int kVals = 1 << BITS;
     Key<W> keys[ScatterCfg<W>::kSub];
-    uint16_t whist[kSortWaves][256];
-    uint64_t gbase[256];
-    uint64_t gdelta[256];
+    uint16_t whist[kSortWaves][kVals];
+    uint64_t gbase[kVals];
+    uint64_t gdelta[kVals];
     uint32_t scratch[kSortThreads / 64 + 1];
 };
 
+template <int BITS = 8, int NEXT_BITS = 8>
 struct SideShared {
-    uint8_t bytes[kBlockTile];
-    uint64_t gtile[256];
-    uint32_t toff[257];
+    static constexpr int kVals = 1 << BITS;
+    SideEntry<NEXT_BITS> bytes[kBlockTile];
+    uint64_t gtile[kVals];
+    uint32_t toff[kVals + 1];
 };
 
-template <int W, bool BIASED = false, bool SIDE = false, bool STABLE = true>
-__device__ __forceinline__ void scatter_subtiles(ScatterShared<W> &sh, const Key<W> *in, Key<W> *out, uint64_t n, Digit d, SideShared *ss = nullptr,
-                                                 Digit d_next = Digit{0, 0, 0}) {
+template <int W, bool BIASED = false, bool SIDE = false, bool STABLE = true, int BITS = 8, int NEXT_BITS = 8>
+__device__ __forceinline__ void scatter_subtiles(ScatterShared<W, BITS> &sh, const Key<W> *in, Key<W> *out, uint64_t n, Digit d,
+                                                 SideShared<BITS, NEXT_BITS> *ss = nullptr, Digit d_next = Digit{0, 0, 0}) {
     constexpr int kItemsPerThread = ScatterCfg<W>::kIpt, kSubTile = ScatterCfg<W>::kSub, kWaveChunk = ScatterCfg<W>::kChunk;
+    constexpr int kVals = 1 << BITS, kValWaves = kVals / 64;
+    constexpr uint32_t kDigitMask = kVals - 1;
+    static_assert(BITS >= 8 && kValWaves <= kSortWaves && BITS + 13 <= 31, "a thread per digit value; digit | place in the sub-tile << BITS | valid << 31");
+    static_assert(STABLE || BITS == 8, "only the first pass to run is unstable, and that one sorts on 8 bits");
     const int tid = threadIdx.x, lane = lane_id(), wv = wave_id();
     uint16_t *whist = sh.whist[wv];
-    for (int i = lane; i < 256; i += 64) whist[i] = 0;
+    for (int i = lane; i < kVals; i += 64) whist[i] = 0;
     constexpr bool kPrefetch = W * kItemsPerThread <= 16;
     Key<W> key[kItemsPerThread], nxt[kItemsPerThread];
     auto load = [&](Key<W> (&dst)[kItemsPerThread], uint64_t sub_base) {
@@ -837,15 +877,16 @@
                 uint32_t j = (uint32_t)wv * kWaveChunk + (uint32_t)it * 64 + (uint32_t)lane;
                 bool valid = j < n_valid;
                 uint32_t dg = valid ? dr[it] : 0u, rank;
-                wave_match(dg, d.bits, valid, rank, cnt[it]);
-                dr[it] = dg | (rank << 8) | ((uint32_t)valid << 31);
+                if constexpr (BITS > 8) wave_match_wide<BITS>(dg, valid, rank, cnt[it]);
+                else wave_match(dg, d.bits, valid, rank, cnt[it]);
+                dr[it] = dg | (rank << BITS) | ((uint32_t)valid << 31);
             }
 #pragma unroll
             for (int it = 0; it < kItemsPerThread; ++it) {
                 if (dr[it] >> 31) {
-                    const uint32_t dg = dr[it] & 255u, rank = (dr[it] >> 8) & 0xFFu, prev = whist[dg];
+                    const uint32_t dg = dr[it] & kDigitMask, rank = (dr[it] >> BITS) & 0xFFu, prev = whist[dg];
                     if (rank == cnt[it] - 1) whist[dg] = (uint16_t)(prev + cnt[it]);
-                    dr[it] += prev << 8;
+                    dr[it] += prev << BITS;
                 }
                 wave_lds_fence();
             }
@@ -858,21 +899,21 @@
                 const uint32_t dg = valid ? dr[it] : 0u;
                 uint32_t taken = 0;
                 if (valid) taken = (atomicAdd(&wh32[dg >> 1], 1u << (16u * (dg & 1u))) >> (16u * (dg & 1u))) & 0xFFFFu;
-                dr[it] = dg | (taken << 8) | ((uint32_t)valid << 31);
+                dr[it] = dg | (taken << BITS) | ((uint32_t)valid << 31);
             }
             wave_lds_fence();
         }
         if (kPrefetch && sub_base + kSubTile < n) load(nxt, sub_base + kSubTile);
         __syncthreads();
         uint32_t tot = 0, inc = 0;
-        if (wv < 4) {
+        if (wv < kValWaves) {
 #pragma unroll
             for (int w = 0; w < kSortWaves; ++w) tot += sh.whist[w][tid];
             inc = wave_incl_scan(tot);
             if (lane == 63) sh.scratch[wv] = inc;
         }
         __syncthreads();
-        if (wv < 4) {
+        if (wv < kValWaves) {
             uint32_t running = inc - tot;
             for (int w = 0; w < wv; ++w) running += sh.scratch[w];
             const uint64_t g = sh.gbase[tid];
@@ -885,13 +926,13 @@
 #pragma unroll
         for (int it = 0; it < kItemsPerThread; ++it) {
             if (dr[it] >> 31) {
-                const uint32_t pos = whist[dr[it] & 255u] + ((dr[it] >> 8) & 0x7FFFFFu);
+                const uint32_t pos = whist[dr[it] & kDigitMask] + ((dr[it] >> BITS) & (0x7FFFFFFFu >> BITS));
 #pragma unroll
                 for (int w = 0; w < W; ++w) sh.keys[pos].w[w] = key[it].w[w];
             }
         }
         __syncthreads();
-        for (int i = lane; i < 256; i += 64) whist[i] = 0;
+        for (int i = lane; i < kVals; i += 64) whist[i] = 0;
         if (kPrefetch) {
             Key<W> kk[kItemsPerThread];
             uint32_t dg[kItemsPerThread];
@@ -910,7 +951,7 @@
                     if (j < n_valid) {
                         const uint64_t to = sh.gdelta[dg[it]] + j;
                         out[to] = kk[it];
-                        ss->bytes[(uint32_t)(to - ss->gtile[dg[it]])] = (uint8_t)dn[it];
+                        ss->bytes[(uint32_t)(to - ss->gtile[dg[it]])] = (SideEntry<NEXT_BITS>)dn[it];
                     }
                 }
             } else {
@@ -931,7 +972,7 @@
                     const uint32_t dg = get_digit<W, BIASED>(kk, d);
                     const uint64_t to = sh.gdelta[dg] + j;
                     out[to] = kk;
-                    if constexpr (SIDE) ss->bytes[(uint32_t)(to - ss->gtile[dg])] = (uint8_t)get_digit<W, BIASED>(kk, d_next);
+                    if constexpr (SIDE) ss->bytes[(uint32_t)(to - ss->gtile[dg])] = (SideEntry<NEXT_BITS>)get_digit<W, BIASED>(kk, d_next);
                 }
             }
             if (sub_base + kSubTile < n) load(key, sub_base + kSubTile);
@@ -939,49 +980,55 @@
     }
 }
 
-template <int W> constexpr bool kSideFits = sizeof(ScatterShared<W>) + sizeof(SideShared) + 1024 <= 160 * 1024;
-
-template <int W, bool BIASED, bool SIDE = false, bool STABLE = true>
+template <int W, int BITS, int SIDE_BITS>
+constexpr bool kScatterFits = sizeof(ScatterShared<W, BITS>) + (SIDE_BITS ? sizeof(SideShared<BITS, (SIDE_BITS ? SIDE_BITS : 8)>) : 0) + 1024 <= 160 * 1024;
+template <int W> constexpr bool kSideFits = kScatterFits<W, 8, 8>;
+template <int W> constexpr bool kWideFits = W >= 2 && W <= 3 && kSideFits<W> && kScatterFits<W, 9, 9> && kScatterFits<W, 8, 9>;
+static_assert(kWideFits<3> && kWideFits<2> && !kWideFits<4> && !kScatterFits<3, 10, 9>, "DESIGN.md 5: the LDS bound of the wide scatter variants");
+
+template <int W, bool BIASED, bool SIDE = false, bool STABLE = true, int BITS = 8, int NEXT_BITS = 8>
 __global__ __launch_bounds__(kSortThreads, 4) void radix_scatter_kernel(const Key<W> *in, Key<W> *out, uint64_t n, Digit d,
                                                                       uint64_t n_tiles, const uint64_t *rowoff,
-                                                                      const uint64_t *totals, uint8_t *side = nullptr,
+                                                                      const uint64_t *totals, SideEntry<NEXT_BITS> *side = nullptr,
                                                                       Digit d_next = Digit{0, 0, 0}) {
-    __shared__ ScatterShared<W> sh;
+    constexpr int kVals = 1 << BITS;
+    static_assert(kVals <= kSortThreads, "a thread per digit value");
+    __shared__ ScatterShared<W, BITS> sh;
     __shared__ uint64_t s64[kSortThreads / 64 + 1];
     const int tid = threadIdx.x;
     const uint32_t tile = xcd_tile(blockIdx.x, (uint32_t)n_tiles);
-    uint64_t t = tid < 256 ? totals[tid] : 0;
+    uint64_t t = tid < kVals ? totals[tid] : 0;
     uint64_t ex = block_excl_scan64<kSortThreads>(t, s64, nullptr);
-    const uint64_t my_off = tid < 256 ? rowoff[(uint64_t)tid * n_tiles + tile] : 0;
-    if (tid < 256) sh.gbase[tid] = ex + my_off;
+    const uint64_t my_off = tid < kVals ? rowoff[(uint64_t)tid * n_tiles + tile] : 0;
+    if (tid < kVals) sh.gbase[tid] = ex + my_off;
     const uint64_t tile_base = (uint64_t)tile * kBlockTile;
     if constexpr (SIDE) {
-        __shared__ SideShared ss;
+        __shared__ SideShared<BITS, NEXT_BITS> ss;
         uint64_t c = 0;
-        if (tid < 256) c = (tile + 1 < n_tiles ? rowoff[(uint64_t)tid * n_tiles + tile + 1] : t) - my_off;
+        if (tid < kVals) c = (tile + 1 < n_tiles ? rowoff[(uint64_t)tid * n_tiles + tile + 1] : t) - my_off;
         __syncthreads();
         const uint64_t place = block_excl_scan64<kSortThreads>(c, s64, nullptr);
-        if (tid < 256) {
+        if (tid < kVals) {
             ss.toff[tid] = (uint32_t)place;
             ss.gtile[tid] = ex + my_off - place;
-            if (tid == 255) ss.toff[256] = (uint32_t)(place + c);
+            if (tid == kVals - 1) ss.toff[kVals] = (uint32_t)(place + c);
         }
         __syncthreads();
         if (tile_base >= n) return;
         const uint64_t cnt = (n - tile_base) < (uint64_t)kBlockTile ? (n - tile_base) : (uint64_t)kBlockTile;
-        scatter_subtiles<W, BIASED, true, STABLE>(sh, in + tile_base, out, cnt, d, &ss, d_next);
+        scatter_subtiles<W, BIASED, true, STABLE, BITS, NEXT_BITS>(sh, in + tile_base, out, cnt, d, &ss, d_next);
         __syncthreads();
         const int lane = lane_id(), wv = wave_id();
-        for (int v = wv * (256 / kSortWaves); v < (wv + 1) * (256 / kSortWaves); ++v) {
+        for (int v = wv * (kVals / kSortWaves); v < (wv + 1) * (kVals / kSortWaves); ++v) {
             const uint32_t from = ss.toff[v], len = ss.toff[v + 1] - from;
-            uint8_t *to = side + ss.gtile[v] + from;
+            SideEntry<NEXT_BITS> *to = side + ss.gtile[v] + from;
             for (uint32_t i = lane; i < len; i += 64) to[i] = ss.bytes[from + i];
         }
     } else {
         __syncthreads();
         if (tile_base >= n) return;
         const uint64_t cnt = (n - tile_base) < (uint64_t)kBlockTile ? (n - tile_base) : (uint64_t)kBlockTile;
-        scatter_subtiles<W, BIASED, false, STABLE>(sh, in + tile_base, out, cnt, d);
+        scatter_subtiles<W, BIASED, false, STABLE, BITS>(sh, in + tile_base, out, cnt, d);
     }
 }
 
@@ -1745,20 +1792,36 @@
 }
 
 struct SortModes {
-    int bias = 1, side = 1, fused = 1;
+    int bias = 1, side = 1, fused = 1, wide = 1;
     static SortModes from_env() {
-        const char *bias = getenv("MGTA_SORT_BIAS"), *side = getenv("MGTA_SORT_SIDE"), *fused = getenv("MGTA_SORT_FUSED");
-        return SortModes{bias ? atoi(bias) : 1, side ? atoi(side) : 1, fused ? atoi(fused) : 1};
+        const char *bias = getenv("MGTA_SORT_BIAS"), *side = getenv("MGTA_SORT_SIDE"), *fused = getenv("MGTA_SORT_FUSED"), *wide = getenv("MGTA_SORT_WIDE");
+        return SortModes{bias ? atoi(bias) : 1, side ? atoi(side) : 1, fused ? atoi(fused) : 1, wide ? atoi(wide) : 1};
     }
 };
 
 static double avg_segment_len(uint64_t n_items, int p, double prefix_frac) { return (double)n_items / std::max(1.0, std::pow(256.0, p) * prefix_frac); }
+static double avg_segment_len_bits(uint64_t n_items, int bits, double prefix_frac) { return (double)n_items / std::max(1.0, std::pow(2.0, bits) * prefix_frac); }
+constexpr int kMaxTop = 4;
 struct TopPlan {
     int P = 0, skip = 0;
     uint32_t bias = 0;
     double frac = 1.0;
-    int T() const { return 8 * P + skip; }
-    Digit pass_digit(int W, int i) const { return Digit{32 * W - 8 * (i + 1) - skip, 8, bias}; }
+    int width[kMaxTop] = {8, 8, 8, 8};
+    int key_bits() const { int t = 0; for (int i = 0; i < P; ++i) t += width[i]; return t; }
+    int T() const { return key_bits() + skip; }
+    int n_wide() const { int c = 0; for (int i = 0; i < P; ++i) c += width[i] > 8; return c; }
+    int max_width() const { int m = 8; for (int i = 0; i < P; ++i) m = std::max(m, width[i]); return m; }
+    bool same_digits(const TopPlan &o) const {
+        bool same = P == o.P && skip == o.skip && bias == o.bias;
+        for (int i = 0; same && i < P; ++i) same = width[i] == o.width[i];
+        return same;
+    }
+    Digit pass_digit(int W, int i) const {
+        int below = skip;
+        for (int j = 0; j <= i; ++j) below += width[j];
+        return Digit{32 * W - below, width[i], bias};
+    }
+    double avg_segment(uint64_t n_items) const { return avg_segment_len_bits(n_items, key_bits(), frac); }
 };
 static TopPlan choose_top_plan(const mgta_ctx *ctx, uint64_t n_items, int max_top, double prefix_frac, uint32_t b_lo = 0, uint32_t b_hi = 0,
                                int mode = 0) {
@@ -1781,6 +1844,35 @@
     return plain;
 }
 
+static TopPlan widen_top_plan(const TopPlan &base, uint64_t n_items, int max_top, double prefix_frac, uint32_t b_lo, uint32_t b_hi, int bias_mode,
+                              int wide) {
+    const int max_bits = 8 * std::min(max_top, kMaxTop);
+    if (wide <= 0 || base.P < 2) return base;
+    if (wide >= 2) {
+        TopPlan tp = base;
+        for (int i = 0; i < tp.P - 1 && tp.key_bits() < max_bits; ++i) tp.width[i] = 9;
+        if (tp.key_bits() + tp.skip > max_bits) {
+            tp.skip = max_bits - tp.key_bits();
+            if (tp.skip < 0 || (tp.skip > 0 && tp.T() < 16)) return base;
+            if (tp.skip == 0) tp.bias = 0;
+            tp.frac = std::min(1.0, prefix_frac * std::pow(2.0, tp.skip));
+        }
+        return tp;
+    }
+    if (base.P < 3) return base;
+    TopPlan tp;
+    tp.P = base.P - 1;
+    for (int i = 0; i < tp.P - 1; ++i) tp.width[i] = 9;
+    const bool sub_range = bias_mode != 0 && b_hi > b_lo && !(b_lo == 0 && b_hi >= (uint32_t)MGTA_NUM_BUCKETS);
+    const int skip_full = sub_range ? __builtin_clz((((b_hi - b_lo) << 16) - 1u) | 1u) : 0;
+    tp.skip = std::max(0, std::min(skip_full, max_bits - tp.key_bits()));
+    if (tp.skip > 0 && tp.T() < 16) tp.skip = 0;
+    tp.bias = tp.skip > 0 ? b_lo << 16 : 0u;
+    tp.frac = std::min(1.0, prefix_frac * std::pow(2.0, tp.skip));
+    if (tp.key_bits() > max_bits || tp.avg_segment(n_items) > 256.0) return base;
+    return tp;
+}
+
 template <int WT>
 struct SortJob {
     Key<WT> *a = nullptr, *b = nullptr;
@@ -1793,57 +1885,92 @@
     bool side_done = false;
     bool first_pass_done = false;
     bool uses_side() const { return side_mode > 0 && top.P >= 2 && kSideFits<WT>; }
+    uint64_t side_bytes() const { return n * (top.max_width() > 8 ? 2u : 1u) + 64; }
+    uint64_t hist_bytes() const { return std::max<uint64_t>(1, (n + kBlockTile - 1) / kBlockTile) * ((uint64_t)8 << top.max_width()); }
 };
+static uint64_t *digit_totals(mgta_ctx *ctx) { return pool_get<uint64_t>(ctx, S_DIGIT_TOTALS, 1024 * 8); }
 struct SortLog {
     mgta_build_stats *S = nullptr;
     std::vector<Timer> scatter;
 };
 
+template <int WT, int BITS, int NEXT_BITS>
+static bool global_pass(mgta_ctx *ctx, const SortJob<WT> &job, SortLog *log, const Key<WT> *src, Key<WT> *dst, Digit dg, Digit dn, bool first,
+                        bool side_valid, bool write_side, void *d_side, uint64_t *d_hist, uint64_t *d_totals) {
+    hipStream_t stream = ctx->stream;
+    const uint64_t n = job.n, tiles = (n + kBlockTile - 1) / kBlockTile;
+    constexpr uint64_t kVals = 1ull << BITS;
+    const dim3 grid((unsigned)tiles), block(kSortThreads);
+    if (!(first && job.census_done)) {
+        if (side_valid) {
+            hipLaunchKernelGGL((radix_census_side_kernel<BITS>), grid, block, 0, stream, static_cast<const SideEntry<BITS> *>(d_side), n, tiles, d_hist);
+            if (job.side_mode >= 2) {
+                std::vector<uint64_t> h_side(tiles * kVals), h_keys(tiles * kVals);
+                MGTA_HIP_CHECK(hipStreamSynchronize(stream));
+                MGTA_HIP_CHECK(hipMemcpy(h_side.data(), d_hist, tiles * kVals * 8, hipMemcpyDeviceToHost));
+                hipLaunchKernelGGL((radix_census_kernel<WT, BITS>), grid, block, 0, stream, src, n, dg, tiles, d_hist);
+                MGTA_HIP_CHECK(hipStreamSynchronize(stream));
+                MGTA_HIP_CHECK(hipMemcpy(h_keys.data(), d_hist, tiles * kVals * 8, hipMemcpyDeviceToHost));
+                if (h_side != h_keys) { set_error("internal: side-digit census differs from the census of the keys"); return false; }
+            }
+        } else
+            hipLaunchKernelGGL((radix_census_kernel<WT, BITS>), grid, block, 0, stream, src, n, dg, tiles, d_hist);
+    }
+    hipLaunchKernelGGL(radix_rowscan_kernel, dim3((unsigned)kVals), dim3(1024), 0, stream, d_hist, tiles, d_totals);
+    if (log) log->scatter.emplace_back(stream).start();
+    auto launch = [&](auto biased, auto side, auto stable) {
+        constexpr bool kSide = decltype(side)::value;
+        hipLaunchKernelGGL((radix_scatter_kernel<WT, decltype(biased)::value, kSide, decltype(stable)::value, BITS, kSide ? NEXT_BITS : 8>), grid, block, 0, stream,
+                           src, dst, n, dg, tiles, d_hist, d_totals, kSide ? static_cast<SideEntry<kSide ? NEXT_BITS : 8> *>(d_side) : nullptr, dn);
+    };
+    auto pick_stable = [&](auto biased, auto side) {
+        if constexpr (BITS == 8) {
+            if (first) { launch(biased, side, std::false_type{}); return; }
+        }
+        launch(biased, side, std::true_type{});
+    };
+    auto pick_side = [&](auto biased) {
+        if constexpr (kScatterFits<WT, BITS, NEXT_BITS>) {
+            if (write_side) { pick_stable(biased, std::true_type{}); return; }
+        }
+        pick_stable(biased, std::false_type{});
+    };
+    dg.bias ? pick_side(std::true_type{}) : pick_side(std::false_type{});
+    if (log) {
+        log->scatter.back().end();
+        log->S->n_sort_launches++;
+        if (BITS > 8) log->S->n_wide_passes++;
+    }
+    return true;
+}
+
 template <int WT>
 static Key<WT> *global_passes(mgta_ctx *ctx, const SortJob<WT> &job, SortLog *log) {
-    hipStream_t stream = ctx->stream;
-    const uint64_t n = job.n, tiles = (n + kBlockTile - 1) / kBlockTile;
-    uint64_t *d_hist = pool_get<uint64_t>(ctx, S_HIST, std::max<uint64_t>(1, tiles) * 256 * 8);
-    uint64_t *d_totals = pool_get<uint64_t>(ctx, S_SMALL, 4096) + 8;
-    uint8_t *d_side = job.uses_side() ? pool_get<uint8_t>(ctx, S_SIDE, n + 64) : nullptr;
+    uint64_t *d_hist = pool_get<uint64_t>(ctx, S_HIST, job.hist_bytes());
+    uint64_t *d_totals = digit_totals(ctx);
+    void *d_side = job.uses_side() ? pool_get<uint8_t>(ctx, S_SIDE, job.side_bytes()) : nullptr;
     bool side_valid = job.side_done && d_side;
-    const dim3 grid((unsigned)tiles), block(kSortThreads);
     Key<WT> *src = job.a, *dst = job.b;
     for (int i = job.top.P - 1 - (job.first_pass_done ? 1 : 0); i >= 0; --i) {
         const bool first = i == job.top.P - 1;
         const Digit dg = job.top.pass_digit(WT, i), dn = i > 0 ? job.top.pass_digit(WT, i - 1) : Digit{0, 0, 0};
-        if (!(first && job.census_done)) {
-            if (side_valid) {
-                hipLaunchKernelGGL(radix_census_side_kernel, grid, block, 0, stream, d_side, n, tiles, d_hist);
-                if (job.side_mode >= 2) {
-                    std::vector<uint64_t> h_side(tiles * 256), h_keys(tiles * 256);
-                    MGTA_HIP_CHECK(hipStreamSynchronize(stream));
-                    MGTA_HIP_CHECK(hipMemcpy(h_side.data(), d_hist, tiles * 256 * 8, hipMemcpyDeviceToHost));
-                    hipLaunchKernelGGL((radix_census_kernel<WT>), grid, block, 0, stream, src, n, dg, tiles, d_hist);
-                    MGTA_HIP_CHECK(hipStreamSynchronize(stream));
-                    MGTA_HIP_CHECK(hipMemcpy(h_keys.data(), d_hist, tiles * 256 * 8, hipMemcpyDeviceToHost));
-                    if (h_side != h_keys) { set_error("internal: side-digit census differs from the census of the keys"); return nullptr; }
-                }
-            } else
-                hipLaunchKernelGGL((radix_census_kernel<WT>), grid, block, 0, stream, src, n, dg, tiles, d_hist);
-        }
-        hipLaunchKernelGGL(radix_rowscan_kernel, dim3(256), dim3(1024), 0, stream, d_hist, tiles, d_totals);
-        if (log) log->scatter.emplace_back(stream).start();
         const bool write_side = d_side && i > 0;
-        auto launch = [&](auto biased, auto side, auto stable) {
-            hipLaunchKernelGGL((radix_scatter_kernel<WT, decltype(biased)::value, decltype(side)::value, decltype(stable)::value>), grid, block, 0, stream, src, dst, n,
-                               dg, tiles, d_hist, d_totals, decltype(side)::value ? d_side : nullptr, dn);
+        const int bits = dg.bits, next = i > 0 ? dn.bits : 8;
+        bool ok = false, known = true;
+        auto run = [&](auto b, auto nb) {
+            ok = global_pass<WT, decltype(b)::value, decltype(nb)::value>(ctx, job, log, src, dst, dg, dn, first, side_valid, write_side, d_side, d_hist, d_totals);
         };
-        auto pick_stable = [&](auto biased, auto side) { first ? launch(biased, side, std::false_type{}) : launch(biased, side, std::true_type{}); };
-        auto pick_side = [&](auto biased) {
-            if constexpr (kSideFits<WT>) {
-                if (write_side) { pick_stable(biased, std::true_type{}); return; }
-            }
-            pick_stable(biased, std::false_type{});
-        };
-        dg.bias ? pick_side(std::true_type{}) : pick_side(std::false_type{});
+        using std::integral_constant;
+        if (bits == 8 && next == 8) run(integral_constant<int, 8>{}, integral_constant<int, 8>{});
+        else if constexpr (kWideFits<WT>) {
+            if (bits == 8 && next == 9) run(integral_constant<int, 8>{}, integral_constant<int, 9>{});
+            else if (bits == 9 && (next == 9 || i == 0)) run(integral_constant<int, 9>{}, integral_constant<int, 9>{});
+            else known = false;
+        } else
+            known = false;
+        if (!known) { set_error("internal: no scatter kernel for a %d-bit digit before a %d-bit one at %d key words", bits, next, WT); return nullptr; }
+        if (!ok) return nullptr;
         side_valid = write_side;
-        if (log) { log->scatter.back().end(); log->S->n_sort_launches++; }
         std::swap(src, dst);
     }
     return src;
@@ -1858,7 +1985,7 @@
     if (low.size() > 64) { set_error("too many sort digits"); return nullptr; }
     Digit *d_plan = pool_get<Digit>(ctx, S_PLAN, 64 * sizeof(Digit));
     MGTA_HIP_CHECK(hipMemcpyAsync(d_plan, low.data(), low.size() * sizeof(Digit), hipMemcpyHostToDevice, stream));
-    const double avg_seg = avg_segment_len(n_items, job.top.P, job.top.frac);
+    const double avg_seg = job.top.avg_segment(n_items);
     uint32_t margin = (uint32_t)std::min<double>(LocalCfg<WT>::kTile / 2, std::max<double>(LocalCfg<WT>::kTile / 8, 2.5 * avg_seg));
     margin = (margin + 63u) & ~63u;
     const uint32_t stride = (uint32_t)LocalCfg<WT>::kTile - margin;
@@ -2092,7 +2219,7 @@
     uint64_t *d_block_base = nullptr, *d_total = nullptr, *d_kmers = nullptr, *d_tot3 = nullptr, *d_sentinel = nullptr;
     uint32_t multi_n = 0, multi_width = 0, multi_lo = 0;
     uint32_t *d_multi_count = nullptr;
-    struct FusedAhead { bool on = false; int P = 0, skip = 0; uint32_t bias = 0; };
+    struct FusedAhead { bool on = false; TopPlan top; };
     FusedAhead fz_plan[kMaxFusedRanges];
     uint64_t *fz_table = nullptr;
     uint64_t wide_items = 0;
@@ -2228,34 +2355,42 @@
     }
 
     int max_top() const { return (2 * k + 4 + 7) / 8 > 1 ? std::min(4, (32 * W - 8) / 8) : 0; }
+    TopPlan top_plan(uint64_t n_items, uint32_t b_lo, uint32_t b_hi) const {
+        const double frac = (double)(b_hi - b_lo) / MGTA_NUM_BUCKETS;
+        const TopPlan tp = choose_top_plan(ctx, n_items, max_top(), frac, b_lo, b_hi, modes.bias);
+        if (!kWideFits<W> || ctx->force_full_lsd) return tp;
+        return widen_top_plan(tp, n_items, max_top(), frac, b_lo, b_hi, modes.bias, modes.wide);
+    }
     uint64_t fused_table_bytes(uint32_t ranges) const { return (uint64_t)ranges * 256 * std::max<uint64_t>(1, n_blocks) * 8; }
 
     bool plan_ahead(ScanArgs &sm, uint32_t b_lo, uint32_t width, uint32_t ranges) {
         for (FusedAhead &f : fz_plan) f = FusedAhead{};
         if (modes.fused <= 0 || W < 2 || !wide_nb || ranges > (uint32_t)kMaxFusedRanges) return false;
         bool any = false;
+        int max_width = 8;
         uint64_t est_max = 0;
         for (uint32_t g = 0; g < ranges; ++g) {
             const uint32_t lo = b_lo + g * width, hi = std::min<uint32_t>(bucket_end, lo + width);
             const uint64_t est = (uint64_t)((double)wide_items * (double)(hi - lo) / (double)wide_nb);
-            const TopPlan tp = choose_top_plan(ctx, est, max_top(), (double)(hi - lo) / MGTA_NUM_BUCKETS, lo, hi, modes.bias);
+            const TopPlan tp = top_plan(est, lo, hi);
             est_max = std::max(est_max, est);
+            max_width = std::max(max_width, tp.max_width());
             sm.fz_bias[g] = 0; sm.fz_shift[g] = 0;
             if (tp.P < 1 || tp.T() > 32) continue;
-            fz_plan[g] = FusedAhead{true, tp.P, tp.skip, tp.bias};
+            fz_plan[g] = FusedAhead{true, tp};
             sm.fz_bias[g] = tp.bias; sm.fz_shift[g] = (uint32_t)(32 - tp.T());
             any = true;
         }
         if (!any) return false;
         uint64_t key_b = 0;
-        const uint64_t need = pass_need(est_max, &key_b) + fused_table_bytes(ranges);
+        const uint64_t need = pass_need(est_max, &key_b, max_width) + fused_table_bytes(ranges);
         return need + need / 8 <= avail_bytes();
     }
 
-    uint64_t pass_need(uint64_t n_items, uint64_t *key_b) const {
+    uint64_t pass_need(uint64_t n_items, uint64_t *key_b, int max_width) const {
         const uint64_t n_tiles = (n_items + kBlockTile - 1) / kBlockTile;
         *key_b = std::max<uint64_t>(n_items * sizeof(Key<W>), n_items * 12) + 4096;
-        return 2 * *key_b + n_tiles * 256 * 8 + n_items * 2 + n_items  + (8u << 20);
+        return 2 * *key_b + n_tiles * ((uint64_t)8 << max_width) + n_items * 2 + n_items * (max_width > 8 ? 2 : 1)  + (8u << 20);
     }
     uint64_t avail_bytes() const {
         uint64_t other = ctx->live_bytes - pool_bytes(ctx);
@@ -2270,7 +2405,7 @@
 
     int admit_pass(Pass &p, int n_pass) {
         p.n_tiles = (p.n_items + kBlockTile - 1) / kBlockTile;
-        uint64_t need = pass_need(p.n_items, &p.key_b);
+        uint64_t need = pass_need(p.n_items, &p.key_b, top_plan(p.n_items, p.b_lo, p.b_hi).max_width());
         const uint64_t avail = avail_bytes();
         if ((int)ctx->pool.size() > S_FUSED_HIST && ctx->pool[S_FUSED_HIST].bytes) {
             const uint64_t with = need + ctx->pool[S_FUSED_HIST].bytes;
@@ -2283,7 +2418,7 @@
     }
 
     SortJob<W> plan_sort(const Pass &p, Key<W> *a, Key<W> *b) const {
-        SortJob<W> job{a, b, p.n_items, choose_top_plan(ctx, p.n_items, max_top(), (double)p.nb() / MGTA_NUM_BUCKETS, p.b_lo, p.b_hi, modes.bias)};
+        SortJob<W> job{a, b, p.n_items, top_plan(p.n_items, p.b_lo, p.b_hi)};
         job.low = low_digit_plan(k, W, job.top.T());
         job.side_mode = modes.side;
         job.census_done = p.closed_form && job.top.P >= 1 && p.n_tiles <= 0x7FFFFFFFull;
@@ -2292,7 +2427,7 @@
             const uint32_t g = (p.b_lo - multi_lo) / p.width;
             if (g < multi_n && g < (uint32_t)kMaxFusedRanges) {
                 const FusedAhead &f = fz_plan[g];
-                job.first_pass_done = f.on && job.top.P >= 1 && f.P == job.top.P && f.skip == job.top.skip && f.bias == job.top.bias;
+                job.first_pass_done = f.on && job.top.P >= 1 && f.top.same_digits(job.top);
             }
         }
         return job;
@@ -2304,21 +2439,22 @@
         if (p.closed_form) MGTA_HIP_CHECK(hipMemsetAsync(d_sentinel, 0, 8, stream));
         const int shift = 32 - job.top.T();
         if (job.census_done) {
-            uint64_t *d_hist = pool_get<uint64_t>(ctx, S_HIST, std::max<uint64_t>(1, p.n_tiles) * 256 * 8);
+            uint64_t *d_hist = pool_get<uint64_t>(ctx, S_HIST, job.hist_bytes());
             hipLaunchKernelGGL((item_write_tiled_kernel<W>), dim3((unsigned)p.n_tiles), dim3(kScanBlock), 0, stream, sa, n_blocks, p.n_items,
                                shift, p.n_tiles, d_hist);
         } else if (p.closed_form)
             hipLaunchKernelGGL((item_write_closed_kernel<W>), dim3((unsigned)n_blocks), dim3(kScanBlock), 0, stream, sa);
         else if (job.first_pass_done) {
             uint64_t *tab = fz_table + (uint64_t)((p.b_lo - multi_lo) / p.width) * 256 * n_blocks;
-            uint64_t *d_totals = pool_get<uint64_t>(ctx, S_SMALL, 4096) + 8;
+            uint64_t *d_totals = digit_totals(ctx);
             hipLaunchKernelGGL(radix_rowscan_kernel, dim3(256), dim3(1024), 0, stream, tab, n_blocks, d_totals);
             sa.fz_hist = tab; sa.fz_totals = d_totals; sa.fz_n = p.n_items;
             sa.fz_bias[0] = job.top.bias; sa.fz_shift[0] = (uint32_t)shift;
             if (job.side_done) {
-                sa.side = pool_get<uint8_t>(ctx, S_SIDE, p.n_items + 64);
+                sa.side = pool_get<uint8_t>(ctx, S_SIDE, job.side_bytes());
                 sa.side_shift = shift + 8;
                 sa.side_bias = job.top.bias;
+                sa.side_bits = job.top.P >= 2 ? job.top.width[job.top.P - 2] : 8;
             }
             if constexpr (W >= 2)
                 hipLaunchKernelGGL((item_write_fused_kernel<W>), dim3((unsigned)n_blocks), dim3(kScanBlock), 0, stream, sa);
@@ -2336,9 +2472,10 @@
             }
         } else {
             if (job.side_done) {
-                sa.side = pool_get<uint8_t>(ctx, S_SIDE, p.n_items + 64);
+                sa.side = pool_get<uint8_t>(ctx, S_SIDE, job.side_bytes());
                 sa.side_shift = shift;
                 sa.side_bias = job.top.bias;
+                sa.side_bits = 8;
             }
             hipLaunchKernelGGL((item_scan_kernel<W, true>), dim3((unsigned)n_blocks), dim3(kScanBlock), 0, stream, sa);
             sa.side = nullptr;
@@ -2585,6 +2722,23 @@
     return MGTA_OK;
 }
 
+int mgta_sort_plan_wide(uint64_t n_items, int words_per_key, uint32_t bucket_begin, uint32_t bucket_end, int *n_passes, int *skip_bits, int *widths) {
+    if (!n_passes || !skip_bits || !widths || words_per_key < 2 || bucket_end > (uint32_t)MGTA_NUM_BUCKETS || bucket_begin >= bucket_end) {
+        set_error("mgta_sort_plan_wide: bad argument");
+        return MGTA_EINVAL;
+    }
+    const SortModes modes = SortModes::from_env();
+    const int max_top = std::min(4, (32 * words_per_key - 8) / 8);
+    const double frac = (double)(bucket_end - bucket_begin) / MGTA_NUM_BUCKETS;
+    TopPlan tp = choose_top_plan(nullptr, n_items, max_top, frac, bucket_begin, bucket_end, modes.bias);
+    const bool fits = with_key_words(words_per_key, [&](auto w) { return (int)kWideFits<decltype(w)::value>; }) > 0;
+    if (fits) tp = widen_top_plan(tp, n_items, max_top, frac, bucket_begin, bucket_end, modes.bias, modes.wide);
+    *n_passes = tp.P;
+    *skip_bits = tp.skip;
+    for (int i = 0; i < kMaxTop; ++i) widths[i] = i < tp.P ? tp.width[tp.P - 1 - i] : 0;
+    return MGTA_OK;
+}
+
 int mgta_sdbg_export_records_device(mgta_ctx *ctx, void *d_dst, uint64_t capacity_bytes, uint64_t *n_records) {
     if (!ctx || !n_records) { set_error("mgta_sdbg_export_records_device: null argument"); return MGTA_EINVAL; }
     *n_records = ctx->last_n_rec;
```

New measurement: 9.004 (median of 6 runs). 1.03x the previous value.
